# sandyresearch/chipmunk

Hardware: AMD Instinct MI355X
Metric: DiT denoise steps/sec at fixed sparsity (higher is better)
Workload: dtype bf16

## Files before the change

### chipmunk_amd/_native.py

```python
from __future__ import annotations

import ctypes
import os

_HERE = os.path.dirname(os.path.abspath(__file__))
LIB_PATH = os.environ.get("CHIPMUNK_HIP_LIB") or os.path.join(_HERE, "lib", "libchipmunk_hip.so")

SYMBOLS = [
    "chipmunk_last_error", "chipmunk_abi_version", "chipmunk_set_option", "chipmunk_set_random_seed",
    "chipmunk_csp_attn", "chipmunk_csp_attn_out", "chipmunk_csp_128_attn", "chipmunk_dense_attn", "chipmunk_dense_colsum_attn",
    "chipmunk_csp_mlp_mm1", "chipmunk_csp_mlp_mm1_scatter", "chipmunk_csp_mlp_mm1_fp8", "chipmunk_csp_mlp_mm2_and_scatter_add", "chipmunk_csp_scatter_add", "chipmunk_csp_mlp_mm2",
    "chipmunk_csp_mlp_mm1_ragged", "chipmunk_csp_mlp_mm1_scatter_ragged", "chipmunk_csp_mlp_mm1_fp8_ragged", "chipmunk_csp_mlp_mm2_ragged",
    "chipmunk_csp_mlp_mm2_and_scatter_add_ragged", "chipmunk_csp_scatter_add_ragged", "chipmunk_block_mean_ragged", "chipmunk_transpose16_pitched",
    "chipmunk_csp_mlp_mm1_batched", "chipmunk_csp_mlp_mm1_scatter_batched", "chipmunk_csp_mlp_mm1_fp8_batched", "chipmunk_csp_mlp_mm2_batched",
    "chipmunk_csp_mlp_mm2_and_scatter_add_batched", "chipmunk_csp_scatter_add_batched",
    "chipmunk_csp_mlp_mm1_glu", "chipmunk_csp_mlp_mm1_glu_batched", "chipmunk_csp_mlp_mm1_glu_fp8", "chipmunk_csp_mlp_mm1_glu_fp8_batched",
    "chipmunk_topk_indices", "chipmunk_topk_delta_indices", "chipmunk_topk_mask", "chipmunk_mask_to_indices", "chipmunk_mask_to_sorted_indices", "chipmunk_packed_mask_to_indices", "chipmunk_mask_row_counts", "chipmunk_mask_to_ragged_indices", "chipmunk_copy_indices",
    "chipmunk_bitpack", "chipmunk_bitunpack", "chipmunk_transpose16", "chipmunk_block_mean", "chipmunk_quantize_fp8", "chipmunk_gather_rows", "chipmunk_qkv_split_norm", "chipmunk_split_heads_rownorm", "chipmunk_dense_colsum_topk_mask", "chipmunk_dense_attn_strided", "chipmunk_csp_attn_out_ragged", "chipmunk_compact_indices", "chipmunk_residual_ln_modulate", "chipmunk_dense_colsum_attn_strided", "chipmunk_dense_colsum_topk_mask_strided", "chipmunk_release_scratch", "chipmunk_big_scratch_fallbacks",
    "chipmunk_host_alloc", "chipmunk_host_free", "chipmunk_copy_d2h_async", "chipmunk_copy_h2d_async", "chipmunk_host_bytes",
]

_lib = None


def lib() -> ctypes.CDLL:
    global _lib
    if _lib is None:
        if not os.path.exists(LIB_PATH):
            raise ImportError(
                f"{LIB_PATH} is missing: build it with `python -m chipmunk_amd.build` (hipcc --offload-arch=gfx950). "
                "chipmunk_amd has no CPU fallback.")
        _lib = ctypes.CDLL(LIB_PATH)
        _lib.chipmunk_last_error.restype = ctypes.c_char_p
        _lib.chipmunk_abi_version.restype = ctypes.c_int
        for item in filter(None, os.environ.get("CHIPMUNK_AMD_OPTIONS", "").split(",")):
            name, _, val = item.partition("=")
            if _lib.chipmunk_set_option(name.strip().encode(), int(val)) != 0:
                raise ValueError(f"CHIPMUNK_AMD_OPTIONS: {_lib.chipmunk_last_error().decode()}")
    return _lib


def last_error() -> str:
    return lib().chipmunk_last_error().decode()


def check(rc: int, what: str) -> None:
    if rc != 0:
        raise RuntimeError(f"{what}: {last_error()}")


def set_option(name: str, value: int) -> None:
    check(lib().chipmunk_set_option(name.encode(), int(value)), "chipmunk_set_option")


def manual_seed(seed: int) -> None:
    check(lib().chipmunk_set_random_seed(ctypes.c_uint64(int(seed) & 0xFFFFFFFFFFFFFFFF)), "chipmunk_set_random_seed")


class HostBuffer:

    def __init__(self, numel: int, dtype) -> None:
        import torch
        self.dtype = dtype
        self._numel = int(numel)
        self._itemsize = torch.empty(0, dtype=dtype).element_size()
        self.nbytes = self._numel * self._itemsize
        p = ctypes.c_void_p()
        check(lib().chipmunk_host_alloc(ctypes.c_size_t(max(self.nbytes, 1)), ctypes.byref(p)), "chipmunk_host_alloc")
        self.ptr = p.value

    def numel(self) -> int:
        return self._numel

    def element_size(self) -> int:
        return self._itemsize

    def is_pinned(self) -> bool:
        return True

    def free(self) -> None:
        if getattr(self, "ptr", None):
            lib().chipmunk_host_free(ctypes.c_void_p(self.ptr))
            self.ptr = None

    def __del__(self):
        try:
            self.free()
        except Exception:
            pass


def copy_d2h_async(host_ptr: int, dev_ptr: int, nbytes: int, stream: int) -> None:
    check(lib().chipmunk_copy_d2h_async(ctypes.c_void_p(host_ptr), ctypes.c_void_p(dev_ptr), ctypes.c_size_t(nbytes), ctypes.c_void_p(stream)),
          "chipmunk_copy_d2h_async")


def copy_h2d_async(dev_ptr: int, host_ptr: int, nbytes: int, stream: int) -> None:
    check(lib().chipmunk_copy_h2d_async(ctypes.c_void_p(dev_ptr), ctypes.c_void_p(host_ptr), ctypes.c_size_t(nbytes), ctypes.c_void_p(stream)),
          "chipmunk_copy_h2d_async")


# ... 5 lines not shown
```

### chipmunk_amd/csrc/attn.hip

```cpp
#include "common.h"
#include "attn_params.h"
#include <type_traits>

namespace {

constexpr int QG = 192;
constexpr int QW = 48;
constexpr int KVT = 32;
constexpr int NST = 4;
constexpr int KRING = 8;
constexpr int HD = 128;
constexpr int TILE_BYTES = KVT * HD * 2;
constexpr float SCALE_LOG2E = 0.08838834764f * 1.44269504089f;
constexpr int NSTV = NST + 1;
constexpr int KEY_RING_OFF = (NST + NSTV) * TILE_BYTES;
constexpr int CS_OFF = KEY_RING_OFF + KRING * 256;
constexpr int ATTN_LDS_BYTES = CS_OFF + 2 * 2 * 4 * KVT * 4;

__device__ __forceinline__ f32x4 mfma16(bf16x8 a, bf16x8 b, f32x4 c) {
    return __builtin_amdgcn_mfma_f32_16x16x32_bf16(a, b, c, 0, 0, 0);
}

#ifdef ATTN_PROF
__device__ unsigned long long g_attn_prof[8 * 8];
// ... 1132 lines not shown
    p.o_scale = 1.f;
    if (use_dense64(B, H, Nq, Nk)) {
        CM_CHECK((int64_t)Nk * p.ks[2] * 2 < (1ll << 32) && (int64_t)Nk * p.vs[2] * 2 < (1ll << 32),
                 "attention: one head's K or V spans more than 4 GiB (32-bit DMA offsets)");
        return chipmunk_dense64_launch(q, k, v, o, l, p.qs, p.ks, p.vs, p.os, B, H, Nq, Nk, (hipStream_t)stream);
    }
    return launch_attn<false, false, true>(p, (hipStream_t)stream);
}

extern "C" int chipmunk_dense_attn(const void *q, const void *k, const void *v, const int64_t q_strides[3],
                                   const int64_t k_strides[3], const int64_t v_strides[3], void *o, float *l, int B,
                                   int H, int Nq, int Nk, void *stream) {
    return chipmunk_dense_attn_strided(q, k, v, q_strides, k_strides, v_strides, o, nullptr, l, B, H, Nq, Nk, stream);
}

extern "C" int chipmunk_dense_colsum_attn_strided(const void *q, const void *k, const void *v, const int64_t q_strides[3],
                                                  const int64_t k_strides[3], const int64_t v_strides[3], const float *pin,
                                                  void *o, const int64_t *o_strides, void *cs, float *l, int B, int H, int Nq,
                                                  int Nk, int cs_stride, void *stream) {
    if (int e = check_common(q, k, v, o, B, H, Nq, Nk)) return e;
    CM_CHECK(l && cs && pin, "dense_colsum_attn: p / cs / l missing");
    CM_CHECK(cs_stride >= Nk, "dense_colsum_attn: cs row stride %d < Nk %d", cs_stride, Nk);
    if (int e = check_strides(q_strides, "q")) return e;
    if (int e = check_strides(k_strides, "k")) return e;
    if (int e = check_strides(v_strides, "v")) return e;
    AttnParams p = {};
    p.q = (const uint16_t *)q, p.k = (const uint16_t *)k, p.v = (const uint16_t *)v, p.o = (uint16_t *)o;
    for (int i = 0; i < 3; ++i) p.qs[i] = q_strides[i], p.ks[i] = k_strides[i], p.vs[i] = v_strides[i];
    if (int e = output_strides(p.os, o_strides, H, Nq)) return e;
    p.l_out = l, p.p_in = pin, p.cs = (uint16_t *)cs, p.cs_stride = cs_stride;
    p.B = B, p.H = H, p.Nq = Nq, p.Nk = Nk, p.G = (Nq + QG - 1) / QG;
    p.o_scale = 1.f;
    hipStream_t st = (hipStream_t)stream;
    int rc;
    if (chipmunk_get_option("attn_fused_colsum") == 5) {
        if (use_colsum64(B, H, Nq, Nk)) return chipmunk_colsum64_launch(p, st);
        return launch_attn<false, false, false, true>(p, st);
    }
    if (use_dense64(B, H, Nq, Nk)) {
        CM_CHECK((int64_t)Nk * p.ks[2] * 2 < (1ll << 32) && (int64_t)Nk * p.vs[2] * 2 < (1ll << 32),
                 "attention: one head's K or V spans more than 4 GiB (32-bit DMA offsets)");
        if (chipmunk_get_option("attn_fused_colsum") != 2) {
            int hc = H;
            uint16_t *part = nullptr;
            const int hc_min = chipmunk_get_option("attn_fused_colsum") == 4 ? 1 : 0;
            if (hc_min) hc = 1;
            for (; hc >= 1; hc /= 2) {
                part = (uint16_t *)chipmunk_big_scratch(st, chipmunk_colsum_part_bytes(hc == H ? B : 1, hc, Nq, Nk));
                if (part) break;
            }
            if (part && hc == H) return chipmunk_dense64_colsum_launch(p, part, st);
            if (part) {
                for (int b = 0; b < B; ++b)
                    for (int h0 = 0; h0 < H; h0 += hc) {
                        AttnParams c = p;
                        const int hn = H - h0 < hc ? H - h0 : hc;
                        const int64_t bh0 = (int64_t)b * H + h0;
                        c.q += b * p.qs[0] + h0 * p.qs[1], c.k += b * p.ks[0] + h0 * p.ks[1], c.v += b * p.vs[0] + h0 * p.vs[1];
                        c.o += b * p.os[0] + h0 * p.os[1];
                        c.l_out += bh0 * Nq, c.p_in += bh0 * Nq, c.cs += bh0 * p.G * (int64_t)cs_stride;
                        c.B = 1, c.H = hn;
                        if (int e = chipmunk_dense64_colsum_launch(c, part, st)) return e;
                    }
                return CHIPMUNK_OK;
            }
        }
        rc = chipmunk_dense64_launch(q, k, v, o, l, p.qs, p.ks, p.vs, p.os, B, H, Nq, Nk, st);
    } else {
        rc = launch_attn<false, false, true>(p, st);
    }
    if (rc != CHIPMUNK_OK) return rc;
    if (use_colsum64(B, H, Nq, Nk)) return chipmunk_colsum64_launch(p, st);
    return launch_attn<false, false, false, true>(p, st);
}

extern "C" int chipmunk_dense_colsum_attn(const void *q, const void *k, const void *v, const int64_t q_strides[3],
                                          const int64_t k_strides[3], const int64_t v_strides[3], const float *pin,
                                          void *o, void *cs, float *l, int B, int H, int Nq, int Nk, int cs_stride,
                                          void *stream) {
    return chipmunk_dense_colsum_attn_strided(q, k, v, q_strides, k_strides, v_strides, pin, o, nullptr, cs, l, B, H, Nq, Nk,
                                              cs_stride, stream);
}

extern "C" int chipmunk_dense_colsum_topk_mask_strided(const void *q, const void *k, const void *v, const int64_t q_strides[3],
                                               const int64_t k_strides[3], const int64_t v_strides[3], const float *pin, void *o,
                                               const int64_t *o_strides, float *l, int B, int H, int Nq, int Nk, const void *static_mask,
                                               int64_t static_stride, int static_rows, const void *group_flags, void *mask,
                                               int topk, double random_amount, void *stream) {
    if (int e = check_common(q, k, v, o, B, H, Nq, Nk)) return e;
    CM_CHECK(l && pin && mask, "dense_colsum_topk_mask: p / l / mask missing");
    if (int e = check_strides(q_strides, "q")) return e;
    if (int e = check_strides(k_strides, "k")) return e;
    if (int e = check_strides(v_strides, "v")) return e;
    hipStream_t st = (hipStream_t)stream;
    if (!use_dense64(B, H, Nq, Nk) || chipmunk_get_option("attn_fused_colsum") == 2 || (Nk & 3) || Nk > CHIPMUNK_TOPK_MASK_MAX_N)
        return CHIPMUNK_ERR_UNSUPPORTED;
    AttnParams p = {};
    p.q = (const uint16_t *)q, p.k = (const uint16_t *)k, p.v = (const uint16_t *)v, p.o = (uint16_t *)o;
    for (int i = 0; i < 3; ++i) p.qs[i] = q_strides[i], p.ks[i] = k_strides[i], p.vs[i] = v_strides[i];
    CM_CHECK((int64_t)Nk * p.ks[2] * 2 < (1ll << 32) && (int64_t)Nk * p.vs[2] * 2 < (1ll << 32),
             "attention: one head's K or V spans more than 4 GiB (32-bit DMA offsets)");
    if (int e = output_strides(p.os, o_strides, H, Nq)) return e;
    p.l_out = l, p.p_in = pin, p.cs = nullptr, p.cs_stride = 0;
    p.B = B, p.H = H, p.Nq = Nq, p.Nk = Nk, p.G = (Nq + QG - 1) / QG;
    p.o_scale = 1.f;
    uint16_t *part = (uint16_t *)chipmunk_big_scratch(st, chipmunk_colsum_part_bytes(B, H, Nq, Nk));
    if (!part) return CHIPMUNK_ERR_UNSUPPORTED;
    if (int e = chipmunk_dense64_colsum_launch(p, part, st)) return e;
    const int nrb = ((Nq + 255) / 256) * 2;
    return chipmunk_topk_mask_parts(part, chipmunk_colsum_part_stride(Nk), nrb, p.G, Nq, static_mask, static_stride, static_rows, group_flags, mask, B * H * p.G, Nk,
                                    topk, random_amount, st);
}

extern "C" int chipmunk_dense_colsum_topk_mask(const void *q, const void *k, const void *v, const int64_t q_strides[3],
                                               const int64_t k_strides[3], const int64_t v_strides[3], const float *pin, void *o,
                                               float *l, int B, int H, int Nq, int Nk, const void *static_mask,
                                               int64_t static_stride, int static_rows, const void *group_flags, void *mask,
                                               int topk, double random_amount, void *stream) {
    return chipmunk_dense_colsum_topk_mask_strided(q, k, v, q_strides, k_strides, v_strides, pin, o, nullptr, l, B, H, Nq, Nk,
                                                   static_mask, static_stride, static_rows, group_flags, mask, topk, random_amount,
                                                   stream);
}
```

### chipmunk_amd/csrc/attn_params.h

```cpp
#pragma once
#include <stdint.h>
#include <hip/hip_runtime.h>

struct AttnParams {
    const uint16_t *q, *k, *v;
    uint16_t *o;
    const uint16_t *o_in;
    int64_t qs[3], ks[3], vs[3], os[3];
    const int32_t *indices, *counts;
    const int64_t *idx_off;
    float *l_out;
    const float *p_in;
    uint16_t *cs;
    int cs_stride;
    int B, H, Nq, Nk, G, idx_stride;
    float o_scale;
    int split_full, nsplit;
    float *ws;
    int32_t *tickets;
    const int32_t *plan;
    int xcd_chunks;
    const float *kmax;
    uint16_t *cs_part;
    int cs_pstride;
    int probe;
};


int chipmunk_csp64_launch(const AttnParams &p, int inplace, int grid, hipStream_t stream);
int chipmunk_dense64_colsum_launch(const AttnParams &p, uint16_t *part, hipStream_t stream);
int chipmunk_topk_mask_parts(const uint16_t *part, int part_stride, int nrb, int groups_per_bh, int Nq, const void *static_mask, int64_t static_stride,
                             int static_rows, const void *group_flags, void *mask, int rows, int n, int k, double random_amount,
                             hipStream_t stream);
size_t chipmunk_colsum_part_bytes(int B, int H, int Nq, int Nk);
int chipmunk_colsum_part_stride(int Nk);
int chipmunk_colsum64_launch(const AttnParams &p, hipStream_t stream);
int chipmunk_csp96_launch(const AttnParams &p, int inplace, int grid, hipStream_t stream);
const float *chipmunk_knorm_max(const uint16_t *k, const int64_t ks[3], int B, int H, int Nk, hipStream_t stream);

__host__ __device__ inline int colsum_part_rows(int j, int nwg, int &r0, int &r1) {
    const int a = (3 * j) >> 2, w0 = 3 * j - 4 * a;
    r0 = 2 * a + (w0 ? 1 : 0);
    r1 = 2 * (a + 1);
    return (w0 >= 2 && a + 1 < nwg) ? 2 : 1;
}

struct IndexRow {
    const int32_t *ptr;
    int width;
};
__device__ __forceinline__ IndexRow index_row(const AttnParams &p, int64_t item) {
    if (p.idx_off) {
        const int64_t o = p.idx_off[item];
        return {p.indices + o, (int)(p.idx_off[item + 1] - o)};
    }
    return {p.indices + item * p.idx_stride, p.idx_stride};
}
```

### chipmunk_amd/csrc/capi.hip

```cpp
#include "common.h"

static thread_local char g_last_error[512] = "";

void chipmunk_set_error(const char *fmt, ...) {
    va_list ap;
    va_start(ap, fmt);
    vsnprintf(g_last_error, sizeof(g_last_error), fmt, ap);
    va_end(ap);
}

extern "C" const char *chipmunk_last_error(void) { return g_last_error; }
extern "C" int chipmunk_abi_version(void) { return 1; }

#include <string.h>
namespace {
struct Option { const char *name; int value; };
Option g_options[] = {{"mm1_variant", 0}, {"mm2_variant", 0}, {"attn_variant", 0}, {"m2i_variant", 0}, {"topk_variant", 0}, {"mm1_nr", 0}, {"mm2_nr", 0}, {"mm1_probe", 0}, {"attn_xcd_chunks", 0}, {"attn_no_order", 0}, {"attn_no_tail", 0}, {"mm1_no_split", 0}, {"mm2_no_split", 0}, {"attn_no_split", 0}, {"attn_split_gather", 0}, {"attn_pp", 0}, {"attn_dense64", 0}, {"attn_csp64", 0}, {"attn_colsum64", 0}, {"attn_csp96", 0}, {"attn_nomax", 0}, {"attn_fused_colsum", 0}, {"attn_cs_probe", 0}, {"big_scratch_gb", 0}, {"attn_balanced", 0}, {"attn_row_split", 0}, {"mm2_order", 0}, {"topk_mask_stream", 0}};
}
int chipmunk_get_option(const char *name) {
    for (auto &o : g_options) if (strcmp(o.name, name) == 0) return o.value;
    return 0;
}
extern "C" int chipmunk_set_option(const char *name, int value) {
    for (auto &o : g_options) if (strcmp(o.name, name) == 0) { o.value = value; return CHIPMUNK_OK; }
    chipmunk_set_error("unknown option '%s'", name);
    return CHIPMUNK_ERR_INVALID;
}

#include <atomic>
namespace {
std::atomic<uint64_t> g_rng_seed{0x243F6A8885A308D3ull};
std::atomic<uint64_t> g_rng_counter{0};
}
uint32_t chipmunk_next_random_salt() {
    uint64_t z = g_rng_seed.load(std::memory_order_relaxed) + 0x9E3779B97F4A7C15ull * (g_rng_counter.fetch_add(1) + 1);
    z = (z ^ (z >> 30)) * 0xBF58476D1CE4E5B9ull;
    z = (z ^ (z >> 27)) * 0x94D049BB133111EBull;
    z ^= z >> 31;
    return (uint32_t)(z >> 16);
}
extern "C" int chipmunk_set_random_seed(uint64_t seed) {
    g_rng_seed.store(seed * 0xD6E8FEB86659FD93ull + 0x243F6A8885A308D3ull);
    g_rng_counter.store(0);
    return CHIPMUNK_OK;
}

#include <algorithm>
#include <map>
#include <mutex>
#include <utility>
namespace {
struct Scratch { void *ptr; size_t bytes; };
std::mutex g_scratch_mu;
std::map<std::pair<int, hipStream_t>, Scratch> g_scratch;
}
void *chipmunk_scratch(hipStream_t stream, size_t bytes) {
    int dev = 0;
    if (hipGetDevice(&dev) != hipSuccess) return nullptr;
    std::lock_guard<std::mutex> lock(g_scratch_mu);
    Scratch &s = g_scratch[{dev, stream}];
    if (s.bytes >= bytes) return s.ptr;
    if (s.ptr) {
        (void)hipStreamSynchronize(stream);
        (void)hipFree(s.ptr);
        s.ptr = nullptr, s.bytes = 0;
    }
    const size_t want = (bytes + (size_t(1) << 20) - 1) & ~((size_t(1) << 20) - 1);
    void *ptr = nullptr;
    if (hipMalloc(&ptr, want) != hipSuccess) return nullptr;
    if (hipMemsetAsync(ptr, 0, want, stream) != hipSuccess) {
        (void)hipFree(ptr);
        return nullptr;
    }
    s.ptr = ptr, s.bytes = want;
    return ptr;
}
namespace {
std::map<std::pair<int, hipStream_t>, Scratch> g_big;
struct BigFail { size_t want, free_then; int calls_left; };
std::map<int, BigFail> g_big_failed;
int g_big_fallbacks = 0;
}
void *chipmunk_big_scratch(hipStream_t stream, size_t bytes) {
    int dev = 0;
    if (hipGetDevice(&dev) != hipSuccess) return nullptr;
    std::lock_guard<std::mutex> lock(g_scratch_mu);
    Scratch &s = g_big[{dev, stream}];
    if (s.bytes >= bytes) return s.ptr;
    const int cap_gb = chipmunk_get_option("big_scratch_gb");
    const size_t cap = (size_t)(cap_gb > 0 ? cap_gb : 24) << 30;
    const size_t want = (bytes + (size_t(1) << 20) - 1) & ~((size_t(1) << 20) - 1);
    if (want > cap) return ++g_big_fallbacks, nullptr;
    size_t free_b = 0, total_b = 0;
    const bool have_info = hipMemGetInfo(&free_b, &total_b) == hipSuccess;
    auto f = g_big_failed.find(dev);
    if (f != g_big_failed.end() && want >= f->second.want) {
        const bool more_free = have_info && free_b > f->second.free_then + ((size_t)1 << 30);
        if (!more_free && --f->second.calls_left > 0) return ++g_big_fallbacks, nullptr;
        g_big_failed.erase(f);
        f = g_big_failed.end();
// ... 90 lines not shown
```

### chipmunk_amd/csrc/indexed_io.hip

```cpp
#include "common.h"
#include "attn_params.h"

namespace {

__device__ __forceinline__ uint32_t wave_incl_scan(uint32_t x) {
    x += (uint32_t)__builtin_amdgcn_update_dpp(0, (int)x, 0x111, 0xf, 0xf, true);
    x += (uint32_t)__builtin_amdgcn_update_dpp(0, (int)x, 0x112, 0xf, 0xf, true);
    x += (uint32_t)__builtin_amdgcn_update_dpp(0, (int)x, 0x114, 0xf, 0xf, true);
    x += (uint32_t)__builtin_amdgcn_update_dpp(0, (int)x, 0x118, 0xf, 0xf, true);
    x += (uint32_t)__builtin_amdgcn_update_dpp(0, (int)x, 0x142, 0xa, 0xf, false);
    x += (uint32_t)__builtin_amdgcn_update_dpp(0, (int)x, 0x143, 0xc, 0xf, false);
    return x;
}
struct M2IParams {
    const uint8_t *mask;
    int32_t *indices;
    int32_t *counts;
    int n, pad_n, multiple_of;
    const int64_t *offsets;
};

template <bool PACKED, bool SORTED = false, bool RAGGED = false>
__global__ __launch_bounds__(256) void mask_to_indices_kernel(const M2IParams p) {
    extern __shared__ __attribute__((aligned(16))) unsigned char smem[];
// ... 136 lines not shown
        for (int blk = 0; blk < NB; ++blk) {
            pre[tid * NB + blk] = run;
            run += __popcll(T[tid * NB + blk]);
        }
        cls[tid + 1] = run;
    }
    __syncthreads();
    if (tid == 0) {
        uint32_t run = 0;
        for (int t = 0; t < 32; ++t) {
            const uint32_t c = cls[t + 1];
            cls[t] = run;
            run += c;
            if (t == 31) cls[32] = run;
        }
    }
    __syncthreads();
    const int total = (int)cls[32];

    for (int cell = tid; cell < 32 * NB; cell += 256) {
        const int t = cell / NB, blk = cell - t * NB;
        unsigned long long v = T[cell];
        int pos = (int)(cls[t] + pre[cell]);
        while (v) {
            const int bit = __builtin_ctzll(v);
            v &= v - 1;
            put(pos++, ((blk * 64 + bit) << 5) + t);
        }
    }
    if constexpr (RAGGED) zero_rest(total);

    if (tid == 0) {
        const int padded = ((total + p.multiple_of - 1) / p.multiple_of) * p.multiple_of;
        int pos = total;
        for (int i = 0; i < NI && pos < padded; ++i) {
            uint32_t z = ~bits[i];
            const int rem = n - i * 32;
            if (rem < 32) z &= (1u << rem) - 1u;
            while (z && pos < padded) {
                const int bit = __builtin_ctz(z);
                z &= z - 1;
                put(pos++, i * 32 + bit);
            }
        }
        if constexpr (!RAGGED) p.counts[row] = padded;
    }
}

struct RowCountParams {
    const uint8_t *mask;
    int32_t *counts;
    int64_t *lengths;
    int64_t rows;
    int n, pad_n, multiple_of;
};

template <bool PACKED>
__global__ __launch_bounds__(256) void mask_row_counts_kernel(const RowCountParams p) {
    const int lane = threadIdx.x & 63;
    const int64_t row = (int64_t)blockIdx.x * 4 + (threadIdx.x >> 6);
    if (row >= p.rows) return;
    const int nbytes = PACKED ? p.n >> 3 : p.n;
    const uint8_t *src = p.mask + (PACKED ? (row * p.n) >> 3 : row * p.n);
    auto set_in_byte = [](uint32_t b) { return PACKED ? (uint32_t)__popc(b) : (uint32_t)(b != 0); };
    auto set_in_word = [](uint32_t x) {
        if constexpr (!PACKED) x = (x | (x >> 1) | (x >> 2) | (x >> 3) | (x >> 4) | (x >> 5) | (x >> 6) | (x >> 7)) & 0x01010101u;
        return (uint32_t)__popc(x);
    };
    const int head = min(nbytes, (int)((16 - ((uintptr_t)src & 15)) & 15));
    uint32_t cnt = lane < head ? set_in_byte(src[lane]) : 0u;
    const int nvec = (nbytes - head) >> 4;
    const u32x4 *vec = (const u32x4 *)(src + head);
#pragma unroll 4
    for (int i = lane; i < nvec; i += 64) {
        const u32x4 x = vec[i];
        cnt += set_in_word(x[0]) + set_in_word(x[1]) + set_in_word(x[2]) + set_in_word(x[3]);
    }
    const int tail = head + (nvec << 4) + lane;
    if (tail < nbytes) cnt += set_in_byte(src[tail]);
    const int64_t kept = (uint32_t)__builtin_amdgcn_readlane((int)wave_incl_scan(cnt), 63);
    if (lane == 0) {
        const int64_t padded = ((kept + p.multiple_of - 1) / p.multiple_of) * p.multiple_of;
        p.counts[row] = (int32_t)padded;
        p.lengths[row] = (min(padded, (int64_t)p.pad_n) + 31) / 32 * 32;
    }
}

struct TopkParams {
    const void *act;
    void *cache;
    int32_t *indices;
    int32_t *counts;
    int rows, cols, multiple_of;
    float quantile, random_amount;
    uint32_t salt;
};

template <typename T>
__device__ __forceinline__ float load_as_float(const T *p, int i);
template <>
__device__ __forceinline__ float load_as_float<uint16_t>(const uint16_t *p, int i) { return bf16_bits_to_f32(p[i]); }
template <>
__device__ __forceinline__ float load_as_float<_Float16>(const _Float16 *p, int i) { return (float)p[i]; }
template <>
__device__ __forceinline__ float load_as_float<float>(const float *p, int i) { return p[i]; }

template <typename T>
__device__ __forceinline__ float round_to(float x);
template <>
__device__ __forceinline__ float round_to<uint16_t>(float x) { return round_bf16(x); }
template <>
__device__ __forceinline__ float round_to<_Float16>(float x) { return (float)(_Float16)x; }
template <>
__device__ __forceinline__ float round_to<float>(float x) { return x; }

__device__ __forceinline__ float hash_uniform(uint32_t row, uint32_t col, uint32_t salt) {
    uint32_t x = (row * 0x9E3779B9u ^ (col + 0x7F4A7C15u) * 0x85EBCA6Bu) + salt * 0xC2B2AE35u;
    x ^= x >> 16, x *= 0x7feb352du, x ^= x >> 15, x *= 0x846ca68bu, x ^= x >> 16;
    return (float)(x >> 8) * (1.0f / 16777216.0f);
}

__device__ __forceinline__ int compact_slot(bool keep, int lane, int w, uint32_t *wave_tot, int &base) {
    const unsigned long long bal = __ballot(keep);
    const int before = __popcll(bal & ((1ull << lane) - 1ull));
    if (lane == 0) wave_tot[w] = __popcll(bal);
    __syncthreads();
    int off = base, tot = 0;
#pragma unroll
    for (int i = 0; i < 16; ++i) {
        const int c = wave_tot[i];
        off += i < w ? c : 0;
        tot += c;
    }
    __syncthreads();
    base += tot;
    return keep ? off + before : -1;
}

template <typename T, bool DELTA>
__global__ __launch_bounds__(1024) void topk_indices_kernel(const TopkParams p) {
    __shared__ uint32_t wave_tot[16];
    __shared__ float thr_s;
    const int tid = threadIdx.x, lane = tid & 63, w = tid >> 6;
    const int row = blockIdx.x;
    const T *x = (const T *)p.act + (int64_t)row * p.cols;
    T *xc = DELTA ? (T *)p.cache + (int64_t)row * p.cols : nullptr;
    int32_t *out = p.indices + (int64_t)row * p.cols;
    const int cols = p.cols;
    auto value = [&](int c) {
        const float b = load_as_float<T>(x, c);
        if constexpr (DELTA) return fabsf(round_to<T>(b - load_as_float<T>(xc, c)));
        else return b;
    };

    const uint32_t salt = p.salt ^ (__float_as_uint(value(0)) * 0x27D4EB2Fu);
    if (p.quantile == 0.f) {
        if constexpr (DELTA)
            for (int c = tid; c < cols; c += 1024) xc[c] = x[c];
        for (int c = tid; c < cols; c += 1024) out[c] = c;
        if (tid == 0) p.counts[row] = cols;
        return;
    }
    if (p.quantile == 1.f) {
        for (int c = tid; c < cols; c += 1024) out[c] = -1;
        if (tid == 0) p.counts[row] = 0;
        return;
    }
// ... 152 lines not shown
        else if (r0 + r < R)
            for (int e = 0; e < 8; ++e)
                if (c0 + ch * 8 + e < C) {
                    const uint32_t x = src[boff + (int64_t)(r0 + r) * C + c0 + ch * 8 + e];
                    v[e >> 1] |= x << (16 * (e & 1));
                }
#pragma unroll
        for (int e = 0; e < 4; ++e) {
            tile[ch * 8 + 2 * e][r] = (uint16_t)(v[e] & 0xffffu);
            tile[ch * 8 + 2 * e + 1][r] = (uint16_t)(v[e] >> 16);
        }
    }
    __syncthreads();
#pragma unroll
    for (int i = 0; i < 2; ++i) {
        const int item = i * 256 + tid, c = item >> 3, ch = item & 7;
        if (c0 + c >= C) continue;
        uint16_t *d = dst + (int64_t)blockIdx.z * C * ld + (int64_t)(c0 + c) * ld + r0 + ch * 8;
        if (r0 + ch * 8 + 8 <= ld && ((ld & 7) == 0)) *(u32x4 *)d = *(const u32x4 *)&tile[c][ch * 8];
        else
            for (int e = 0; e < 8; ++e)
                if (r0 + ch * 8 + e < ld) d[e] = tile[c][ch * 8 + e];
    }
}

__global__ __launch_bounds__(256) void compact_indices_kernel(const int32_t *indices, int64_t idx_stride, const int32_t *counts,
                                                             const int64_t *offsets, int32_t *flat) {
    const int64_t r = blockIdx.x;
    const int32_t *src = indices + r * idx_stride;
    const int64_t o = offsets[r];
    int32_t *dst = flat + o;
    const int width = (int)(offsets[r + 1] - o);
    int c = counts[r];
    c = c < 0 ? 0 : (c < width ? c : width);
    c = c < idx_stride ? c : (int)idx_stride;
    if ((((uintptr_t)src | (uintptr_t)dst) & 15) == 0) {
        const int c4 = c >> 2;
        for (int i = threadIdx.x; i < c4; i += 256) ((u32x4 *)dst)[i] = ((const u32x4 *)src)[i];
        for (int i = (c4 << 2) + threadIdx.x; i < c; i += 256) dst[i] = src[i];
    } else {
        for (int i = threadIdx.x; i < c; i += 256) dst[i] = src[i];
    }
    for (int i = c + threadIdx.x; i < width; i += 256) dst[i] = 0;
}

size_t m2i_lds_bytes(int n, bool sorted) {
    const int NI = (n + 31) >> 5, NB = (NI + 63) >> 6;
    if (sorted) return (size_t)NB * 64 * 4 + (size_t)(NB + 1) * 4 + 16;
    return (size_t)NB * 64 * 4 + (size_t)32 * NB * 8 + (size_t)32 * NB * 4 + 33 * 4 + 16;
}

template <bool PACKED, bool SORTED = false, bool RAGGED = false>
int launch_m2i(const void *mask, int32_t *indices, int32_t *counts, int64_t rows, int n, int pad_n, int multiple_of,
               void *stream, const int64_t *offsets = nullptr) {
    CM_CHECK(mask && indices && (RAGGED ? (const void *)offsets : (const void *)counts), "mask_to_indices: null pointer");
    CM_CHECK(rows >= 0 && n > 0 && pad_n >= n && multiple_of > 0, "mask_to_indices: bad sizes rows=%lld n=%d pad_n=%d multiple_of=%d",
             (long long)rows, n, pad_n, multiple_of);
    CM_CHECK(rows < (1ll << 31), "mask_to_indices: too many rows");
    if (PACKED) CM_CHECK(n % 8 == 0, "packed_mask_to_indices: n must be a multiple of 8 (got %d)", n);
    const size_t lds = m2i_lds_bytes(n, SORTED);
    CM_CHECK(lds <= 160 * 1024, "mask_to_indices: row length %d needs %zu B of LDS (> 160 KiB)", n, lds);
    if (rows == 0) return CHIPMUNK_OK;
    auto kern = mask_to_indices_kernel<PACKED, SORTED, RAGGED>;
    if (lds > 64 * 1024) (void)hipFuncSetAttribute((const void *)kern, hipFuncAttributeMaxDynamicSharedMemorySize, (int)lds);
    M2IParams p = {(const uint8_t *)mask, indices, counts, n, pad_n, multiple_of, offsets};
    hipLaunchKernelGGL(kern, dim3((unsigned)rows), dim3(256), lds, (hipStream_t)stream, p);
    CM_LAUNCH_CHECK();
    return CHIPMUNK_OK;
}


struct TopkMaskParams {
    const uint16_t *cs;
    const uint8_t *stat;
    const uint8_t *groups;
    uint8_t *mask;
    int64_t cs_stride, stat_stride;
    int rows, n, k, stat_rows;
    float random_amount;
    uint32_t salt;
    const uint16_t *parts;
    int64_t pstride;
    int nrb, ngroups, nq;
};

__device__ __forceinline__ uint32_t bf16_key(uint32_t u) {
    return (u & 0x8000u) ? (~u & 0xffffu) : (u | 0x8000u);
}

template <int KPT, bool ALIGNED, bool PARTS = false>
__global__ __launch_bounds__(1024) void topk_mask_kernel(const TopkMaskParams p) {
    constexpr int NV = KPT / 4;
    __shared__ int wave_cnt[16];
    const int tid = threadIdx.x, lane = tid & 63, w = tid >> 6;
    const int row = blockIdx.x;
    const int n = p.n;
    const uint16_t *x = nullptr;
    int prow = 1;
    int64_t row1 = 0;
    if constexpr (PARTS) {
        const int bh = row / p.ngroups, g = row - bh * p.ngroups;
        int r0, r1;
        prow = colsum_part_rows(g, p.nrb / 2, r0, r1);
        x = p.parts + ((int64_t)bh * p.nrb + r0) * p.pstride;
        row1 = (int64_t)(r1 - r0) * p.pstride;
    } else {
        x = p.cs + (int64_t)row * p.cs_stride;
    }
    const uint32_t lane_off8 = 8u * (uint32_t)tid;
    const uint32_t lane_off4 = 4u * (uint32_t)tid;
    uint32_t key[NV][2];
    constexpr int LB = NV % 10 == 0 ? 10 : (NV % 8 == 0 ? 8 : (NV % 6 == 0 ? 6 : 4));
    static_assert(NV % LB == 0, "NV must split into whole load batches");
#pragma unroll
    for (int j0 = 0; j0 < NV; j0 += LB) {
        uint32_t raw[LB][2];
#pragma unroll
        for (int jj = 0; jj < LB; ++jj) {
            const int c = 4 * tid + 4096 * (j0 + jj);
            uint32_t v0 = 0xffffffffu, v1 = 0xffffffffu;
            if constexpr (ALIGNED) {
                if (c < n) {
                    const u32x2 v = *(const u32x2 *)((const unsigned char *)(x + 4096 * (j0 + jj)) + lane_off8);
                    v0 = v[0], v1 = v[1];
                    if constexpr (PARTS) {
                        if (prow == 2) {
                            float a0 = __uint_as_float(v0 << 16), a1 = __uint_as_float(v0 & 0xffff0000u);
                            float a2 = __uint_as_float(v1 << 16), a3 = __uint_as_float(v1 & 0xffff0000u);
                            const u32x2 y = *(const u32x2 *)((const unsigned char *)(x + row1 + 4096 * (j0 + jj)) + lane_off8);
                            a0 += __uint_as_float(y[0] << 16), a1 += __uint_as_float(y[0] & 0xffff0000u);
                            a2 += __uint_as_float(y[1] << 16), a3 += __uint_as_float(y[1] & 0xffff0000u);
                            v0 = pack_bf16x2(a0, a1), v1 = pack_bf16x2(a2, a3);
                        }
                    }
                }
            } else if (c < n) {
                v0 = v1 = 0;
#pragma unroll
                for (int e = 0; e < 4; ++e) {
                    const uint32_t u = c + e < n ? x[c + e] : 0xffffu;
                    if (e < 2) v0 |= u << (16 * e);
                    else v1 |= u << (16 * (e - 2));
                }
            }
            raw[jj][0] = v0, raw[jj][1] = v1;
        }
#pragma unroll
        for (int jj = 0; jj < LB; ++jj) {
            key[j0 + jj][0] = bf16_key(raw[jj][0] & 0xffffu) | (bf16_key(raw[jj][0] >> 16) << 16);
            key[j0 + jj][1] = bf16_key(raw[jj][1] & 0xffffu) | (bf16_key(raw[jj][1] >> 16) << 16);
        }
        __builtin_amdgcn_sched_barrier(0);
    }
    auto block_count = [&](int mine) {
#pragma unroll
        for (int d = 32; d > 0; d >>= 1) mine += __shfl_xor(mine, d);
        if (lane == 0) wave_cnt[w] = mine;
        __syncthreads();
        int t = 0;
#pragma unroll
        for (int i = 0; i < 16; ++i) t += wave_cnt[i];
        __syncthreads();
        return t;
    };
    const bool active = p.groups == nullptr || p.groups[row] != 0;
    const int k = p.k < n ? p.k : n;
// ... 274 lines not shown
                    }
                }
            }
            const int mine = (int)(cnt2 & 0xffffu) + (int)(cnt2 >> 16);
            if (block_count(mine) >= k) res = cand;
        }
        thr = res;
        int gt = 0;
        for (int j0 = 0; j0 < nsteps; j0 += U) {
            uint32_t kw[U][2];
#pragma unroll
            for (int jj = 0; jj < U; ++jj) load_raw(j0 + jj, kw[jj][0], kw[jj][1]);
#pragma unroll
            for (int jj = 0; jj < U; ++jj) {
                to_keys(kw[jj][0], kw[jj][1]);
#pragma unroll
                for (int h = 0; h < 2; ++h) {
                    const uint32_t lo = kw[jj][h] & 0xffffu, hi = kw[jj][h] >> 16;
                    gt += (lo > thr ? 1 : 0) + (hi > thr ? 1 : 0);
                    my_ties += (lo == thr ? 1 : 0) + (hi == thr ? 1 : 0);
                }
            }
        }
        ties_to_take = k - block_count(gt);
    }
    int tie_budget = 0;
    {
        int incl = my_ties;
#pragma unroll
        for (int d = 1; d < 64; d <<= 1) {
            const int o = __shfl_up(incl, d);
            if (lane >= d) incl += o;
        }
        if (lane == 63) wave_cnt[w] = incl;
        __syncthreads();
        int before = incl - my_ties;
#pragma unroll
        for (int i = 0; i < 16; ++i) before += i < w ? wave_cnt[i] : 0;
        __syncthreads();
        tie_budget = ties_to_take - before;
    }
    uint8_t *out = p.mask + (int64_t)row * n;
    const uint8_t *st = p.stat ? p.stat + (int64_t)(row % p.stat_rows) * p.stat_stride : nullptr;
    for (int j0 = 0; j0 < nsteps; j0 += U) {
        uint32_t kw[U][2], sbv[U];
#pragma unroll
        for (int jj = 0; jj < U; ++jj) {
            const int c = 4 * tid + 4096 * (j0 + jj);
            kw[jj][0] = kw[jj][1] = 0;
            if (select) load_raw(j0 + jj, kw[jj][0], kw[jj][1]);
            sbv[jj] = 0;
            if constexpr (ALIGNED) {
                if (st && c < n) sbv[jj] = *(const uint32_t *)(st + c);
            } else if (st) {
#pragma unroll
                for (int e = 0; e < 4; ++e)
                    if (c + e < n) sbv[jj] |= (uint32_t)st[c + e] << (8 * e);
            }
        }
#pragma unroll
        for (int jj = 0; jj < U; ++jj) {
            const int c = 4 * tid + 4096 * (j0 + jj);
            if (c >= n) continue;
            if (select) to_keys(kw[jj][0], kw[jj][1]);
            uint32_t bytes = 0;
#pragma unroll
            for (int e = 0; e < 4; ++e) {
                const uint32_t kv = (kw[jj][e >> 1] >> (16 * (e & 1))) & 0xffffu;
                bool keep = kv > thr;
                const bool tie = kv == thr && tie_budget > 0 && c + e < n;
                tie_budget -= tie ? 1 : 0;
                keep = keep || tie;
                if (rnd && !keep) keep = hash_uniform(row, c + e, salt) < p.random_amount;
                keep = keep || ((sbv[jj] >> (8 * e)) & 0xffu) != 0;
                bytes |= (keep ? 1u : 0u) << (8 * e);
            }
            if constexpr (ALIGNED) {
                *(uint32_t *)(out + c) = bytes;
            } else {
#pragma unroll
                for (int e = 0; e < 4; ++e)
                    if (c + e < n) out[c + e] = (uint8_t)(bytes >> (8 * e));
            }
        }
    }
}

}

extern "C" int chipmunk_mask_to_indices(const void *mask, int32_t *indices, int32_t *counts, int64_t rows, int n,
                                        int pad_n, int multiple_of, void *stream) {
    return launch_m2i<false>(mask, indices, counts, rows, n, pad_n, multiple_of, stream);
}

extern "C" int chipmunk_packed_mask_to_indices(const void *packed, int32_t *indices, int32_t *counts, int64_t rows,
                                               int n, int pad_n, int multiple_of, void *stream) {
    return launch_m2i<true>(packed, indices, counts, rows, n, pad_n, multiple_of, stream);
}

static int launch_topk(const void *activation, void *cache, int dtype, int32_t *indices, int32_t *counts, int rows,
                       int cols, double sparsity_amount, int multiple_of, double random_amount, void *stream) {
    CM_CHECK(activation && indices && counts, "topk_indices: null pointer");
    CM_CHECK(rows >= 0 && cols >= 1024, "topk_indices: rows >= 0 and cols >= 1024 required (the quantile is taken over the first 1024 columns); got rows=%d cols=%d", rows, cols);
    CM_CHECK(multiple_of > 0, "topk_indices: multiple_of must be positive");
    CM_CHECK(sparsity_amount >= 0.0 && sparsity_amount <= 1.0, "topk_indices: sparsity_amount must be in [0,1]");
    if (rows == 0) return CHIPMUNK_OK;
    TopkParams p = {activation, cache, indices, counts, rows, cols, multiple_of, (float)sparsity_amount, (float)random_amount,
                    random_amount > 0.0 ? chipmunk_next_random_salt() : 0u};
    hipStream_t s = (hipStream_t)stream;
#define LAUNCH_TOPK(T)                                                                                           \
    do {                                                                                                         \
        if (cache) hipLaunchKernelGGL((topk_indices_kernel<T, true>), dim3(rows), dim3(1024), 0, s, p);          \
        else hipLaunchKernelGGL((topk_indices_kernel<T, false>), dim3(rows), dim3(1024), 0, s, p);               \
    } while (0)
    switch (dtype) {
        case CHIPMUNK_DTYPE_BF16: LAUNCH_TOPK(uint16_t); break;
        case CHIPMUNK_DTYPE_FP16: LAUNCH_TOPK(_Float16); break;
        case CHIPMUNK_DTYPE_FP32: LAUNCH_TOPK(float); break;
        default: CM_CHECK(false, "topk_indices: unsupported dtype code %d", dtype);
    }
#undef LAUNCH_TOPK
    CM_LAUNCH_CHECK();
    return CHIPMUNK_OK;
}

extern "C" int chipmunk_mask_to_sorted_indices(const void *mask, int packed, int32_t *indices, int32_t *counts,
                                               int64_t rows, int n, int pad_n, int multiple_of, void *stream) {
    return packed ? launch_m2i<true, true>(mask, indices, counts, rows, n, pad_n, multiple_of, stream)
                  : launch_m2i<false, true>(mask, indices, counts, rows, n, pad_n, multiple_of, stream);
}

extern "C" int chipmunk_mask_row_counts(const void *mask, int packed, int32_t *counts, int64_t *lengths, int64_t rows, int n,
                                        int pad_n, int multiple_of, void *stream) {
    CM_CHECK(mask && counts && lengths, "mask_row_counts: null pointer");
    CM_CHECK(rows >= 0 && n > 0 && pad_n >= n && multiple_of > 0, "mask_row_counts: bad sizes rows=%lld n=%d pad_n=%d multiple_of=%d",
             (long long)rows, n, pad_n, multiple_of);
    CM_CHECK(rows < (1ll << 31), "mask_row_counts: too many rows");
    CM_CHECK(!packed || n % 8 == 0, "mask_row_counts: n must be a multiple of 8 for a packed mask (got %d)", n);
    const size_t lds = m2i_lds_bytes(n, true);
    CM_CHECK(lds <= 160 * 1024, "mask_to_indices: row length %d needs %zu B of LDS (> 160 KiB)", n, lds);
    if (rows == 0) return CHIPMUNK_OK;
    RowCountParams p = {(const uint8_t *)mask, counts, lengths, rows, n, pad_n, multiple_of};
    const dim3 grid((unsigned)((rows + 3) / 4));
    if (packed) hipLaunchKernelGGL(mask_row_counts_kernel<true>, grid, dim3(256), 0, (hipStream_t)stream, p);
    else hipLaunchKernelGGL(mask_row_counts_kernel<false>, grid, dim3(256), 0, (hipStream_t)stream, p);
    CM_LAUNCH_CHECK();
    return CHIPMUNK_OK;
}

extern "C" int chipmunk_mask_to_ragged_indices(const void *mask, int packed, int sorted, const int64_t *offsets, int32_t *flat,
                                               int64_t rows, int n, int multiple_of, void *stream) {
    if (packed) return sorted ? launch_m2i<true, true, true>(mask, flat, nullptr, rows, n, n, multiple_of, stream, offsets)
                              : launch_m2i<true, false, true>(mask, flat, nullptr, rows, n, n, multiple_of, stream, offsets);
    return sorted ? launch_m2i<false, true, true>(mask, flat, nullptr, rows, n, n, multiple_of, stream, offsets)
                  : launch_m2i<false, false, true>(mask, flat, nullptr, rows, n, n, multiple_of, stream, offsets);
}

extern "C" int chipmunk_topk_indices(const void *activation, int dtype, int32_t *indices, int32_t *counts, int rows,
                                     int cols, double sparsity_amount, int multiple_of, double random_amount,
                                     void *stream) {
    return launch_topk(activation, nullptr, dtype, indices, counts, rows, cols, sparsity_amount, multiple_of,
                       random_amount, stream);
}

extern "C" int chipmunk_topk_delta_indices(const void *activation, void *cache, int dtype, int32_t *indices,
                                           int32_t *counts, int rows, int cols, double sparsity_amount,
// ... 15 lines not shown
    if (elem_size == 2)
        hipLaunchKernelGGL(copy_indices_kernel<uint16_t>, dim3((unsigned)rows), dim3(256), 0, s, (const uint16_t *)src,
                           (uint16_t *)dst, inds, counts, M, R, F);
    else
        hipLaunchKernelGGL(copy_indices_kernel<uint32_t>, dim3((unsigned)rows), dim3(256), 0, s, (const uint32_t *)src,
                           (uint32_t *)dst, inds, counts, M, R, F);
    CM_LAUNCH_CHECK();
    return CHIPMUNK_OK;
}

extern "C" int chipmunk_bitpack(const void *mask, void *packed, int64_t n, void *stream) {
    CM_CHECK(mask && packed && n >= 0, "bitpack: bad arguments");
    if (n == 0) return CHIPMUNK_OK;
    const int64_t nb = (n + 7) >> 3;
    const unsigned grid = (unsigned)((nb + 255) / 256 < 8192 ? (nb + 255) / 256 : 8192);
    hipLaunchKernelGGL(bitpack_kernel, dim3(grid), dim3(256), 0, (hipStream_t)stream, (const uint8_t *)mask,
                       (uint8_t *)packed, n);
    CM_LAUNCH_CHECK();
    return CHIPMUNK_OK;
}

extern "C" int chipmunk_bitunpack(const void *packed, void *mask, int64_t n, void *stream) {
    CM_CHECK(mask && packed && n >= 0, "bitunpack: bad arguments");
    if (n == 0) return CHIPMUNK_OK;
    const int64_t nb = (n + 7) >> 3;
    const unsigned grid = (unsigned)((nb + 255) / 256 < 8192 ? (nb + 255) / 256 : 8192);
    hipLaunchKernelGGL(bitunpack_kernel, dim3(grid), dim3(256), 0, (hipStream_t)stream, (const uint8_t *)packed,
                       (uint8_t *)mask, n);
    CM_LAUNCH_CHECK();
    return CHIPMUNK_OK;
}

extern "C" int chipmunk_transpose16(const void *src, void *dst, int B, int R, int C, void *stream) {
    CM_CHECK(src && dst && B > 0 && R > 0 && C > 0, "transpose16: bad arguments");
    CM_CHECK((C & 7) == 0 || true, "unreachable");
    hipLaunchKernelGGL(transpose16_kernel, dim3((C + 63) / 64, (R + 63) / 64, B), dim3(256), 0, (hipStream_t)stream,
                       (const uint16_t *)src, (uint16_t *)dst, R, C, R);
    CM_LAUNCH_CHECK();
    return CHIPMUNK_OK;
}

extern "C" int chipmunk_transpose16_pitched(const void *src, void *dst, int B, int R, int C, int ld, void *stream) {
    CM_CHECK(src && dst && B > 0 && R > 0 && C > 0, "transpose16: bad arguments");
    CM_CHECK(ld >= R, "transpose16: the output pitch ld (%d) must be at least R (%d)", ld, R);
    hipLaunchKernelGGL(transpose16_kernel, dim3((C + 63) / 64, (ld + 63) / 64, B), dim3(256), 0, (hipStream_t)stream,
                       (const uint16_t *)src, (uint16_t *)dst, R, C, ld);
    CM_LAUNCH_CHECK();
    return CHIPMUNK_OK;
}

template <typename V>
__global__ __launch_bounds__(256) void gather_rows_kernel(const V *src, V *dst, const int32_t *map, int64_t n_out,
                                                          int64_t n_src, int64_t cpr, int64_t total) {
    for (int64_t idx = (int64_t)blockIdx.x * 256 + threadIdx.x; idx < total; idx += (int64_t)gridDim.x * 256) {
        const int64_t row = idx / cpr, c = idx - row * cpr;
        const int64_t o = row / n_out, r = row - o * n_out;
        dst[idx] = src[(o * n_src + map[r]) * cpr + c];
    }
}

extern "C" int chipmunk_gather_rows(const void *src, void *dst, const int32_t *map, int64_t outer, int64_t n_src,
                                    int64_t n_out, int64_t row_bytes, void *stream) {
    CM_CHECK(src && dst && map, "gather_rows: null pointer");
    CM_CHECK(outer >= 0 && n_src > 0 && n_out >= 0 && row_bytes > 0, "gather_rows: bad sizes");
    if (outer == 0 || n_out == 0) return CHIPMUNK_OK;
    hipStream_t s = (hipStream_t)stream;
    const uintptr_t align = (uintptr_t)src | (uintptr_t)dst | (uintptr_t)row_bytes;
#define LAUNCH_GATHER(V)                                                                                              \
    do {                                                                                                              \
        const int64_t cpr = row_bytes / (int64_t)sizeof(V), total = outer * n_out * cpr;                               \
        const int64_t blocks = (total + 255) / 256;                                                                    \
        hipLaunchKernelGGL((gather_rows_kernel<V>), dim3((unsigned)(blocks > 65536 * 16 ? 65536 * 16 : blocks)),       \
                           dim3(256), 0, s, (const V *)src, (V *)dst, map, n_out, n_src, cpr, total);                  \
    } while (0)
    if ((align & 15) == 0) LAUNCH_GATHER(u32x4);
    else if ((align & 3) == 0) LAUNCH_GATHER(uint32_t);
    else if ((align & 1) == 0) LAUNCH_GATHER(uint16_t);
    else LAUNCH_GATHER(uint8_t);
#undef LAUNCH_GATHER
    CM_LAUNCH_CHECK();
    return CHIPMUNK_OK;
}

int chipmunk_topk_mask_parts(const uint16_t *part, int part_stride, int nrb, int groups_per_bh, int Nq, const void *static_mask, int64_t static_stride,
                             int static_rows, const void *group_flags, void *mask, int rows, int n, int k, double random_amount,
                             hipStream_t s) {
    CM_CHECK(part && mask && rows >= 0 && n > 0 && (n & 3) == 0 && n <= CHIPMUNK_TOPK_MASK_MAX_N && k >= 0 && part_stride >= n && (part_stride & 3) == 0, "topk_mask_parts: bad arguments");
    CM_CHECK(!static_mask || (static_rows > 0 && static_stride >= n && (static_stride & 3) == 0 && ((uintptr_t)static_mask & 3) == 0),
             "topk_mask_parts: bad static mask geometry");
    CM_CHECK(((uintptr_t)mask & 3) == 0 && ((uintptr_t)part & 7) == 0, "topk_mask_parts: unaligned buffers");
    if (rows == 0) return CHIPMUNK_OK;
    TopkMaskParams p = {nullptr, (const uint8_t *)static_mask, (const uint8_t *)group_flags, (uint8_t *)mask, 0, static_stride,
                        rows, n, k, static_mask ? static_rows : 1, (float)random_amount,
                        random_amount > 0.0 ? chipmunk_next_random_salt() : 0u};
    p.parts = part, p.pstride = part_stride, p.nrb = nrb, p.ngroups = groups_per_bh, p.nq = Nq;
    if (n > 1024 * 120 || chipmunk_get_option("topk_mask_stream") == 1) hipLaunchKernelGGL((topk_mask_stream_kernel<true, true>), dim3(rows), dim3(1024), 0, s, p);
    else if (n <= 1024 * 16) hipLaunchKernelGGL((topk_mask_kernel<16, true, true>), dim3(rows), dim3(1024), 0, s, p);
    else if (n <= 1024 * 48) hipLaunchKernelGGL((topk_mask_kernel<48, true, true>), dim3(rows), dim3(1024), 0, s, p);
    else hipLaunchKernelGGL((topk_mask_kernel<120, true, true>), dim3(rows), dim3(1024), 0, s, p);
    CM_LAUNCH_CHECK();
    return CHIPMUNK_OK;
}

__global__ __launch_bounds__(256) void qkv_split_norm_kernel(const uint16_t *qkv, int64_t row_stride, const uint16_t *qw,
                                                             const uint16_t *kw, uint16_t *q, uint16_t *k, uint16_t *v, int64_t n,
                                                             int H, float eps, int64_t segments, const float *fcos, const float *fsin,
                                                             int64_t rope_rows) {
    const int l15 = threadIdx.x & 15;
    u32x4 wq = {0x3f803f80u, 0x3f803f80u, 0x3f803f80u, 0x3f803f80u}, wk = wq;
    if (qw) wq = *(const u32x4 *)(qw + l15 * 8);
    if (kw) wk = *(const u32x4 *)(kw + l15 * 8);
    for (int64_t seg = ((int64_t)blockIdx.x * 256 + threadIdx.x) >> 4; seg < segments; seg += ((int64_t)gridDim.x * 256) >> 4) {
        const int64_t tok = seg / (3 * H);
        const int rem = (int)(seg - tok * 3 * H), which = rem / H, h = rem - which * H;
        u32x4 x = *(const u32x4 *)(qkv + tok * row_stride + (int64_t)rem * 128 + l15 * 8);
        uint16_t *dst = (which == 0 ? q : which == 1 ? k : v) + ((int64_t)h * n + tok) * 128 + l15 * 8;
        if (which < 2) {
            float f[8], ss = 0.f;
#pragma unroll
            for (int e = 0; e < 4; ++e) {
                f[2 * e] = __uint_as_float(x[e] << 16), f[2 * e + 1] = __uint_as_float(x[e] & 0xffff0000u);
                ss = __builtin_fmaf(f[2 * e], f[2 * e], ss);
                ss = __builtin_fmaf(f[2 * e + 1], f[2 * e + 1], ss);
            }
            ss = row16_sum(ss);
            const float r = 1.0f / __builtin_sqrtf(ss * (1.0f / 128.0f) + eps);
            const u32x4 w = which == 0 ? wq : wk;
#pragma unroll
            for (int e = 0; e < 4; ++e) {
                float a = f[2 * e] * r, b = f[2 * e + 1] * r;
                round_bf16_pair(a, b);
                x[e] = pack_bf16x2(a * __uint_as_float(w[e] << 16), b * __uint_as_float(w[e] & 0xffff0000u));
            }
            if (fcos && tok < rope_rows) {
                const f32x4 c0 = *(const f32x4 *)(fcos + tok * 128 + l15 * 8), c1 = *(const f32x4 *)(fcos + tok * 128 + l15 * 8 + 4);
                const f32x4 s0 = *(const f32x4 *)(fsin + tok * 128 + l15 * 8), s1 = *(const f32x4 *)(fsin + tok * 128 + l15 * 8 + 4);
#pragma unroll
                for (int e = 0; e < 4; ++e) {
                    const float re = __uint_as_float(x[e] << 16), im = __uint_as_float(x[e] & 0xffff0000u);
                    const float cr = e < 2 ? c0[2 * e] : c1[2 * e - 4], ci = e < 2 ? c0[2 * e + 1] : c1[2 * e - 3];
                    const float sr = e < 2 ? s0[2 * e] : s1[2 * e - 4], si = e < 2 ? s0[2 * e + 1] : s1[2 * e - 3];
                    x[e] = pack_bf16x2(re * cr + (-im) * sr, im * ci + re * si);
                }
            }
        }
        *(u32x4 *)dst = x;
    }
}

extern "C" int chipmunk_qkv_split_norm(const void *qkv, int64_t row_stride, const void *q_weight, const void *k_weight, void *q,
                                       void *k, void *v, int64_t n, int heads, float eps, const float *freqs_cos,
                                       const float *freqs_sin, int64_t rope_rows, void *stream) {
    CM_CHECK(qkv && q && k && v, "qkv_split_norm: null pointer");
    CM_CHECK(n >= 0 && heads > 0 && row_stride >= (int64_t)3 * heads * 128, "qkv_split_norm: bad sizes");
    CM_CHECK((((uintptr_t)qkv | (uintptr_t)q | (uintptr_t)k | (uintptr_t)v | (uintptr_t)q_weight | (uintptr_t)k_weight) & 15) == 0 &&
                 (row_stride & 7) == 0 && (((uintptr_t)freqs_cos | (uintptr_t)freqs_sin) & 15) == 0,
             "qkv_split_norm: pointers and the row stride must be 16-byte aligned");
    CM_CHECK((freqs_cos == nullptr) == (freqs_sin == nullptr) && rope_rows >= 0 && rope_rows <= n, "qkv_split_norm: bad rotary arguments");
    if (n == 0) return CHIPMUNK_OK;
    const int64_t segments = n * 3 * heads, blocks = (segments + 15) / 16;
    hipLaunchKernelGGL(qkv_split_norm_kernel, dim3((unsigned)(blocks > 256 * 64 ? 256 * 64 : blocks)), dim3(256), 0, (hipStream_t)stream,
                       (const uint16_t *)qkv, row_stride, (const uint16_t *)q_weight, (const uint16_t *)k_weight, (uint16_t *)q,
                       (uint16_t *)k, (uint16_t *)v, n, heads, eps, segments, freqs_cos, freqs_sin, freqs_cos ? rope_rows : 0);
    CM_LAUNCH_CHECK();
    return CHIPMUNK_OK;
}

extern "C" int chipmunk_topk_mask(const void *cs, int64_t cs_stride, const void *static_mask, int64_t static_stride,
                                  int static_rows, const void *group_flags, void *mask, int rows, int n, int k,
                                  double random_amount, void *stream) {
    CM_CHECK(cs && mask, "topk_mask: null pointer");
    CM_CHECK(rows >= 0 && n > 0 && k >= 0, "topk_mask: bad sizes (rows=%d n=%d k=%d)", rows, n, k);
    CM_CHECK(cs_stride >= n, "topk_mask: cs row stride %lld < n %d", (long long)cs_stride, n);
    CM_CHECK(n <= CHIPMUNK_TOPK_MASK_MAX_N, "topk_mask: rows of more than %d columns are not supported (got %d)", CHIPMUNK_TOPK_MASK_MAX_N, n);
    CM_CHECK(!static_mask || (static_rows > 0 && static_stride >= n), "topk_mask: bad static mask geometry");
    CM_CHECK(random_amount >= 0.0 && random_amount <= 1.0, "topk_mask: random_amount must be in [0,1]");
    if (rows == 0) return CHIPMUNK_OK;
    TopkMaskParams p = {(const uint16_t *)cs, (const uint8_t *)static_mask, (const uint8_t *)group_flags, (uint8_t *)mask,
                        cs_stride, static_stride, rows, n, k, static_mask ? static_rows : 1, (float)random_amount,
                        random_amount > 0.0 ? chipmunk_next_random_salt() : 0u};
    hipStream_t s = (hipStream_t)stream;
    const bool aligned = n % 4 == 0 && (((uintptr_t)cs) & 7) == 0 && (cs_stride * 2) % 8 == 0 && (((uintptr_t)mask) & 3) == 0 &&
                         (!static_mask || ((((uintptr_t)static_mask) & 3) == 0 && static_stride % 4 == 0));
#define LAUNCH_TM(KPT)                                                                                       \
    do {                                                                                                     \
        if (aligned) hipLaunchKernelGGL((topk_mask_kernel<KPT, true>), dim3(rows), dim3(1024), 0, s, p);     \
        else hipLaunchKernelGGL((topk_mask_kernel<KPT, false>), dim3(rows), dim3(1024), 0, s, p);            \
    } while (0)
    if (n > 1024 * 120 || chipmunk_get_option("topk_mask_stream") == 1) {
        if (aligned) hipLaunchKernelGGL((topk_mask_stream_kernel<true, false>), dim3(rows), dim3(1024), 0, s, p);
        else hipLaunchKernelGGL((topk_mask_stream_kernel<false, false>), dim3(rows), dim3(1024), 0, s, p);
    } else if (n <= 1024 * 16) LAUNCH_TM(16);
    else if (n <= 1024 * 48) LAUNCH_TM(48);
    else LAUNCH_TM(120);
#undef LAUNCH_TM
    CM_LAUNCH_CHECK();
    return CHIPMUNK_OK;
}

extern "C" int chipmunk_compact_indices(const int32_t *indices, int64_t idx_stride, const int32_t *counts, const int64_t *offsets,
                                        int32_t *flat, int64_t rows, void *stream) {
    CM_CHECK(indices && counts && offsets && flat, "compact_indices: null pointer");
    CM_CHECK(rows >= 0 && rows < (1ll << 31) && idx_stride > 0, "compact_indices: bad sizes rows=%lld idx_stride=%lld", (long long)rows,
             (long long)idx_stride);
    if (rows == 0) return CHIPMUNK_OK;
    hipLaunchKernelGGL(compact_indices_kernel, dim3((unsigned)rows), dim3(256), 0, (hipStream_t)stream, indices, idx_stride, counts,
                       offsets, flat);
    CM_LAUNCH_CHECK();
    return CHIPMUNK_OK;
}
```

### chipmunk_amd/csrc/torch_registry.cpp

```cpp
#include <ATen/ATen.h>
#include <ATen/hip/impl/HIPStreamMasqueradingAsCUDA.h>
#include <Python.h>
#include <c10/core/DeviceGuard.h>
#include <torch/library.h>

#include <vector>

#include "../../include/chipmunk_hip.h"

extern "C" {
PyObject *PyInit_cuda(void) {
    static struct PyModuleDef module_def = {PyModuleDef_HEAD_INIT, "cuda", NULL, -1, NULL};
    return PyModule_Create(&module_def);
}
}

namespace chipmunk {
namespace {

void *cur_stream(const at::Tensor &t) {
    return (void *)c10::hip::getCurrentHIPStreamMasqueradingAsCUDA(t.device().index()).stream();
}
void check(int rc, const char *op) { TORCH_CHECK(rc == 0, "chipmunk::", op, ": ", chipmunk_last_error()); }

// ... 659 lines not shown
          "packed_mask_to_indices");
    return {indices, counts};
}

at::Tensor transpose_last2(at::Tensor x) {
    CHECK_DEV(x);
    TORCH_CHECK(x.dim() >= 2 && x.element_size() == 2, "transpose_last2: need a >=2-D tensor of a 16-bit dtype");
    x = x.contiguous();
    const int64_t R = x.size(-2), C = x.size(-1), B = x.numel() / (R * C);
    auto sizes = x.sizes().vec();
    std::swap(sizes[sizes.size() - 1], sizes[sizes.size() - 2]);
    c10::DeviceGuard guard(x.device());
    at::Tensor out = at::empty(sizes, x.options());
    check(chipmunk_transpose16(x.data_ptr(), out.data_ptr(), (int)B, (int)R, (int)C, cur_stream(x)), "transpose_last2");
    return out;
}

at::Tensor transpose_last2_pitched(at::Tensor x, int64_t ld) {
    CHECK_DEV(x);
    TORCH_CHECK(x.dim() >= 2 && x.element_size() == 2, "transpose_last2_pitched: need a >=2-D tensor of a 16-bit dtype");
    x = x.contiguous();
    const int64_t R = x.size(-2), C = x.size(-1), B = x.numel() / (R * C);
    TORCH_CHECK(ld >= R, "transpose_last2_pitched: ld must be at least the row count");
    auto sizes = x.sizes().vec();
    sizes[sizes.size() - 2] = C;
    sizes[sizes.size() - 1] = ld;
    c10::DeviceGuard guard(x.device());
    at::Tensor out = at::empty(sizes, x.options());
    check(chipmunk_transpose16_pitched(x.data_ptr(), out.data_ptr(), (int)B, (int)R, (int)C, (int)ld, cur_stream(x)), "transpose_last2_pitched");
    return out;
}

at::Tensor block_mean(at::Tensor x, int64_t mbm) {
    CHECK_DEV(x);
    TORCH_CHECK(x.dim() == 3 && x.scalar_type() == at::kBFloat16, "block_mean: need a [b, n, c] bfloat16 tensor");
    TORCH_CHECK(mbm > 0 && x.size(1) > 0, "block_mean: mbm and n must be positive");
    x = x.contiguous();
    c10::DeviceGuard guard(x.device());
    const int64_t n = x.size(1), blocks = (n + mbm - 1) / mbm;
    at::Tensor out = at::empty({x.size(0), blocks, x.size(2)}, x.options());
    if (n % mbm == 0) {
        check(chipmunk_block_mean(x.data_ptr(), out.data_ptr(), x.size(0) * n, (int)x.size(2), (int)mbm, cur_stream(x)), "block_mean");
    } else {
        for (int64_t b = 0; b < x.size(0); ++b)
            check(chipmunk_block_mean_ragged(x[b].data_ptr(), out[b].data_ptr(), n, (int)x.size(2), (int)mbm, cur_stream(x)), "block_mean");
    }
    return out;
}

at::Tensor quantize_fp8(at::Tensor x, at::Tensor scale, double max_value) {
    CHECK_DEV(x); CHECK_DEV(scale);
    TORCH_CHECK(x.scalar_type() == at::kBFloat16, "quantize_fp8: x must be bfloat16");
    TORCH_CHECK(scale.scalar_type() == at::kFloat && scale.numel() == 1, "quantize_fp8: scale must be a one-element float32 tensor");
    TORCH_CHECK(x.numel() % 8 == 0, "quantize_fp8: the element count must be a multiple of 8");
    x = x.contiguous();
    c10::DeviceGuard guard(x.device());
    at::Tensor out = at::empty(x.sizes(), x.options().dtype(at::kFloat8_e4m3fn));
    check(chipmunk_quantize_fp8(x.data_ptr(), scale.data_ptr<float>(), out.data_ptr(), x.numel(), (float)max_value, cur_stream(x)), "quantize_fp8");
    return out;
}

std::vector<at::Tensor> mask_to_sorted_indices(at::Tensor mask, at::IntArrayRef shape, int64_t multiple_of,
                                               int64_t pad_to_multiple_of) {
    CHECK_DEV(mask);
    const bool packed = mask.scalar_type() == at::kByte;
    TORCH_CHECK(packed || mask.scalar_type() == at::kBool, "mask must be bool, or uint8 bit-packed with a shape");
    mask = mask.contiguous();
    std::vector<int64_t> shp = packed ? shape.vec() : mask.sizes().vec();
    TORCH_CHECK(shp.size() == 4, "shape must be [b, h, m, n]");
    const int64_t b = shp[0], h = shp[1], m = shp[2], n = shp[3];
    if (packed) TORCH_CHECK(n % 8 == 0 && mask.numel() * 8 >= b * h * m * n, "bad packed mask");
    const int64_t pad_n = ((n + pad_to_multiple_of - 1) / pad_to_multiple_of) * pad_to_multiple_of;
    c10::DeviceGuard guard(mask.device());
    at::Tensor indices = at::empty({b, h, m, pad_n}, mask.options().dtype(at::kInt));
    at::Tensor counts = at::empty({b, h, m}, mask.options().dtype(at::kInt));
    check(chipmunk_mask_to_sorted_indices(mask.data_ptr(), packed ? 1 : 0, indices.data_ptr<int>(),
                                          counts.data_ptr<int>(), b * h * m, (int)n, (int)pad_n, (int)multiple_of,
                                          cur_stream(mask)),
          "mask_to_sorted_indices");
    return {indices, counts};
}

std::vector<at::Tensor> mask_to_ragged_indices(at::Tensor mask, at::IntArrayRef shape, int64_t multiple_of, int64_t pad_to_multiple_of,
                                               bool sorted) {
    CHECK_DEV(mask);
    const bool packed = mask.scalar_type() == at::kByte;
    TORCH_CHECK(packed || mask.scalar_type() == at::kBool, "mask must be bool, or uint8 bit-packed with a shape");
    TORCH_CHECK(multiple_of > 0 && pad_to_multiple_of > 0, "multiple_of and pad_to_multiple_of must be positive");
    mask = mask.contiguous();
    std::vector<int64_t> shp = packed ? shape.vec() : mask.sizes().vec();
    TORCH_CHECK(shp.size() == 4, "shape must be [b, h, m, n]");
    const int64_t b = shp[0], h = shp[1], m = shp[2], n = shp[3], rows = b * h * m;
    if (packed) TORCH_CHECK(n % 8 == 0 && mask.numel() * 8 >= rows * n, "bad packed mask");
    const int64_t pad_n = ((n + pad_to_multiple_of - 1) / pad_to_multiple_of) * pad_to_multiple_of;
    TORCH_CHECK(n > 0 && pad_n <= INT_MAX, "rows must have between 1 and 2^31 - 1 columns");
    c10::DeviceGuard guard(mask.device());
    at::Tensor counts = at::empty({b, h, m}, mask.options().dtype(at::kInt));
    at::Tensor len = at::empty({rows}, mask.options().dtype(at::kLong));
    check(chipmunk_mask_row_counts(mask.data_ptr(), packed ? 1 : 0, counts.data_ptr<int>(), len.data_ptr<int64_t>(), rows, (int)n,
                                   (int)pad_n, (int)multiple_of, cur_stream(mask)),
          "mask_to_ragged_indices");
    at::Tensor offsets = at::zeros({rows + 1}, len.options());
    if (rows) offsets.narrow(0, 1, rows).copy_(len.cumsum(0));
    const int64_t total = rows ? offsets[rows].item<int64_t>() : 0;
    at::Tensor flat = at::empty({total + 64}, counts.options());
    flat.narrow(0, total, 64).zero_();
    check(chipmunk_mask_to_ragged_indices(mask.data_ptr(), packed ? 1 : 0, sorted ? 1 : 0, offsets.data_ptr<int64_t>(), flat.data_ptr<int>(),
                                          rows, (int)n, (int)multiple_of, cur_stream(mask)),
          "mask_to_ragged_indices");
    return {flat, offsets, counts};
}

std::vector<at::Tensor> dense_colsum_attn_layout(at::Tensor q, at::Tensor k, at::Tensor v, at::Tensor p, bool token_major_o);
at::Tensor topk_mask(at::Tensor cs, int64_t k, double random_amount, const c10::optional<at::Tensor> &groups,
                     const c10::optional<at::Tensor> &static_mask);
std::vector<at::Tensor> dense_colsum_topk_mask(at::Tensor q, at::Tensor k, at::Tensor v, at::Tensor p, int64_t k_top, double random_amount,
                                               const c10::optional<at::Tensor> &groups, const c10::optional<at::Tensor> &static_mask,
                                               bool token_major_o) {
    CHECK_DEV(q); CHECK_DEV(k); CHECK_DEV(v); CHECK_DEV(p);
    CHECK_BF16(q); CHECK_BF16(k); CHECK_BF16(v);
    const bool shapes_ok = q.dim() == 4 && k.dim() == 4 && v.dim() == 4 && q.size(3) == 128 && q.stride(3) == 1 && k.stride(3) == 1 &&
                           v.stride(3) == 1 && p.scalar_type() == at::kFloat && p.is_contiguous();
    if (shapes_ok) {
        const int64_t B = q.size(0), H = q.size(1), Nq = q.size(2), Nk = k.size(2), G = (Nq + 191) / 192;
        const void *st = nullptr, *gf = nullptr;
        int64_t st_stride = 0, st_rows = 1;
        at::Tensor stc, gfc;
        bool ok = p.numel() == B * H * Nq;
        if (ok && static_mask.has_value() && static_mask->defined()) {
            stc = *static_mask;
            ok = stc.is_cuda() && stc.scalar_type() == at::kBool && stc.dim() == 4 && stc.size(3) == Nk && stc.size(2) == G && stc.size(1) == H &&
                 (stc.size(0) == 1 || stc.size(0) == B) && stc.stride(3) == 1 && stc.stride(1) == G * stc.stride(2) &&
                 (stc.size(0) == 1 || stc.stride(0) == H * stc.stride(1));
            if (ok) st = stc.data_ptr(), st_stride = stc.stride(2), st_rows = stc.size(0) * H * G;
        }
        if (ok && groups.has_value() && groups->defined()) {
            gfc = *groups;
            ok = gfc.is_cuda() && gfc.scalar_type() == at::kBool && gfc.dim() == 4 && gfc.size(3) == 1 && gfc.size(2) == G && gfc.size(1) == H &&
                 (gfc.size(0) == 1 || gfc.size(0) == B);
            if (ok) {
                gfc = gfc.expand({B, H, G, 1}).contiguous();
                gf = gfc.data_ptr();
            }
        }
        if (ok) {
            c10::DeviceGuard guard(q.device());
            at::Tensor o = alloc_o(q, q, token_major_o);
            const int64_t os[3] = {o.stride(0), o.stride(1), o.stride(2)};
            at::Tensor l = at::empty({B, H, Nq, 1}, q.options().dtype(at::kFloat));
            at::Tensor mask = at::empty({B, H, G, Nk}, q.options().dtype(at::kBool));
            const int64_t qs[3] = {q.stride(0), q.stride(1), q.stride(2)}, ks[3] = {k.stride(0), k.stride(1), k.stride(2)},
                          vs[3] = {v.stride(0), v.stride(1), v.stride(2)};
            const int rc = chipmunk_dense_colsum_topk_mask_strided(q.data_ptr(), k.data_ptr(), v.data_ptr(), qs, ks, vs, p.data_ptr<float>(), o.data_ptr(),
                                                           os, l.data_ptr<float>(), (int)B, (int)H, (int)Nq, (int)Nk, st, st_stride, (int)st_rows, gf,
                                                           mask.data_ptr(), (int)k_top, random_amount, cur_stream(q));
            if (rc == CHIPMUNK_OK) return {o, mask, l};
            if (rc != CHIPMUNK_ERR_UNSUPPORTED) check(rc, "dense_colsum_topk_mask");
        }
    }
    auto ocl = dense_colsum_attn_layout(q, k, v, p, token_major_o);
    at::Tensor cs = ocl[1];
    const int64_t Nk = k.size(2), G = (q.size(2) + 191) / 192;
    if (cs.size(-1) != Nk || cs.size(-2) != G) cs = cs.slice(-2, 0, G).slice(-1, 0, Nk);
    return {ocl[0], topk_mask(cs, k_top, random_amount, groups, static_mask), ocl[2]};
}

at::Tensor topk_mask(at::Tensor cs, int64_t k, double random_amount, const c10::optional<at::Tensor> &groups,
                     const c10::optional<at::Tensor> &static_mask) {
    CHECK_DEV(cs); CHECK_BF16(cs);
    TORCH_CHECK(cs.dim() == 4 && cs.stride(3) == 1, "cs must be [B, H, G, N] with a contiguous last dim");
    const int64_t B = cs.size(0), H = cs.size(1), G = cs.size(2), N = cs.size(3);
    if (!(cs.stride(1) == G * cs.stride(2) && (B == 1 || cs.stride(0) == H * cs.stride(1)))) cs = cs.contiguous();
    const int64_t rows = B * H * G;
    c10::DeviceGuard guard(cs.device());
    at::Tensor mask = at::empty({B, H, G, N}, cs.options().dtype(at::kBool));
    const void *st = nullptr, *gf = nullptr;
    int64_t st_stride = 0, st_rows = 1;
    at::Tensor stc, gfc;
    if (static_mask.has_value() && static_mask->defined()) {
        stc = *static_mask;
        CHECK_DEV(stc);
        TORCH_CHECK(stc.scalar_type() == at::kBool && stc.dim() == 4 && stc.size(3) == N && stc.size(2) == G &&
                    stc.size(1) == H && (stc.size(0) == 1 || stc.size(0) == B), "static_mask must be bool [1|B, H, G, N]");
        if (!(stc.stride(3) == 1 && stc.stride(1) == G * stc.stride(2) && (stc.size(0) == 1 || stc.stride(0) == H * stc.stride(1))))
            stc = stc.contiguous();
        st = stc.data_ptr(), st_stride = stc.stride(2), st_rows = stc.size(0) * H * G;
    }
    if (groups.has_value() && groups->defined()) {
        gfc = *groups;
        CHECK_DEV(gfc);
        TORCH_CHECK(gfc.scalar_type() == at::kBool && gfc.dim() == 4 && gfc.size(3) == 1 && gfc.size(2) == G &&
                    gfc.size(1) == H && (gfc.size(0) == 1 || gfc.size(0) == B), "groups must be bool [1|B, H, G, 1]");
        gfc = gfc.expand({B, H, G, 1}).contiguous();
        gf = gfc.data_ptr();
    }
    check(chipmunk_topk_mask(cs.data_ptr(), cs.stride(2), st, st_stride, (int)st_rows, gf, mask.data_ptr(), (int)rows, (int)N,
                             (int)k, random_amount, cur_stream(cs)),
          "topk_mask");
    return mask;
}

at::Tensor bitpack(at::Tensor mask) {
    TORCH_CHECK(mask.scalar_type() == at::kBool, "mask must be bool type");
    CHECK_DEV(mask);
    mask = mask.contiguous();
    c10::DeviceGuard guard(mask.device());
    at::Tensor packed = at::empty({(mask.numel() + 7) / 8}, mask.options().dtype(at::kByte));
    check(chipmunk_bitpack(mask.data_ptr(), packed.data_ptr(), mask.numel(), cur_stream(mask)), "bitpack");
    return packed;
}
at::Tensor bitunpack(at::Tensor packed, at::IntArrayRef shape) {
    TORCH_CHECK(packed.scalar_type() == at::kByte && packed.is_contiguous(), "packed must be a contiguous uint8 tensor");
    CHECK_DEV(packed);
    int64_t n = 1;
    for (auto d : shape) n *= d;
    TORCH_CHECK(packed.numel() * 8 >= n, "packed is too short for the given shape");
    c10::DeviceGuard guard(packed.device());
    at::Tensor mask = at::empty(shape, packed.options().dtype(at::kBool));
    check(chipmunk_bitunpack(packed.data_ptr(), mask.data_ptr(), n, cur_stream(packed)), "bitunpack");
    return mask;
}

std::vector<at::Tensor> qkv_split_norm(at::Tensor qkv, const c10::optional<at::Tensor> &q_weight, const c10::optional<at::Tensor> &k_weight,
                                       int64_t heads, double eps, const c10::optional<at::Tensor> &freqs_cos,
                                       const c10::optional<at::Tensor> &freqs_sin) {
    CHECK_DEV(qkv); CHECK_BF16(qkv);
    TORCH_CHECK(qkv.dim() == 2 && qkv.stride(1) == 1 && qkv.size(1) >= 3 * heads * 128, "qkv_split_norm: qkv must be [n, >= 3*heads*128] with a contiguous last dim");
    const void *qw = nullptr, *kw = nullptr;
    at::Tensor qwc, kwc;
    if (q_weight.has_value() && q_weight->defined()) { qwc = q_weight->contiguous(); CHECK_DEV(qwc); CHECK_BF16(qwc); TORCH_CHECK(qwc.numel() == 128); qw = qwc.data_ptr(); }
    if (k_weight.has_value() && k_weight->defined()) { kwc = k_weight->contiguous(); CHECK_DEV(kwc); CHECK_BF16(kwc); TORCH_CHECK(kwc.numel() == 128); kw = kwc.data_ptr(); }
    const int64_t n = qkv.size(0);
    const float *fc = nullptr, *fs = nullptr;
    int64_t rope_rows = 0;
    at::Tensor fcc, fsc;
    if (freqs_cos.has_value() && freqs_cos->defined()) {
        TORCH_CHECK(freqs_sin.has_value() && freqs_sin->defined(), "qkv_split_norm: freqs_cos without freqs_sin");
        fcc = freqs_cos->contiguous(), fsc = freqs_sin->contiguous();
        CHECK_DEV(fcc); CHECK_DEV(fsc);
        TORCH_CHECK(fcc.scalar_type() == at::kFloat && fsc.scalar_type() == at::kFloat && fcc.dim() == 2 && fcc.size(1) == 128 &&
                    fsc.sizes() == fcc.sizes() && fcc.size(0) <= n, "qkv_split_norm: freqs must be float32 [rows <= n, 128]");
        fc = fcc.data_ptr<float>(), fs = fsc.data_ptr<float>(), rope_rows = fcc.size(0);
    }
    c10::DeviceGuard guard(qkv.device());
    at::Tensor out = at::empty({3, 1, heads, n, 128}, qkv.options());
    check(chipmunk_qkv_split_norm(qkv.data_ptr(), qkv.stride(0), qw, kw, out[0].data_ptr(), out[1].data_ptr(), out[2].data_ptr(), n,
                                  (int)heads, (float)eps, fc, fs, rope_rows, cur_stream(qkv)),
          "qkv_split_norm");
    return {out[0], out[1], out[2]};
}

std::vector<at::Tensor> split_heads_rownorm(at::Tensor x, int64_t heads, int64_t parts, const c10::optional<at::Tensor> &w0,
                                            const c10::optional<at::Tensor> &w1, const c10::optional<at::Tensor> &w2, int64_t norm_mask,
                                            int64_t rope_mask, double eps, const c10::optional<at::Tensor> &freqs_cos,
                                            const c10::optional<at::Tensor> &freqs_sin) {
    CHECK_DEV(x); CHECK_BF16(x);
    TORCH_CHECK(parts >= 1 && parts <= 3 && heads >= 1 && heads <= 64, "split_heads_rownorm: parts must be in 1 .. 3 and heads in 1 .. 64");
    TORCH_CHECK((x.dim() == 2 || x.dim() == 3) && x.stride(-1) == 1 && x.size(-1) >= parts * heads * 128,
                "split_heads_rownorm: x must be [B, n, >= parts*heads*128] or [n, >= parts*heads*128] with a contiguous last dim");
    TORCH_CHECK(norm_mask >= 0 && rope_mask >= 0 && (norm_mask >> parts) == 0 && (rope_mask >> parts) == 0, "split_heads_rownorm: a mask names a part past parts");
    const int64_t B = x.dim() == 3 ? x.size(0) : 1, n = x.size(-2), C = heads * 128;
    TORCH_CHECK(B >= 1, "split_heads_rownorm: empty batch");
    const c10::optional<at::Tensor> *ws[3] = {&w0, &w1, &w2};
    at::Tensor wc[3];
    const void *wp[3] = {nullptr, nullptr, nullptr};
    int wd[3] = {0, 0, 0};
    for (int p = 0; p < 3; ++p) {
        if (!(ws[p]->has_value() && (*ws[p])->defined())) continue;
        TORCH_CHECK(p < parts && (norm_mask >> p & 1), "split_heads_rownorm: weight ", p, " belongs to a part that is not normalised");
        wc[p] = (*ws[p])->contiguous();
        CHECK_DEV(wc[p]);
        TORCH_CHECK((wc[p].scalar_type() == at::kBFloat16 || wc[p].scalar_type() == at::kFloat) && wc[p].numel() == C,
                    "split_heads_rownorm: a weight must be bfloat16 or float32 with heads*128 entries");
        wp[p] = wc[p].data_ptr(), wd[p] = wc[p].scalar_type() == at::kFloat ? 2 : 1;
    }
    const float *fc = nullptr, *fs = nullptr;
    int64_t rope_rows = 0;
    at::Tensor fcc, fsc;
    const bool has_cos = freqs_cos.has_value() && freqs_cos->defined(), has_sin = freqs_sin.has_value() && freqs_sin->defined();
    TORCH_CHECK(has_cos == has_sin, "split_heads_rownorm: freqs_cos and freqs_sin come together");
    TORCH_CHECK(rope_mask == 0 || has_cos, "split_heads_rownorm: a rotated part needs freqs_cos / freqs_sin");
    if (has_cos) {
        fcc = freqs_cos->contiguous(), fsc = freqs_sin->contiguous();
        CHECK_DEV(fcc); CHECK_DEV(fsc);
        TORCH_CHECK(fcc.scalar_type() == at::kFloat && fsc.scalar_type() == at::kFloat && fcc.dim() == 2 && fcc.size(1) == 128 &&
                    fsc.sizes() == fcc.sizes() && fcc.size(0) <= n, "split_heads_rownorm: freqs must be float32 [rows <= n, 128]");
        fc = fcc.data_ptr<float>(), fs = fsc.data_ptr<float>(), rope_rows = fcc.size(0);
    }
    c10::DeviceGuard guard(x.device());
    at::Tensor out = at::empty({parts, B, heads, n, 128}, x.options());
    void *op[3] = {nullptr, nullptr, nullptr};
    std::vector<at::Tensor> res;
    for (int p = 0; p < parts; ++p) res.push_back(out[p]), op[p] = res.back().data_ptr();
    if (n == 0) return res;
    check(chipmunk_split_heads_rownorm(x.data_ptr(), x.dim() == 3 ? x.stride(0) : 0, x.stride(-2), (int)parts, wp[0], wd[0], wp[1], wd[1], wp[2],
                                       wd[2], op[0], op[1], op[2], (unsigned)norm_mask, (unsigned)rope_mask, B, n, (int)heads, (float)eps, fc,
                                       fs, rope_rows, cur_stream(x)),
          "split_heads_rownorm");
    return res;
}

at::Tensor gather_rows(at::Tensor src, at::Tensor map) {
    CHECK_DEV(src);
    CHECK_DEV(map);
    TORCH_CHECK(src.dim() >= 2, "gather_rows: src must be [..., n, d]");
    TORCH_CHECK(map.scalar_type() == at::kInt && map.dim() == 1 && map.is_contiguous(), "gather_rows: map must be a contiguous int32 vector");
    src = src.contiguous();
    const int64_t n_src = src.size(-2), d = src.size(-1), n_out = map.numel();
    const int64_t outer = n_src * d == 0 ? 0 : src.numel() / (n_src * d);
    auto sizes = src.sizes().vec();
    sizes[sizes.size() - 2] = n_out;
    c10::DeviceGuard guard(src.device());
    at::Tensor dst = at::empty(sizes, src.options());
    if (dst.numel() == 0) return dst;
    check(chipmunk_gather_rows(src.data_ptr(), dst.data_ptr(), map.data_ptr<int>(), outer, n_src, n_out,
                               d * (int64_t)src.element_size(), cur_stream(src)),
          "gather_rows");
    return dst;
}

}

TORCH_LIBRARY(chipmunk, m) {
    m.def("csp_mlp_mm1(Tensor a, Tensor b_colmajor, Tensor(c!) c, Tensor bias, Tensor pa_cache_colmajor, Tensor indices, Tensor indices_counts) -> ()");
    m.def("csp_mlp_mm2_and_scatter_add(Tensor packed, Tensor(unpacked_colmajor!) unpacked_colmajor, Tensor sp_inds, Tensor sp_counts, Tensor mma_a, Tensor mma_b, Tensor mma_c, int num_sms_scatter_add, int matmul_kernel) -> ()");

    m.def("csp_attn(Tensor q, Tensor k, Tensor v, Tensor o, Tensor indices, Tensor indices_counts, int o_scale) -> ()");
    m.def("csp_128_attn(Tensor q, Tensor k, Tensor v, Tensor indices, Tensor indices_counts) -> Tensor");
    m.def("dense_attn(Tensor q, Tensor k, Tensor v) -> Tensor[]");
    m.def("dense_colsum_attn(Tensor q, Tensor k, Tensor v, Tensor p) -> Tensor[]");

    m.def("copy_indices(Tensor bmfc1, Tensor(bm_mid_cache!) bm_mid_cache, Tensor sp_inds, Tensor sp_counts) -> ()");
    m.def("topk_indices(Tensor activation, Tensor(indices!) indices, Tensor counts, float sparsity_amount, int multiple_of, float random_amount) -> ()");
    m.def("csp_scatter_add(Tensor packed, Tensor(unpacked_colmajor!) unpacked_colmajor, Tensor sp_inds, Tensor sp_counts, int num_sms) -> ()");
    m.def("mask_to_indices(Tensor mask, int multiple_of, int pad_to_multiple_of) -> Tensor[]");

    m.def("csp_attn_out(Tensor q, Tensor k, Tensor v, Tensor o_in, Tensor indices, Tensor indices_counts, int o_scale) -> Tensor");
    m.def("csp_mlp_mm1_scatter(Tensor a, Tensor b_colmajor, Tensor(c!) c, Tensor bias, Tensor(pa_cache_colmajor!) pa_cache_colmajor, Tensor indices, Tensor indices_counts) -> ()");
    m.def("csp_mlp_mm2(Tensor mma_a, Tensor mma_b, Tensor indices, Tensor counts, Tensor(mma_c!) mma_c) -> ()");
    m.def("csp_mlp_mm1_fp8(Tensor a, Tensor b, Tensor(c!) c, Tensor bias, Tensor(pa_cache_colmajor!) pa_cache_colmajor, Tensor indices, Tensor indices_counts, Tensor scale_a, Tensor scale_b, bool update_cache) -> ()");
    m.def("csp_mlp_mm1_fp8_scatter(Tensor a, Tensor b, Tensor(c!) c, Tensor bias, Tensor(pa_cache_colmajor!) pa_cache_colmajor, Tensor indices, Tensor indices_counts, Tensor scale_a, Tensor scale_b) -> ()");
    m.def("csp_mlp_mm1_glu(Tensor a, Tensor b_gate, Tensor b_up, Tensor(c!) c, Tensor? bias_gate, Tensor? bias_up, Tensor(pa_cache_colmajor!) pa_cache_colmajor, Tensor indices, Tensor indices_counts, str act, bool update_cache) -> ()");
    m.def("csp_mlp_mm1_glu_fp8(Tensor a, Tensor b_gate, Tensor b_up, Tensor(c!) c, Tensor? bias_gate, Tensor? bias_up, Tensor(pa_cache_colmajor!) pa_cache_colmajor, Tensor indices, Tensor indices_counts, Tensor scale_a, Tensor scale_b_gate, Tensor scale_b_up, str act, bool update_cache) -> ()");
    m.def("topk_delta_indices(Tensor activation, Tensor(cache!) cache, Tensor(indices!) indices, Tensor(counts!) counts, float sparsity_amount, int multiple_of, float random_amount) -> ()");
    m.def("packed_mask_to_indices(Tensor packed, int[] shape, int multiple_of, int pad_to_multiple_of) -> Tensor[]");
    m.def("mask_to_sorted_indices(Tensor mask, int[] shape, int multiple_of, int pad_to_multiple_of) -> Tensor[]");
    m.def("topk_mask(Tensor cs, int k, float random_amount, Tensor? groups, Tensor? static_mask) -> Tensor");
    m.def("dense_colsum_topk_mask(Tensor q, Tensor k, Tensor v, Tensor p, int k_top, float random_amount, Tensor? groups, Tensor? static_mask, bool token_major_o=False) -> Tensor[]");
    m.def("dense_attn_layout(Tensor q, Tensor k, Tensor v, bool token_major_o) -> Tensor[]");
    m.def("dense_colsum_attn_layout(Tensor q, Tensor k, Tensor v, Tensor p, bool token_major_o) -> Tensor[]");
    m.def("compact_indices(Tensor indices, Tensor counts) -> Tensor[]");
    m.def("mask_to_ragged_indices(Tensor mask, int[] shape, int multiple_of, int pad_to_multiple_of, bool sorted) -> Tensor[]");
    m.def("csp_attn_out_ragged(Tensor q, Tensor k, Tensor v, Tensor o_in, Tensor indices, Tensor offsets, Tensor indices_counts, int o_scale) -> Tensor");
    m.def("residual_ln_modulate(Tensor x, Tensor? y, Tensor? gate, Tensor shift, Tensor scale, float eps) -> Tensor[]");
    m.def("transpose_last2(Tensor x) -> Tensor");
    m.def("transpose_last2_pitched(Tensor x, int ld) -> Tensor");
    m.def("block_mean(Tensor x, int mbm) -> Tensor");
    m.def("quantize_fp8(Tensor x, Tensor scale, float max_value) -> Tensor");
    m.def("bitpack(Tensor mask) -> Tensor");
    m.def("bitunpack(Tensor packed, int[] shape) -> Tensor");
    m.def("gather_rows(Tensor src, Tensor map) -> Tensor");
    m.def("qkv_split_norm(Tensor qkv, Tensor? q_weight, Tensor? k_weight, int heads, float eps, Tensor? freqs_cos=None, Tensor? freqs_sin=None) -> Tensor[]");
    m.def("split_heads_rownorm(Tensor x, int heads, int parts, Tensor? w0, Tensor? w1, Tensor? w2, int norm_mask, int rope_mask, float eps, Tensor? freqs_cos=None, Tensor? freqs_sin=None) -> Tensor[]");
}

TORCH_LIBRARY_IMPL(chipmunk, CUDA, m) {
    m.impl("qkv_split_norm", &qkv_split_norm);
    m.impl("split_heads_rownorm", &split_heads_rownorm);
    m.impl("csp_mlp_mm1_fp8_scatter", &csp_mlp_mm1_fp8_scatter);
    m.impl("dense_colsum_topk_mask", &dense_colsum_topk_mask);
    m.impl("csp_mlp_mm1", &csp_mlp_mm1);
    m.impl("csp_mlp_mm2_and_scatter_add", &csp_mlp_mm2_and_scatter_add);
    m.impl("copy_indices", &copy_indices);
    m.impl("topk_indices", &topk_indices);
    m.impl("csp_scatter_add", &csp_scatter_add);
    m.impl("mask_to_indices", &mask_to_indices);
    m.impl("csp_attn", &csp_attn);
    m.impl("csp_128_attn", &csp_128_attn);
    m.impl("dense_attn", &dense_attn);
    m.impl("dense_colsum_attn", &dense_colsum_attn);
    m.impl("compact_indices", &compact_indices);
    m.impl("residual_ln_modulate", &residual_ln_modulate);
    m.impl("csp_attn_out_ragged", &csp_attn_out_ragged);
    m.impl("dense_attn_layout", &dense_attn_layout);
    m.impl("dense_colsum_attn_layout", &dense_colsum_attn_layout);
    m.impl("csp_attn_out", &csp_attn_out);
    m.impl("csp_mlp_mm1_scatter", &csp_mlp_mm1_scatter);
    m.impl("csp_mlp_mm2", &csp_mlp_mm2);
    m.impl("csp_mlp_mm1_fp8", &csp_mlp_mm1_fp8);
    m.impl("csp_mlp_mm1_glu", &csp_mlp_mm1_glu);
    m.impl("csp_mlp_mm1_glu_fp8", &csp_mlp_mm1_glu_fp8);
    m.impl("topk_delta_indices", &topk_delta_indices);
    m.impl("packed_mask_to_indices", &packed_mask_to_indices);
    m.impl("mask_to_sorted_indices", &mask_to_sorted_indices);
    m.impl("mask_to_ragged_indices", &mask_to_ragged_indices);
    m.impl("topk_mask", &topk_mask);
    m.impl("transpose_last2", &transpose_last2);
    m.impl("transpose_last2_pitched", &transpose_last2_pitched);
    m.impl("block_mean", &block_mean);
    m.impl("quantize_fp8", &quantize_fp8);
    m.impl("bitpack", &bitpack);
    m.impl("bitunpack", &bitunpack);
    m.impl("gather_rows", &gather_rows);
}

}
```

### chipmunk_amd/modules/attn.py

```python
from __future__ import annotations

from typing import Optional, Tuple

import torch
import torch.nn.functional as F
from torch import Tensor, nn

from .. import ops
from ..ops.voxel import get_local_indices_with_text
from ..util.config import GLOBAL_CONFIG, amd_key
from ..util.layer_counter import LayerCounter
from ..util.storage import AttnStorage
from ..util.storage.offloaded_tensor import release_kept_offloaded, release_resident, reserve_kept_offloaded, reserve_resident

singleton_static_mask: Optional[Tensor] = None
singleton_video_query_groups: Optional[Tensor] = None


def _cdiv(a: int, b: int) -> int:
    return (a + b - 1) // b


def _dense_attn_raw(q: Tensor, k: Tensor, v: Tensor, token_major_o: bool):
    return torch.ops.chipmunk.dense_attn_layout(q, k, v, True) if token_major_o else torch.ops.chipmunk.dense_attn(q, k, v)
# ... 32 lines not shown

    def _static(self, heads: int, qg: int, n: int):
        g0 = self.query_group_offset
        assert heads <= singleton_static_mask.shape[1] or singleton_static_mask.shape[1] == 1, (
            f"this module serves {heads} heads but initialize_static_mask() built {singleton_static_mask.shape[1]} head planes "
            "(local_heads_num): build the static mask for the largest head chunk")
        h = min(heads, singleton_static_mask.shape[1])
        return (singleton_static_mask[:, :h, g0:g0 + qg, :n], singleton_video_query_groups[:, :h, g0:g0 + qg, :])

    def random_and_topk(self, cs: Tensor, topk: int) -> Tensor:
        cfg = GLOBAL_CONFIG["attn"]
        qg, n = cs.shape[-2], cs.shape[-1]
        static, groups = self._static(cs.shape[1], qg, n)
        if cs.is_cuda and amd_key("attn", "fused_topk_mask") and cs.dtype == torch.bfloat16 and n <= ops.TOPK_MASK_MAX_N:
            return ops.topk_mask(cs, topk, 0.01, groups, static)
        mask = torch.randint(0, 100, cs.shape, device=cs.device, dtype=torch.uint8) == 0
        mask.scatter_(-1, cs.topk(k=topk, dim=-1).indices, True)
        mask.logical_and_(groups)
        mask.logical_or_(static)
        return mask

    def release_kept_indices(self) -> None:
        for inv, old in enumerate(self._unpacked):
            if old is not None:
                self._release_kept(old)
                self._unpacked[inv] = None

    @staticmethod
    def _release_kept(kept) -> None:
        release_resident(kept[3])
        if kept[4]:
            release_kept_offloaded(kept[3])

    def __del__(self):
        try:
            self.release_kept_indices()
        except Exception:
            pass

    @torch.compiler.disable
    def _remember_indices(self, inds: Optional[Tensor], counts: Tensor, ragged=None) -> None:
        inv = self.layer_counter.cur_model_invocation_per_step
        old, self._unpacked[inv] = self._unpacked[inv], None
        if old is not None:
            self._release_kept(old)
        self.storage.indices.suppress_current(False)
        if not (counts.is_cuda and amd_key("attn", "keep_unpacked_indices") and amd_key("attn", "fused_residual")
                and (self.storage.indices.is_resident() or amd_key("attn", "keep_unpacked_indices_offloaded"))):
            return
        if not reserve_resident(0):
            return
        flat, offsets = ragged if ragged is not None else ops.compact_indices(inds, counts)
        nbytes = 4 * flat.numel() + 8 * offsets.numel() + 4 * counts.numel()
        off_mode = not self.storage.indices.is_resident()
        if off_mode and not reserve_kept_offloaded(nbytes):
            return
        if not reserve_resident(nbytes):
            if off_mode:
                release_kept_offloaded(nbytes)
            return
        self._unpacked[inv] = (flat, offsets, counts, nbytes, off_mode)
        self.storage.indices.suppress_current(off_mode and bool(GLOBAL_CONFIG["attn"]["recompute_mask"]))

    def _kept_indices(self):
        kept = self._unpacked[self.layer_counter.cur_model_invocation_per_step]
        if kept is not None and GLOBAL_CONFIG["attn"]["should_compress_indices"] and (
                self.storage.indices.is_resident() or amd_key("attn", "keep_unpacked_indices_offloaded")):
            return kept[:3]
        return None

    def _stored_mask(self):
        if self.storage.indices.is_suppressed():
            self.storage.indices.suppress_current(False)
            self.storage.indices.load_async()
            self.storage.indices.load_async_wait()
        return self.storage.get_indices(), self.mask_shape[self.layer_counter.cur_model_invocation_per_step]

    @staticmethod
    def _ragged_enabled(x: Tensor) -> bool:
        return bool(x.is_cuda and GLOBAL_CONFIG["attn"]["should_compress_indices"] and amd_key("attn", "fused_residual")
                    and amd_key("attn", "fused_packed_mask_to_indices") and amd_key("attn", "ragged_mask_to_indices"))

    @torch.compiler.disable
    def _ragged_indices(self, packed: Tensor, shape, multiple_of: int, bm: int, mask: Optional[Tensor] = None):
        if shape[-1] % 8 != 0:
            packed = mask if mask is not None else ops.bitunpack(packed, shape)
        return ops.mask_to_ragged_indices(packed, shape, multiple_of, bm, bool(amd_key("attn", "sorted_indices")))

    def _stored_indices(self, multiple_of: int, bm: int):
        cfg = GLOBAL_CONFIG["attn"]
        if cfg["should_compress_indices"]:
            packed, shape = self._stored_mask()
            if amd_key("attn", "fused_packed_mask_to_indices") and packed.is_cuda and shape[-1] % 8 == 0:
                if amd_key("attn", "sorted_indices"):
                    return ops.mask_to_sorted_indices(packed, shape, multiple_of, bm)
                return ops.packed_mask_to_indices(packed, shape, multiple_of, bm)
            return ops.mask_to_indices(ops.bitunpack(packed, shape), multiple_of, bm)
        return self.storage.get_indices(), self.storage.get_counts()

    def _fast_attention(self, q: Tensor, k: Tensor, v: Tensor, inference_step: int, do_full_step: bool) -> Tensor:
        cfg = GLOBAL_CONFIG["attn"]
        bm = cfg["mbm"]
        assert bm == 192, "The kernel was written for BM=192. You may need to change the kernel."
        do_padding = cfg["pad_qkv_before_kernel"]
        multiple_of = 128 if do_padding else cfg["counts_multiple_of"]

        tm = bool(q.is_cuda and amd_key("attn", "token_major_output"))
        use_ragged = self._ragged_enabled(q)
        if self.layer_num < cfg["first_n_dense_layers"]:
            o, _ = ops.dense_attn(q, k, v, tm)
            return o

        if do_full_step:
            if inference_step == 0:
                o, lse = ops.dense_attn(q, k, v, tm) if do_padding else _dense_attn_raw(q, k, v, tm)
                lse[..., k.shape[-2]:, :] = 0
                self.storage.set_lse_constants(lse)
                return o

            ragged = None
            if inference_step == 1 or cfg["recompute_mask"]:
                prev_lse = self.storage.get_lse_constants()
                tk = int(multiple_of * round((cfg["top_keys"] * k.shape[-2]) / multiple_of))
                mask = bs = None
                if (q.is_cuda and cfg["should_compress_indices"] and tk > 0 and amd_key("attn", "fused_colsum_topk")
                        and amd_key("attn", "fused_topk_mask") and k.shape[-2] <= ops.TOPK_MASK_MAX_N):
                    static, groups = self._static(q.shape[1], _cdiv(q.shape[-2], bm), k.shape[-2])
                    o, mask, lse = ops.dense_colsum_topk_mask(q, k, v, prev_lse, tk, 0.01, groups, static, tm)
                elif do_padding:
                    o, bs, lse = ops.dense_colsum_attn(q, k, v, prev_lse, tm)
                else:
                    o, bs, lse = (torch.ops.chipmunk.dense_colsum_attn_layout(q, k, v, prev_lse, True) if tm else
                                  torch.ops.chipmunk.dense_colsum_attn(q, k, v, prev_lse))
                lse[..., k.shape[-2]:, :] = 0
                self.storage.set_lse_constants(lse)
                if cfg["should_compress_indices"]:
                    if mask is not None:
                        pass
                    elif tk > 0:
                        mask = self.random_and_topk(bs, tk)
                    else:
                        mask = self._static(bs.shape[1], bs.shape[-2], bs.shape[-1])[0]
                    packed, mask_shape = ops.bitpack(mask)
                    self.mask_shape[self.layer_counter.cur_model_invocation_per_step] = mask_shape
                    self.storage.set_indices(packed)
                    if use_ragged:
                        ragged = self._ragged_indices(packed, mask_shape, multiple_of, bm, mask)
                        self._remember_indices(None, ragged[2], ragged[:2])
                    else:
                        if mask.is_cuda and amd_key("attn", "fused_packed_mask_to_indices") and amd_key("attn", "sorted_indices"):
                            inds, counts = ops.mask_to_sorted_indices(mask, mask.shape, multiple_of, bm)
                        else:
                            inds, counts = ops.mask_to_indices(mask, multiple_of, bm)
                        self._remember_indices(inds, counts)
                else:
                    kseq = k.shape[-2]
                    bs = bs[..., :_cdiv(kseq, bm), :kseq]
                    inds = torch.topk(bs, k=tk, dim=-1).indices
                    counts = torch.full((q.shape[0], q.shape[1], _cdiv(q.shape[-2], bm)), tk, device=q.device,
                                        dtype=torch.int32)
                    pad = torch.empty((*counts.shape, q.shape[-2] - tk), device=q.device, dtype=torch.int32)
                    inds = torch.cat([inds, pad], dim=-1).to(torch.int32)
                    self.storage.set_indices(inds)
                    self.storage.set_counts(counts)
            else:
                o, _ = ops.dense_attn(q, k, v, tm)

            if use_ragged:
                if ragged is None:
                    ragged = self._ragged_indices(*self._stored_mask(), multiple_of, bm)
            elif not (inference_step == 1 or cfg["recompute_mask"]):
                inds, counts = self._stored_indices(multiple_of, bm)

            if ragged is not None:
                o_cache = ops.csp_attn_out_ragged(q, k, v, o, ragged[0], ragged[1], ragged[2], -1)
            elif o.is_cuda and amd_key("attn", "fused_residual"):
                o_cache = ops.csp_attn_out(q, k, v, o, inds, counts, -1)
            elif do_padding:
                o_cache = o - ops.csp_attn(q, k, v, inds, counts)
            else:
                o_cache = o.clone()
                ops.csp_attn_inplace(q, k, v, o_cache, inds, counts, -1)
            self.storage.set_out_cache(o_cache)
            return o

        o = self.storage.get_out_cache()
        kept = self._kept_indices() if (o.is_cuda and amd_key("attn", "fused_residual")) else None
        if kept is not None:
            return ops.csp_attn_out_ragged(q, k, v, o, kept[0], kept[1], kept[2], 1)
        if use_ragged:
            flat, offsets, counts = self._ragged_indices(*self._stored_mask(), multiple_of, bm)
            return ops.csp_attn_out_ragged(q, k, v, o, flat, offsets, counts, 1)
        inds, counts = self._stored_indices(multiple_of, bm)
        if do_padding:
            if o.is_cuda and amd_key("attn", "fused_residual"):
                return ops.csp_attn_out(q, k, v, o, inds, counts, 1)
            return o + ops.csp_attn(q, k, v, inds, counts)
        persistent = self.storage.out_cache.is_resident()
        if o.is_cuda and amd_key("attn", "fused_residual") and persistent:
            return ops.csp_attn_out(q, k, v, o, inds, counts, 1)
        if persistent:
            o = o.clone()
        ops.csp_attn_inplace(q, k, v, o, inds, counts, 1)
        return o

    def forward(self, q: Tensor, k: Tensor, v: Tensor) -> Tensor:
        if not GLOBAL_CONFIG["attn"]["is_enabled"]:
            return F.scaled_dot_product_attention(q, k, v)
        do_full_step = self.layer_counter.should_do_full_attn_step()
        out = self._fast_attention(q, k, v, self.layer_counter.cur_inference_step, do_full_step)
        self.layer_counter.increment()
        return out

    def __call__(self, *args, **kwargs):
        return self.forward(*args, **kwargs)
```

### chipmunk_amd/ops/__init__.py

```python
from .mlp import run_e2e as mlp
from .mlp import run_e2e_glu as mlp_glu, run_e2e_glu, mm1_glu
from .mlp import run_e2e_glu_fp8 as mlp_glu_fp8, run_e2e_glu_fp8, mm1_glu_fp8
from .indexed_io import (copy_indices, topk_indices, mask_to_indices, scatter_add, packed_mask_to_indices,
                         mask_to_sorted_indices, mask_to_ragged_indices, topk_mask, manual_seed, TOPK_MASK_MAX_N)
from .attn import compact_indices, csp_attn, csp_attn_inplace, csp_attn_out, csp_attn_out_ragged, dense_attn, dense_colsum_attn, dense_colsum_topk_mask
from .patch import patchify, unpatchify, patchify_rope
from .bitpack import bitpack, bitunpack
from . import voxel
from .qkv import qkv_split_norm, residual_ln_modulate, split_heads_rownorm, wan_rope_table

__all__ = ["mlp", "copy_indices", "topk_indices", "mask_to_indices", "scatter_add", "csp_attn", "dense_attn",
           "dense_colsum_attn", "patchify", "unpatchify", "patchify_rope", "bitpack", "bitunpack",
           "packed_mask_to_indices", "mask_to_sorted_indices", "csp_attn_inplace", "csp_attn_out", "topk_mask", "TOPK_MASK_MAX_N", "voxel", "manual_seed", "qkv_split_norm", "dense_colsum_topk_mask", "compact_indices", "csp_attn_out_ragged", "residual_ln_modulate",
           "split_heads_rownorm", "wan_rope_table", "mask_to_ragged_indices", "mlp_glu", "run_e2e_glu", "mm1_glu",
           "mlp_glu_fp8", "run_e2e_glu_fp8", "mm1_glu_fp8"]

from . import _fake
```

### chipmunk_amd/ops/_fake.py

```python
import torch


def _o_like(q, token_major):
    B, H, N, D = q.shape
    return q.new_empty((B, N, H, D)).permute(0, 2, 1, 3) if token_major else q.new_empty((B, H, N, D))


def _register():
    lib = torch.library

    @lib.register_fake("chipmunk::csp_128_attn")
    def _(q, k, v, indices, indices_counts):
        return torch.empty_like(q)

    @lib.register_fake("chipmunk::csp_attn_out")
    def _(q, k, v, o_in, indices, indices_counts, o_scale):
        return torch.empty_like(o_in)

    @lib.register_fake("chipmunk::residual_ln_modulate")
    def _(x, y, gate, shift, scale, eps):
        return [torch.empty_like(x), torch.empty_like(x)] if y is not None else [torch.empty_like(x)]

    @lib.register_fake("chipmunk::csp_attn_out_ragged")
    def _(q, k, v, o_in, indices, offsets, indices_counts, o_scale):
        return torch.empty_like(o_in)

    @lib.register_fake("chipmunk::dense_attn")
    def _(q, k, v):
        return [_o_like(q, False), q.new_empty((q.shape[0], q.shape[1], q.shape[2], 1), dtype=torch.float32)]

    @lib.register_fake("chipmunk::dense_attn_layout")
    def _(q, k, v, token_major_o):
        return [_o_like(q, token_major_o), q.new_empty((q.shape[0], q.shape[1], q.shape[2], 1), dtype=torch.float32)]

    @lib.register_fake("chipmunk::dense_colsum_attn_layout")
    def _(q, k, v, p, token_major_o):
        groups = (q.shape[2] + 191) // 192
        return [_o_like(q, token_major_o),
                q.new_empty((q.shape[0], q.shape[1], groups, max(q.shape[2], k.shape[2]))),
                q.new_empty((q.shape[0], q.shape[1], q.shape[2], 1), dtype=torch.float32)]

    @lib.register_fake("chipmunk::dense_colsum_attn")
    def _(q, k, v, p):
        groups = (q.shape[2] + 191) // 192
        return [_o_like(q, False),
                q.new_empty((q.shape[0], q.shape[1], groups, max(q.shape[2], k.shape[2]))),
                q.new_empty((q.shape[0], q.shape[1], q.shape[2], 1), dtype=torch.float32)]

    @lib.register_fake("chipmunk::mask_to_indices")
    def _(mask, multiple_of, pad_to_multiple_of):
        b, h, m, n = mask.shape
        pad_n = (n + pad_to_multiple_of - 1) // pad_to_multiple_of * pad_to_multiple_of
        return [mask.new_empty((b, h, m, pad_n), dtype=torch.int32), mask.new_empty((b, h, m), dtype=torch.int32)]

    @lib.register_fake("chipmunk::packed_mask_to_indices")
    def _(packed, shape, multiple_of, pad_to_multiple_of):
        b, h, m, n = shape
        pad_n = (n + pad_to_multiple_of - 1) // pad_to_multiple_of * pad_to_multiple_of
        return [packed.new_empty((b, h, m, pad_n), dtype=torch.int32), packed.new_empty((b, h, m), dtype=torch.int32)]

    @lib.register_fake("chipmunk::topk_mask")
    def _(cs, k, random_amount, groups, static_mask):
        return cs.new_empty(cs.shape, dtype=torch.bool)

    @lib.register_fake("chipmunk::block_mean")
    def _(x, mbm):
        return x.new_empty((x.shape[0], (x.shape[1] + mbm - 1) // mbm, x.shape[2]))

    @lib.register_fake("chipmunk::transpose_last2")
    def _(x):
        return x.new_empty(x.shape[:-2] + (x.shape[-1], x.shape[-2]))

    @lib.register_fake("chipmunk::transpose_last2_pitched")
    def _(x, ld):
        return x.new_empty(x.shape[:-2] + (x.shape[-1], ld))

    @lib.register_fake("chipmunk::quantize_fp8")
    def _(x, scale, max_value):
        return x.new_empty(x.shape, dtype=torch.float8_e4m3fn)

    @lib.register_fake("chipmunk::bitpack")
    def _(mask):
        return mask.new_empty(((mask.numel() + 7) // 8,), dtype=torch.uint8)

    @lib.register_fake("chipmunk::bitunpack")
    def _(packed, shape):
        return packed.new_empty(tuple(shape), dtype=torch.bool)

    @lib.register_fake("chipmunk::gather_rows")
    def _(src, map):
        shape = list(src.shape)
        shape[-2] = map.shape[0]
        return src.new_empty(shape)

    @lib.register_fake("chipmunk::dense_colsum_topk_mask")
    def _(q, k, v, p, k_top, random_amount, groups, static_mask, token_major_o=False):
        B, H, Nq, D = q.shape
        G = (Nq + 191) // 192
        return [_o_like(q, token_major_o), q.new_empty((B, H, G, k.shape[2]), dtype=torch.bool),
                q.new_empty((B, H, Nq, 1), dtype=torch.float32)]

    @lib.register_fake("chipmunk::qkv_split_norm")
    def _(qkv, q_weight, k_weight, heads, eps, freqs_cos=None, freqs_sin=None):
        out = qkv.new_empty((3, 1, heads, qkv.shape[0], 128))
        return [out[0], out[1], out[2]]

    @lib.register_fake("chipmunk::split_heads_rownorm")
    def _(x, heads, parts, w0, w1, w2, norm_mask, rope_mask, eps, freqs_cos=None, freqs_sin=None):
        out = x.new_empty((parts, x.shape[0] if x.dim() == 3 else 1, heads, x.shape[-2], 128))
        return [out[p] for p in range(parts)]

    @lib.register_fake("chipmunk::csp_mlp_mm1_glu")
    def _(a, b_gate, b_up, c, bias_gate, bias_up, pa_cache_colmajor, indices, indices_counts, act, update_cache):
        torch._check(a.shape[-1] == b_gate.shape[1] and b_gate.shape == b_up.shape, lambda: "a, b_gate and b_up must share K; b_up the shape of b_gate")
        torch._check(c.shape == a.shape[:-1] + (b_gate.shape[0],), lambda: "c must be [M, F] ([B, M, F] with the batch size of a)")
        torch._check(act in ("gelu_tanh", "silu", "gelu"), lambda: f"csp_mlp_mm1_glu: unknown activation '{act}'")
        return None

    @lib.register_fake("chipmunk::csp_mlp_mm1_glu_fp8")
    def _(a, b_gate, b_up, c, bias_gate, bias_up, pa_cache_colmajor, indices, indices_counts, scale_a, scale_b_gate, scale_b_up, act,
          update_cache):
        f8 = torch.float8_e4m3fn
        torch._check(a.dtype == f8 and b_gate.dtype == f8 and b_up.dtype == f8, lambda: "a, b_gate and b_up must be float8_e4m3fn")
        torch._check(c.dtype == torch.bfloat16 and pa_cache_colmajor.dtype == torch.bfloat16, lambda: "c and pa_cache_colmajor must be bfloat16")
        torch._check(a.shape[-1] == b_gate.shape[1] and b_gate.shape == b_up.shape, lambda: "a, b_gate and b_up must share K; b_up the shape of b_gate")
        torch._check(c.shape == a.shape[:-1] + (b_gate.shape[0],), lambda: "c must be [M, F] ([B, M, F] with the batch size of a)")
        for s in (scale_a, scale_b_gate, scale_b_up):
            torch._check(s.dtype == torch.float32 and s.numel() == 1, lambda: "scale_a, scale_b_gate and scale_b_up must be one-element float32 tensors")
        torch._check(act in ("gelu_tanh", "silu", "gelu"), lambda: f"csp_mlp_mm1_glu_fp8: unknown activation '{act}'")
        return None


_register()
```

### chipmunk_amd/ops/attn.py

```python
from __future__ import annotations

from typing import Tuple

import torch
import torch.nn.functional as F

PM = 192


def _pad_len(n: int) -> int:
    return ((n + PM - 1) // PM) * PM


def _last_dim_contiguous(t: torch.Tensor) -> torch.Tensor:
    return t if t.stride(-1) == 1 else t.contiguous()


def dense_attn(q: torch.Tensor, k: torch.Tensor, v: torch.Tensor, token_major_o: bool = False) -> Tuple[torch.Tensor, torch.Tensor]:
    n = q.shape[-2]
    q, k, v = _last_dim_contiguous(q), _last_dim_contiguous(k), _last_dim_contiguous(v)
    o, l = torch.ops.chipmunk.dense_attn_layout(q, k, v, True) if token_major_o else torch.ops.chipmunk.dense_attn(q, k, v)
    padded = _pad_len(n)
    if padded != n:
        l = F.pad(l, (0, 0, 0, padded - n))
    return o, l


def dense_colsum_attn(q: torch.Tensor, k: torch.Tensor, v: torch.Tensor, p: torch.Tensor, token_major_o: bool = False
                      ) -> Tuple[torch.Tensor, torch.Tensor, torch.Tensor]:
    n = q.shape[-2]
    padded = _pad_len(n)
    assert p.shape[-2] in (n, padded), "p must be the l vector of the previous full step"
    p_rows = p[..., :n, :].contiguous()
    q, k, v = _last_dim_contiguous(q), _last_dim_contiguous(k), _last_dim_contiguous(v)
    if token_major_o:
        o, cs, l = torch.ops.chipmunk.dense_colsum_attn_layout(q, k, v, p_rows, True)
    else:
        o, cs, l = torch.ops.chipmunk.dense_colsum_attn(q, k, v, p_rows)
    if padded != n:
        l = F.pad(l, (0, 0, 0, padded - n))
    kseq = k.shape[-2]
    kgroups = (kseq + PM - 1) // PM
    if cs.shape[-2] != kgroups or cs.shape[-1] != kseq:
        cs = cs[..., :kgroups, :kseq]
    return o, cs, l


def dense_colsum_topk_mask(q: torch.Tensor, k: torch.Tensor, v: torch.Tensor, p: torch.Tensor, k_top: int, random_amount: float,
                           groups, static_mask, token_major_o: bool = False) -> Tuple[torch.Tensor, torch.Tensor, torch.Tensor]:
    n = q.shape[-2]
    padded = _pad_len(n)
    assert p.shape[-2] in (n, padded), "p must be the l vector of the previous full step"
    o, mask, l = torch.ops.chipmunk.dense_colsum_topk_mask(_last_dim_contiguous(q), _last_dim_contiguous(k), _last_dim_contiguous(v),
                                                           p[..., :n, :].contiguous(), k_top, random_amount, groups, static_mask,
                                                           token_major_o)
    if padded != n:
        l = F.pad(l, (0, 0, 0, padded - n))
    return o, mask, l


def csp_attn(q: torch.Tensor, k: torch.Tensor, v: torch.Tensor, indices: torch.Tensor,
             indices_counts: torch.Tensor) -> torch.Tensor:
    return torch.ops.chipmunk.csp_128_attn(q.contiguous(), k.contiguous(), v.contiguous(), indices.contiguous(),
                                           indices_counts.contiguous())


def csp_attn_inplace(q: torch.Tensor, k: torch.Tensor, v: torch.Tensor, o: torch.Tensor, indices: torch.Tensor,
                     indices_counts: torch.Tensor, o_scale: int) -> None:
    torch.ops.chipmunk.csp_attn(q, k, v, o, indices, indices_counts, o_scale)


def csp_attn_out(q: torch.Tensor, k: torch.Tensor, v: torch.Tensor, o_in: torch.Tensor, indices: torch.Tensor,
                 indices_counts: torch.Tensor, o_scale: int) -> torch.Tensor:
    return torch.ops.chipmunk.csp_attn_out(q, k, v, o_in, indices, indices_counts, o_scale)


def compact_indices(indices: torch.Tensor, indices_counts: torch.Tensor) -> Tuple[torch.Tensor, torch.Tensor]:
    return tuple(torch.ops.chipmunk.compact_indices(indices.contiguous(), indices_counts.contiguous()))


def csp_attn_out_ragged(q: torch.Tensor, k: torch.Tensor, v: torch.Tensor, o_in: torch.Tensor, indices: torch.Tensor,
                        offsets: torch.Tensor, indices_counts: torch.Tensor, o_scale: int) -> torch.Tensor:
    return torch.ops.chipmunk.csp_attn_out_ragged(q, k, v, o_in, indices, offsets, indices_counts, o_scale)


__all__ = ["csp_attn", "csp_attn_inplace", "csp_attn_out", "csp_attn_out_ragged", "compact_indices", "dense_attn", "dense_colsum_attn",
           "dense_colsum_topk_mask"]
```

### chipmunk_amd/ops/indexed_io.py

```python
from __future__ import annotations

from typing import List, Optional, Sequence

import torch

TOPK_MASK_MAX_N = 1024 * 512


def copy_indices(bm_fc1: torch.Tensor, bm_mid_cache: torch.Tensor, indices: torch.Tensor, counts: torch.Tensor) -> None:
    torch.ops.chipmunk.copy_indices(bm_fc1, bm_mid_cache, indices, counts)


def topk_indices(activations: torch.Tensor, indices_out: torch.Tensor, counts_out: torch.Tensor,
                 sparsity_amount: float, multiple_of: int, rk: float) -> None:
    torch.ops.chipmunk.topk_indices(activations, indices_out, counts_out, sparsity_amount, multiple_of, rk)


def scatter_add(packed: torch.Tensor, unpacked: torch.Tensor, indices: torch.Tensor, counts: torch.Tensor,
                num_sms: int) -> None:
    if packed.ndim == 3:
        torch.ops.chipmunk.csp_scatter_add(packed, unpacked, indices, counts, num_sms)
        return
    torch.ops.chipmunk.csp_scatter_add(packed.unsqueeze(0), unpacked.unsqueeze(0), indices.unsqueeze(0),
                                       counts.unsqueeze(0), num_sms)


def mask_to_indices(mask: torch.Tensor, multiple_of: int, pad_to_multiple_of: int) -> List[torch.Tensor]:
    return torch.ops.chipmunk.mask_to_indices(mask, multiple_of, pad_to_multiple_of)


def packed_mask_to_indices(packed: torch.Tensor, shape: Sequence[int], multiple_of: int,
                           pad_to_multiple_of: int) -> List[torch.Tensor]:
    return torch.ops.chipmunk.packed_mask_to_indices(packed, list(shape), multiple_of, pad_to_multiple_of)


def mask_to_sorted_indices(mask: torch.Tensor, shape: Sequence[int], multiple_of: int,
                           pad_to_multiple_of: int) -> List[torch.Tensor]:
    return torch.ops.chipmunk.mask_to_sorted_indices(mask, list(shape), multiple_of, pad_to_multiple_of)


def mask_to_ragged_indices(mask: torch.Tensor, shape: Sequence[int], multiple_of: int, pad_to_multiple_of: int,
                           sorted: bool = True) -> List[torch.Tensor]:
    if mask.is_cuda:
        return torch.ops.chipmunk.mask_to_ragged_indices(mask, list(shape), multiple_of, pad_to_multiple_of, sorted)
    if mask.dtype == torch.uint8:
        from .bitpack import bitunpack
        mask = bitunpack(mask, shape)
    b, h, m, n = mask.shape
    pad_n = (n + pad_to_multiple_of - 1) // pad_to_multiple_of * pad_to_multiple_of
    rows = mask.reshape(-1, n) != 0
    kept = rows.sum(dim=1)
    counts = (kept + multiple_of - 1) // multiple_of * multiple_of
    lengths = (counts.clamp(max=pad_n) + 31) // 32 * 32
    offsets = torch.zeros(rows.shape[0] + 1, dtype=torch.int64)
    offsets[1:] = lengths.cumsum(0)
    flat = torch.zeros(int(offsets[-1]) + 64, dtype=torch.int32)
    cols = torch.arange(n, dtype=torch.int32)
    for r in range(rows.shape[0]):
        true = cols[rows[r]]
        if not sorted:
            true = true[torch.argsort(true % 32, stable=True)]
        row = torch.cat([true, cols[~rows[r]][:int(counts[r] - kept[r])]])
        flat[int(offsets[r]):int(offsets[r]) + row.numel()] = row
    return [flat, offsets, counts.to(torch.int32).view(b, h, m)]


def topk_mask(cs: torch.Tensor, k: int, random_amount: float = 0.0, groups: Optional[torch.Tensor] = None,
              static_mask: Optional[torch.Tensor] = None) -> torch.Tensor:
    return torch.ops.chipmunk.topk_mask(cs, k, random_amount, groups, static_mask)


def manual_seed(seed: int) -> None:
    from .._native import manual_seed as _seed
    _seed(seed)
```

### chipmunk_amd/util/config.py

```python
from __future__ import annotations

import copy
from typing import Any, Dict

import yaml

BASE_CONFIG: Dict[str, Any] = {
    "num_model_invocations_per_inference_step": 1,
    "should_profile": False,
    "generation_index": 0,
    "steps": 50,
    "world_size": 1,
    "mlp": {
        "is_enabled": True,
        "is_fp8": False,
        "top_keys": "dd",
        "random_keys": 0.05,
        "full_step_every": 10,
        "block_mask_cache": 2,
        "first_n_dense_layers": 2,
        "counts_multiple_of": 256,
        "bm": 128,
        "mbm": 128,
    },
    "patchify": {
        "is_enabled": True,
        "chunk_size_1": 8,
        "chunk_size_2": 4,
    },
    "attn": {
        "is_enabled": True,
        "top_keys": 0.05,
        "random_keys": 0.01,
        "local_voxels": 0,
        "local_1d_window": 0,
        "first_n_dense_layers": 2,
        "full_step_every": 10,
        "full_step_schedule": None,
        "recompute_mask": True,
        "should_compress_indices": True,
        "counts_multiple_of": 128,
        "pad_qkv_before_kernel": True,
        "mbm": 192,
    },
    "offloading": {
        "global_disable_offloading": False,
        "mlp.out_cache": False,
        "mlp.indices": False,
        "mlp.counts": False,
        "mlp.sparse_act_T": False,
        "mlp.blockmean_mid_cache": False,
        "attn.out_cache": True,
        "attn.indices": True,
        "attn.counts": False,
        "attn.lse_constants": False,
        "text_encoders": True,
    },
    "step_caching": {
        "is_enabled": True,
        "skip_step_schedule": {7, 11, 13, 14, 15, 17, 18, 19, 21, 22, 23, 25, 26, 27, 29, 31, 33, 34, 35, 37, 38, 39,
                               41, 42, 43},
    },
}

AMD_EXTRA_KEYS: Dict[str, Any] = {
    "offloading.keep_resident_if_fits": False,
    "offloading.hbm_budget_gb": 200.0,
    "offloading.native_host_pool": True,
    "attn.fused_packed_mask_to_indices": True,
    "attn.sorted_indices": True,
    "mlp.fused_topk_delta": True,
    "mlp.fused_block_mean": True,
    "mlp.fused_fp8_quantize": True,
    "attn.fused_residual": True,
    "attn.fused_topk_mask": True,
    "attn.fused_colsum_topk": True,
    "mlp.fused_scatter": True,
    "attn.token_major_output": False,
    "attn.keep_unpacked_indices": True,
    "attn.keep_unpacked_indices_offloaded": True,
    "attn.kept_indices_offloaded_budget_gb": 8.0,
    "attn.ragged_mask_to_indices": True,
}
BASE_CONFIG["offloading"]["keep_resident_if_fits"] = AMD_EXTRA_KEYS["offloading.keep_resident_if_fits"]
BASE_CONFIG["offloading"]["hbm_budget_gb"] = AMD_EXTRA_KEYS["offloading.hbm_budget_gb"]
BASE_CONFIG["offloading"]["native_host_pool"] = AMD_EXTRA_KEYS["offloading.native_host_pool"]
BASE_CONFIG["attn"]["fused_packed_mask_to_indices"] = AMD_EXTRA_KEYS["attn.fused_packed_mask_to_indices"]
BASE_CONFIG["attn"]["sorted_indices"] = AMD_EXTRA_KEYS["attn.sorted_indices"]
BASE_CONFIG["mlp"]["fused_topk_delta"] = AMD_EXTRA_KEYS["mlp.fused_topk_delta"]
BASE_CONFIG["attn"]["fused_residual"] = AMD_EXTRA_KEYS["attn.fused_residual"]
BASE_CONFIG["attn"]["fused_topk_mask"] = AMD_EXTRA_KEYS["attn.fused_topk_mask"]
BASE_CONFIG["attn"]["fused_colsum_topk"] = AMD_EXTRA_KEYS["attn.fused_colsum_topk"]
BASE_CONFIG["mlp"]["fused_scatter"] = AMD_EXTRA_KEYS["mlp.fused_scatter"]
BASE_CONFIG["attn"]["token_major_output"] = AMD_EXTRA_KEYS["attn.token_major_output"]
BASE_CONFIG["attn"]["keep_unpacked_indices"] = AMD_EXTRA_KEYS["attn.keep_unpacked_indices"]
BASE_CONFIG["attn"]["keep_unpacked_indices_offloaded"] = AMD_EXTRA_KEYS["attn.keep_unpacked_indices_offloaded"]
BASE_CONFIG["attn"]["kept_indices_offloaded_budget_gb"] = AMD_EXTRA_KEYS["attn.kept_indices_offloaded_budget_gb"]
BASE_CONFIG["attn"]["ragged_mask_to_indices"] = AMD_EXTRA_KEYS["attn.ragged_mask_to_indices"]

GLOBAL_CONFIG: Dict[str, Any] = copy.deepcopy(BASE_CONFIG)


def amd_key(section: str, key: str) -> Any:
    return GLOBAL_CONFIG.get(section, {}).get(key, AMD_EXTRA_KEYS[f"{section}.{key}"])


def update_global_config(config: Dict[str, Any]) -> None:
    GLOBAL_CONFIG.update(config)


def _deep_update(dst: Dict[str, Any], src: Dict[str, Any]) -> None:
    for key, value in src.items():
        if isinstance(value, dict) and isinstance(dst.get(key), dict):
            _deep_update(dst[key], value)
        else:
            dst[key] = value


def load_from_file(config_file: str) -> None:
    with open(config_file, "r") as f:
        loaded = yaml.safe_load(f)
    if loaded:
        _deep_update(GLOBAL_CONFIG, loaded)
        print(f"CHIPMUNK: using config file {config_file}")


def reset_to_base() -> None:
    fresh = copy.deepcopy(BASE_CONFIG)
    GLOBAL_CONFIG.clear()
    GLOBAL_CONFIG.update(fresh)
```

### include/chipmunk_hip.h

```cpp
#ifndef CHIPMUNK_HIP_H
#define CHIPMUNK_HIP_H

#include <stdint.h>

#ifdef __cplusplus
extern "C" {
#endif

#define CHIPMUNK_OK 0
#define CHIPMUNK_ERR_INVALID 1
#define CHIPMUNK_ERR_LAUNCH 2
#define CHIPMUNK_ERR_UNSUPPORTED 3

#define CHIPMUNK_DTYPE_BF16 0
#define CHIPMUNK_DTYPE_FP16 1
#define CHIPMUNK_DTYPE_FP32 2

const char *chipmunk_last_error(void);
int chipmunk_abi_version(void);
int chipmunk_set_option(const char *name, int value);
int chipmunk_set_random_seed(uint64_t seed);

int chipmunk_csp_attn(const void *q, const void *k, const void *v, void *o, const int64_t q_strides[3],
                      const int64_t k_strides[3], const int64_t v_strides[3], const int64_t o_strides[3],
// ... 51 lines not shown

int chipmunk_csp_mlp_mm2_and_scatter_add(const void *packed, void *unpacked_colmajor, const int32_t *indices,
                                         const int32_t *counts, const void *mma_a, const void *mma_b, void *mma_c,
                                         int M, int F, int N2, int num_sms_scatter_add, void *stream);

int chipmunk_csp_scatter_add(const void *packed, void *unpacked_colmajor, const int32_t *indices,
                             const int32_t *counts, int M, int F, int num_sms, void *stream);

int chipmunk_csp_mlp_mm2(const void *mma_a, const void *mma_b, void *mma_c, const int32_t *indices,
                         const int32_t *counts, int M, int F, int N2, void *stream);

int chipmunk_csp_mlp_mm1_ragged(const void *a, const void *b, void *c, const void *bias, const void *pa_cache,
                                const int32_t *indices, const int32_t *counts, int M, int K, int F, int ldc, void *stream);
int chipmunk_csp_mlp_mm1_scatter_ragged(const void *a, const void *b, void *c, const void *bias, void *pa_cache,
                                        const int32_t *indices, const int32_t *counts, int M, int K, int F, int ldc,
                                        void *stream);
int chipmunk_csp_mlp_mm1_fp8_ragged(const void *a, const void *b, void *c, const void *bias, void *pa_cache,
                                    const int32_t *indices, const int32_t *counts, const float *scale_a,
                                    const float *scale_b, int M, int K, int F, int ldc, int update_cache, void *stream);
int chipmunk_csp_mlp_mm2_ragged(const void *mma_a, const void *mma_b, void *mma_c, const int32_t *indices,
                                const int32_t *counts, int M, int F, int N2, void *stream);
int chipmunk_csp_mlp_mm2_and_scatter_add_ragged(const void *packed, void *unpacked_colmajor, const int32_t *indices,
                                                const int32_t *counts, const void *mma_a, const void *mma_b, void *mma_c,
                                                int M, int F, int N2, int ldc, void *stream);
int chipmunk_csp_scatter_add_ragged(const void *packed, void *unpacked_colmajor, const int32_t *indices,
                                    const int32_t *counts, int M, int F, int ldc, void *stream);

int chipmunk_csp_mlp_mm1_batched(const void *a, const void *b, void *c, const void *bias, const void *pa_cache,
                                 const int32_t *indices, const int32_t *counts, int M, int K, int F, int ldc, int B,
                                 int64_t cache_batch_stride, void *stream);
int chipmunk_csp_mlp_mm1_scatter_batched(const void *a, const void *b, void *c, const void *bias, void *pa_cache,
                                         const int32_t *indices, const int32_t *counts, int M, int K, int F, int ldc, int B,
                                         int64_t cache_batch_stride, void *stream);
int chipmunk_csp_mlp_mm1_fp8_batched(const void *a, const void *b, void *c, const void *bias, void *pa_cache,
                                     const int32_t *indices, const int32_t *counts, const float *scale_a, const float *scale_b,
                                     int M, int K, int F, int ldc, int update_cache, int B, int64_t cache_batch_stride,
                                     void *stream);
int chipmunk_csp_mlp_mm2_batched(const void *mma_a, const void *mma_b, void *mma_c, const int32_t *indices,
                                 const int32_t *counts, int M, int F, int N2, int B, void *stream);
int chipmunk_csp_mlp_mm2_and_scatter_add_batched(const void *packed, void *unpacked_colmajor, const int32_t *indices,
                                                 const int32_t *counts, const void *mma_a, const void *mma_b, void *mma_c,
                                                 int M, int F, int N2, int ldc, int B, int64_t cache_batch_stride,
                                                 void *stream);
int chipmunk_csp_scatter_add_batched(const void *packed, void *unpacked_colmajor, const int32_t *indices,
                                     const int32_t *counts, int M, int F, int ldc, int B, int64_t cache_batch_stride,
                                     void *stream);

#define CHIPMUNK_ACT_GELU_TANH 0
#define CHIPMUNK_ACT_SILU 1
#define CHIPMUNK_ACT_GELU_ERF 2
int chipmunk_csp_mlp_mm1_glu(const void *a, const void *b_gate, const void *b_up, void *c, const void *bias_gate,
                             const void *bias_up, void *pa_cache, const int32_t *indices, const int32_t *counts, int M, int K,
                             int F, int ldc, int act, int update_cache, void *stream);
int chipmunk_csp_mlp_mm1_glu_batched(const void *a, const void *b_gate, const void *b_up, void *c, const void *bias_gate,
                                     const void *bias_up, void *pa_cache, const int32_t *indices, const int32_t *counts, int M,
                                     int K, int F, int ldc, int act, int update_cache, int B, int64_t cache_batch_stride,
                                     void *stream);
int chipmunk_csp_mlp_mm1_glu_fp8(const void *a, const void *b_gate, const void *b_up, void *c, const void *bias_gate,
                                 const void *bias_up, void *pa_cache, const int32_t *indices, const int32_t *counts,
                                 const float *scale_a, const float *scale_b_gate, const float *scale_b_up, int M, int K, int F,
                                 int ldc, int act, int update_cache, void *stream);
int chipmunk_csp_mlp_mm1_glu_fp8_batched(const void *a, const void *b_gate, const void *b_up, void *c, const void *bias_gate,
                                         const void *bias_up, void *pa_cache, const int32_t *indices, const int32_t *counts,
                                         const float *scale_a, const float *scale_b_gate, const float *scale_b_up, int M, int K,
                                         int F, int ldc, int act, int update_cache, int B, int64_t cache_batch_stride,
                                         void *stream);

int chipmunk_topk_indices(const void *activation, int dtype, int32_t *indices, int32_t *counts, int rows, int cols,
                          double sparsity_amount, int multiple_of, double random_amount, void *stream);

int chipmunk_topk_delta_indices(const void *activation, void *cache, int dtype, int32_t *indices, int32_t *counts,
                                int rows, int cols, double sparsity_amount, int multiple_of, double random_amount,
                                void *stream);

int chipmunk_dense_colsum_topk_mask(const void *q, const void *k, const void *v, const int64_t q_strides[3],
                                    const int64_t k_strides[3], const int64_t v_strides[3], const float *p, void *o, float *l,
                                    int B, int H, int Nq, int Nk, const void *static_mask, int64_t static_stride, int static_rows,
                                    const void *group_flags, void *mask, int k_top, double random_amount, void *stream);

int chipmunk_topk_mask(const void *cs, int64_t cs_stride, const void *static_mask, int64_t static_stride,
                       int static_rows, const void *group_flags, void *mask, int rows, int n, int k,
                       double random_amount, void *stream);

int chipmunk_mask_to_indices(const void *mask, int32_t *indices, int32_t *counts, int64_t rows, int n, int pad_n,
                             int multiple_of, void *stream);

int chipmunk_packed_mask_to_indices(const void *packed, int32_t *indices, int32_t *counts, int64_t rows, int n,
                                    int pad_n, int multiple_of, void *stream);

int chipmunk_mask_to_sorted_indices(const void *mask, int packed, int32_t *indices, int32_t *counts, int64_t rows,
                                    int n, int pad_n, int multiple_of, void *stream);

int chipmunk_mask_row_counts(const void *mask, int packed, int32_t *counts, int64_t *lengths, int64_t rows, int n, int pad_n,
                             int multiple_of, void *stream);
int chipmunk_mask_to_ragged_indices(const void *mask, int packed, int sorted, const int64_t *offsets, int32_t *flat, int64_t rows,
                                    int n, int multiple_of, void *stream);

int chipmunk_copy_indices(const void *src, void *dst, const int32_t *inds, const int32_t *counts, int B, int M, int R,
                          int F, int elem_size, void *stream);

int chipmunk_transpose16(const void *src, void *dst, int B, int R, int C, void *stream);
int chipmunk_transpose16_pitched(const void *src, void *dst, int B, int R, int C, int ld, void *stream);

int chipmunk_block_mean(const void *x, void *out, int64_t rows, int C, int mbm, void *stream);
int chipmunk_block_mean_ragged(const void *x, void *out, int64_t rows, int C, int mbm, void *stream);

int chipmunk_quantize_fp8(const void *x, const float *scale, void *out, int64_t n, float max_value, void *stream);

int chipmunk_bitpack(const void *mask, void *packed, int64_t n, void *stream);
int chipmunk_bitunpack(const void *packed, void *mask, int64_t n, void *stream);

int chipmunk_gather_rows(const void *src, void *dst, const int32_t *map, int64_t outer, int64_t n_src, int64_t n_out,
                         int64_t row_bytes, void *stream);

int chipmunk_host_alloc(size_t bytes, void **host_ptr);
int chipmunk_host_free(void *host_ptr);
int chipmunk_copy_d2h_async(void *host_dst, const void *dev_src, size_t bytes, void *stream);
int chipmunk_copy_h2d_async(void *dev_dst, const void *host_src, size_t bytes, void *stream);
size_t chipmunk_host_bytes(void);

int chipmunk_release_scratch(void);
int chipmunk_big_scratch_fallbacks(void);

int chipmunk_qkv_split_norm(const void *qkv, int64_t row_stride, const void *q_weight, const void *k_weight, void *q, void *k,
                            void *v, int64_t n, int heads, float eps, const float *freqs_cos, const float *freqs_sin,
                            int64_t rope_rows, void *stream);

int chipmunk_split_heads_rownorm(const void *x, int64_t batch_stride, int64_t row_stride, int parts, const void *w0, int w0_dtype,
                                 const void *w1, int w1_dtype, const void *w2, int w2_dtype, void *out0, void *out1, void *out2,
                                 unsigned norm_mask, unsigned rope_mask, int64_t B, int64_t n, int heads, float eps,
                                 const float *freqs_cos, const float *freqs_sin, int64_t rope_rows, void *stream);

#ifdef __cplusplus
}
#endif
#endif
```

Before: 0.5810.

## Fuse packed mask and padded counts into topk selection kernel

Adds a topk select kernel that, while thresholding column sums, directly emits the bit-packed mask and per-row padded counts, plus an _ex variant of the fused dense colsum+topk path that can skip the byte mask. This removes the separate bitpack and mask row-count passes, and the unpacked byte mask write, in the attention sparsity update step. It adds new output plumbing through the C API, torch ops and config, and the tie-breaking logic has to match the previous kernel.

```diff
diff --git a/chipmunk_amd/_native.py b/chipmunk_amd/_native.py
--- a/chipmunk_amd/_native.py
+++ b/chipmunk_amd/_native.py
@@ -17,6 +17,7 @@
     "chipmunk_csp_mlp_mm1_glu", "chipmunk_csp_mlp_mm1_glu_batched", "chipmunk_csp_mlp_mm1_glu_fp8", "chipmunk_csp_mlp_mm1_glu_fp8_batched",
     "chipmunk_topk_indices", "chipmunk_topk_delta_indices", "chipmunk_topk_mask", "chipmunk_mask_to_indices", "chipmunk_mask_to_sorted_indices", "chipmunk_packed_mask_to_indices", "chipmunk_mask_row_counts", "chipmunk_mask_to_ragged_indices", "chipmunk_copy_indices",
     "chipmunk_bitpack", "chipmunk_bitunpack", "chipmunk_transpose16", "chipmunk_block_mean", "chipmunk_quantize_fp8", "chipmunk_gather_rows", "chipmunk_qkv_split_norm", "chipmunk_split_heads_rownorm", "chipmunk_dense_colsum_topk_mask", "chipmunk_dense_attn_strided", "chipmunk_csp_attn_out_ragged", "chipmunk_compact_indices", "chipmunk_residual_ln_modulate", "chipmunk_dense_colsum_attn_strided", "chipmunk_dense_colsum_topk_mask_strided", "chipmunk_release_scratch", "chipmunk_big_scratch_fallbacks",
+    "chipmunk_topk_mask_ex", "chipmunk_topk_select_fused", "chipmunk_dense_colsum_topk_mask_ex",
     "chipmunk_host_alloc", "chipmunk_host_free", "chipmunk_copy_d2h_async", "chipmunk_copy_h2d_async", "chipmunk_host_bytes",
 ]
 
diff --git a/chipmunk_amd/csrc/attn.hip b/chipmunk_amd/csrc/attn.hip
--- a/chipmunk_amd/csrc/attn.hip
+++ b/chipmunk_amd/csrc/attn.hip
@@ -1238,19 +1238,22 @@
                                               cs_stride, stream);
 }
 
-extern "C" int chipmunk_dense_colsum_topk_mask_strided(const void *q, const void *k, const void *v, const int64_t q_strides[3],
+extern "C" int chipmunk_dense_colsum_topk_mask_ex(const void *q, const void *k, const void *v, const int64_t q_strides[3],
                                                const int64_t k_strides[3], const int64_t v_strides[3], const float *pin, void *o,
                                                const int64_t *o_strides, float *l, int B, int H, int Nq, int Nk, const void *static_mask,
-                                               int64_t static_stride, int static_rows, const void *group_flags, void *mask,
-                                               int topk, double random_amount, void *stream) {
+                                               int64_t static_stride, int static_rows, const void *group_flags, void *mask, void *packed,
+                                               int32_t *counts, int multiple_of, int topk, double random_amount, void *stream) {
     if (int e = check_common(q, k, v, o, B, H, Nq, Nk)) return e;
-    CM_CHECK(l && pin && mask, "dense_colsum_topk_mask: p / l / mask missing");
+    CM_CHECK(l && pin && (mask || packed), "dense_colsum_topk_mask: p / l / mask missing");
+    CM_CHECK(!packed || Nk % 8 == 0, "dense_colsum_topk_mask: the packed output needs Nk %% 8 == 0 (got %d)", Nk);
+    CM_CHECK(!counts || multiple_of > 0, "dense_colsum_topk_mask: counts need a positive multiple_of (got %d)", multiple_of);
     if (int e = check_strides(q_strides, "q")) return e;
     if (int e = check_strides(k_strides, "k")) return e;
     if (int e = check_strides(v_strides, "v")) return e;
     hipStream_t st = (hipStream_t)stream;
     if (!use_dense64(B, H, Nq, Nk) || chipmunk_get_option("attn_fused_colsum") == 2 || (Nk & 3) || Nk > CHIPMUNK_TOPK_MASK_MAX_N)
         return CHIPMUNK_ERR_UNSUPPORTED;
+    if (!mask && !chipmunk_topk_select_fused(Nk)) return CHIPMUNK_ERR_UNSUPPORTED;
     AttnParams p = {};
     p.q = (const uint16_t *)q, p.k = (const uint16_t *)k, p.v = (const uint16_t *)v, p.o = (uint16_t *)o;
     for (int i = 0; i < 3; ++i) p.qs[i] = q_strides[i], p.ks[i] = k_strides[i], p.vs[i] = v_strides[i];
@@ -1264,8 +1267,18 @@
     if (!part) return CHIPMUNK_ERR_UNSUPPORTED;
     if (int e = chipmunk_dense64_colsum_launch(p, part, st)) return e;
     const int nrb = ((Nq + 255) / 256) * 2;
-    return chipmunk_topk_mask_parts(part, chipmunk_colsum_part_stride(Nk), nrb, p.G, Nq, static_mask, static_stride, static_rows, group_flags, mask, B * H * p.G, Nk,
-                                    topk, random_amount, st);
+    return chipmunk_topk_mask_parts_ex(part, chipmunk_colsum_part_stride(Nk), nrb, p.G, Nq, static_mask, static_stride, static_rows, group_flags, mask,
+                                       packed, counts, multiple_of, B * H * p.G, Nk, topk, random_amount, st);
+}
+
+extern "C" int chipmunk_dense_colsum_topk_mask_strided(const void *q, const void *k, const void *v, const int64_t q_strides[3],
+                                               const int64_t k_strides[3], const int64_t v_strides[3], const float *pin, void *o,
+                                               const int64_t *o_strides, float *l, int B, int H, int Nq, int Nk, const void *static_mask,
+                                               int64_t static_stride, int static_rows, const void *group_flags, void *mask,
+                                               int topk, double random_amount, void *stream) {
+    CM_CHECK(mask, "dense_colsum_topk_mask: p / l / mask missing");
+    return chipmunk_dense_colsum_topk_mask_ex(q, k, v, q_strides, k_strides, v_strides, pin, o, o_strides, l, B, H, Nq, Nk, static_mask,
+                                              static_stride, static_rows, group_flags, mask, nullptr, nullptr, 0, topk, random_amount, stream);
 }
 
 extern "C" int chipmunk_dense_colsum_topk_mask(const void *q, const void *k, const void *v, const int64_t q_strides[3],
diff --git a/chipmunk_amd/csrc/attn_params.h b/chipmunk_amd/csrc/attn_params.h
--- a/chipmunk_amd/csrc/attn_params.h
+++ b/chipmunk_amd/csrc/attn_params.h
@@ -32,6 +32,9 @@
 int chipmunk_topk_mask_parts(const uint16_t *part, int part_stride, int nrb, int groups_per_bh, int Nq, const void *static_mask, int64_t static_stride,
                              int static_rows, const void *group_flags, void *mask, int rows, int n, int k, double random_amount,
                              hipStream_t stream);
+int chipmunk_topk_mask_parts_ex(const uint16_t *part, int part_stride, int nrb, int groups_per_bh, int Nq, const void *static_mask,
+                                int64_t static_stride, int static_rows, const void *group_flags, void *mask, void *packed, int32_t *counts,
+                                int multiple_of, int rows, int n, int k, double random_amount, hipStream_t stream);
 size_t chipmunk_colsum_part_bytes(int B, int H, int Nq, int Nk);
 int chipmunk_colsum_part_stride(int Nk);
 int chipmunk_colsum64_launch(const AttnParams &p, hipStream_t stream);
diff --git a/chipmunk_amd/csrc/capi.hip b/chipmunk_amd/csrc/capi.hip
--- a/chipmunk_amd/csrc/capi.hip
+++ b/chipmunk_amd/csrc/capi.hip
@@ -15,7 +15,8 @@
 #include <string.h>
 namespace {
 struct Option { const char *name; int value; };
-Option g_options[] = {{"mm1_variant", 0}, {"mm2_variant", 0}, {"attn_variant", 0}, {"m2i_variant", 0}, {"topk_variant", 0}, {"mm1_nr", 0}, {"mm2_nr", 0}, {"mm1_probe", 0}, {"attn_xcd_chunks", 0}, {"attn_no_order", 0}, {"attn_no_tail", 0}, {"mm1_no_split", 0}, {"mm2_no_split", 0}, {"attn_no_split", 0}, {"attn_split_gather", 0}, {"attn_pp", 0}, {"attn_dense64", 0}, {"attn_csp64", 0}, {"attn_colsum64", 0}, {"attn_csp96", 0}, {"attn_nomax", 0}, {"attn_fused_colsum", 0}, {"attn_cs_probe", 0}, {"big_scratch_gb", 0}, {"attn_balanced", 0}, {"attn_row_split", 0}, {"mm2_order", 0}, {"topk_mask_stream", 0}};
+Option g_options[] = {{"mm1_variant", 0}, {"mm2_variant", 0}, {"attn_variant", 0}, {"m2i_variant", 0}, {"topk_variant", 0}, {"mm1_nr", 0}, {"mm2_nr", 0}, {"mm1_probe", 0}, {"attn_xcd_chunks", 0}, {"attn_no_order", 0}, {"attn_no_tail", 0}, {"mm1_no_split", 0}, {"mm2_no_split", 0}, {"attn_no_split", 0}, {"attn_split_gather", 0}, {"attn_pp", 0}, {"attn_dense64", 0}, {"attn_csp64", 0}, {"attn_colsum64", 0}, {"attn_csp96", 0}, {"attn_nomax", 0}, {"attn_fused_colsum", 0}, {"attn_cs_probe", 0}, {"big_scratch_gb", 0}, {"attn_balanced", 0}, {"attn_row_split", 0}, {"mm2_order", 0}, {"topk_mask_stream", 0},
+                      {"topk_mask_select", 1}};
 }
 int chipmunk_get_option(const char *name) {
     for (auto &o : g_options) if (strcmp(o.name, name) == 0) return o.value;
diff --git a/chipmunk_amd/csrc/indexed_io.hip b/chipmunk_amd/csrc/indexed_io.hip
--- a/chipmunk_amd/csrc/indexed_io.hip
+++ b/chipmunk_amd/csrc/indexed_io.hip
@@ -242,7 +242,7 @@
     if (lane == 0) {
         const int64_t padded = ((kept + p.multiple_of - 1) / p.multiple_of) * p.multiple_of;
         p.counts[row] = (int32_t)padded;
-        p.lengths[row] = (min(padded, (int64_t)p.pad_n) + 31) / 32 * 32;
+        if (p.lengths) p.lengths[row] = (min(padded, (int64_t)p.pad_n) + 31) / 32 * 32;
     }
 }
 
@@ -561,6 +561,9 @@
     const uint16_t *parts;
     int64_t pstride;
     int nrb, ngroups, nq;
+    uint8_t *packed;
+    int32_t *counts;
+    int multiple_of;
 };
 
 __device__ __forceinline__ uint32_t bf16_key(uint32_t u) {
@@ -1001,6 +1004,222 @@
                 for (int e = 0; e < 4; ++e)
                     if (c + e < n) out[c + e] = (uint8_t)(bytes >> (8 * e));
             }
+        }
+    }
+}
+
+template <int KPT, bool PARTS>
+__global__ __launch_bounds__(1024) void topk_select_kernel(const TopkMaskParams p) {
+    constexpr int NV = KPT / 4;
+    __shared__ int wave_cnt[2][16];
+    __shared__ int wave_tie[16];
+    __shared__ uint32_t wave_lo[16], wave_hi[16];
+    const int tid = threadIdx.x, lane = tid & 63, w = tid >> 6;
+    const int row = blockIdx.x;
+    const int n = p.n;
+    const uint16_t *x = nullptr;
+    int prow = 1;
+    int64_t row1 = 0;
+    if constexpr (PARTS) {
+        const int bh = row / p.ngroups, g = row - bh * p.ngroups;
+        int r0, r1;
+        prow = colsum_part_rows(g, p.nrb / 2, r0, r1);
+        x = p.parts + ((int64_t)bh * p.nrb + r0) * p.pstride;
+        row1 = (int64_t)(r1 - r0) * p.pstride;
+    } else {
+        x = p.cs + (int64_t)row * p.cs_stride;
+    }
+    const uint32_t lane_off8 = 8u * (uint32_t)tid;
+    uint32_t key[NV][2];
+    constexpr int LB = NV % 10 == 0 ? 10 : (NV % 8 == 0 ? 8 : (NV % 6 == 0 ? 6 : 4));
+    static_assert(NV % LB == 0, "NV must split into whole load batches");
+#pragma unroll
+    for (int j0 = 0; j0 < NV; j0 += LB) {
+        uint32_t raw[LB][2];
+#pragma unroll
+        for (int jj = 0; jj < LB; ++jj) {
+            const int c = 4 * tid + 4096 * (j0 + jj);
+            uint32_t v0 = 0xffffffffu, v1 = 0xffffffffu;
+            if (c < n) {
+                const u32x2 v = *(const u32x2 *)((const unsigned char *)(x + 4096 * (j0 + jj)) + lane_off8);
+                v0 = v[0], v1 = v[1];
+                if constexpr (PARTS) {
+                    if (prow == 2) {
+                        float a0 = __uint_as_float(v0 << 16), a1 = __uint_as_float(v0 & 0xffff0000u);
+                        float a2 = __uint_as_float(v1 << 16), a3 = __uint_as_float(v1 & 0xffff0000u);
+                        const u32x2 y = *(const u32x2 *)((const unsigned char *)(x + row1 + 4096 * (j0 + jj)) + lane_off8);
+                        a0 += __uint_as_float(y[0] << 16), a1 += __uint_as_float(y[0] & 0xffff0000u);
+                        a2 += __uint_as_float(y[1] << 16), a3 += __uint_as_float(y[1] & 0xffff0000u);
+                        v0 = pack_bf16x2(a0, a1), v1 = pack_bf16x2(a2, a3);
+                    }
+                }
+            }
+            raw[jj][0] = v0, raw[jj][1] = v1;
+        }
+#pragma unroll
+        for (int jj = 0; jj < LB; ++jj) {
+            const uint32_t k0 = bf16_key2(raw[jj][0]), k1 = bf16_key2(raw[jj][1]);
+            key[j0 + jj][0] = k0, key[j0 + jj][1] = k1;
+        }
+        __builtin_amdgcn_sched_barrier(0);
+    }
+    const bool active = p.groups == nullptr || p.groups[row] != 0;
+    const int k = p.k < n ? p.k : n;
+    uint32_t thr = 0x10000u;
+    int ties_to_take = 0;
+    if (active && k > 0) {
+        uint32_t lo2 = 0xffffffffu, hi2 = 0u;
+        int tid_b = tid;
+        asm volatile("" : "+v"(tid_b));
+#pragma unroll
+        for (int j = 0; j < NV; ++j) {
+            uint32_t pm;
+            asm volatile("v_pk_max_u16 %0, %1, %2" : "=v"(pm) : "v"(key[j][0]), "v"(key[j][1]));
+            asm volatile("v_pk_max_u16 %0, %1, %2" : "=v"(hi2) : "v"(hi2), "v"(pm));
+            const uint32_t pmr = 4 * tid_b + 4096 * j < n ? pm : 0xffffffffu;
+            asm volatile("v_pk_min_u16 %0, %1, %2" : "=v"(lo2) : "v"(lo2), "v"(pmr));
+        }
+        uint32_t lo = min(lo2 & 0xffffu, lo2 >> 16), hi = max(hi2 & 0xffffu, hi2 >> 16);
+#pragma unroll
+        for (int d = 32; d > 0; d >>= 1) {
+            lo = min(lo, (uint32_t)__shfl_xor((int)lo, d));
+            hi = max(hi, (uint32_t)__shfl_xor((int)hi, d));
+        }
+        if (lane == 0) wave_lo[w] = lo, wave_hi[w] = hi;
+        __syncthreads();
+#pragma unroll
+        for (int i = 0; i < 16; ++i) lo = min(lo, wave_lo[i]), hi = max(hi, wave_hi[i]);
+        if (2 * k > n) lo = 0;
+        int above = 0, buf = 0;
+        while (lo < hi) {
+            const uint32_t cand = (lo + hi + 1u) >> 1;
+            const uint32_t cm1 = (cand - 1u) | ((cand - 1u) << 16);
+            const uint32_t one2 = 0x00010001u;
+            uint32_t cnt2 = 0;
+#pragma unroll
+            for (int j = 0; j < NV; ++j)
+#pragma unroll
+                for (int h = 0; h < 2; ++h) {
+                    uint32_t d;
+                    asm volatile("v_pk_sub_u16 %0, %1, %2 clamp\n\tv_pk_min_u16 %0, %0, %3" : "=&v"(d) : "v"(key[j][h]), "v"(cm1), "v"(one2));
+                    asm volatile("v_pk_add_u16 %0, %0, %1" : "+v"(cnt2) : "v"(d));
+                }
+            int t = (int)(cnt2 & 0xffffu) + (int)(cnt2 >> 16);
+#pragma unroll
+            for (int d = 32; d > 0; d >>= 1) t += __shfl_xor(t, d);
+            if (lane == 0) wave_cnt[buf][w] = t;
+            __syncthreads();
+            t = 0;
+#pragma unroll
+            for (int i = 0; i < 16; ++i) t += wave_cnt[buf][i];
+            buf ^= 1;
+            if (t >= k) lo = cand;
+            else hi = cand - 1u, above = t;
+        }
+        thr = lo;
+        ties_to_take = k - above;
+    }
+    int my_ties = 0;
+    if (ties_to_take > 0) {
+        const uint32_t t2 = thr | (thr << 16), one2 = 0x00010001u;
+        uint32_t ne2 = 0;
+#pragma unroll
+        for (int j = 0; j < NV; ++j)
+#pragma unroll
+            for (int h = 0; h < 2; ++h) {
+                uint32_t d = key[j][h] ^ t2;
+                asm volatile("v_pk_min_u16 %0, %0, %1" : "+v"(d) : "v"(one2));
+                asm volatile("v_pk_add_u16 %0, %0, %1" : "+v"(ne2) : "v"(d));
+            }
+        my_ties = 4 * NV - (int)(ne2 & 0xffffu) - (int)(ne2 >> 16);
+    }
+    int tie_budget = 0;
+    {
+        int incl = my_ties;
+#pragma unroll
+        for (int d = 1; d < 64; d <<= 1) {
+            const int o = __shfl_up(incl, d);
+            if (lane >= d) incl += o;
+        }
+        if (lane == 63) wave_tie[w] = incl;
+        __syncthreads();
+        int before = incl - my_ties;
+#pragma unroll
+        for (int i = 0; i < 16; ++i) before += i < w ? wave_tie[i] : 0;
+        tie_budget = ties_to_take - before;
+    }
+    uint8_t *out = p.mask ? p.mask + (int64_t)row * n : nullptr;
+    uint8_t *outp = p.packed ? p.packed + (((int64_t)row * n) >> 3) : nullptr;
+    const uint8_t *st = p.stat ? p.stat + (int64_t)(row % p.stat_rows) * p.stat_stride : nullptr;
+    const bool rnd = active && p.random_amount > 0.f;
+    uint32_t first = x[0];
+    if constexpr (PARTS) {
+        float a0 = __uint_as_float(first << 16);
+        if (prow == 2) a0 += __uint_as_float((uint32_t)x[row1] << 16);
+        first = pack_bf16x2(a0, 0.f) & 0xffffu;
+    }
+    const uint32_t salt = p.salt ^ (first * 0x27D4EB2Fu);
+    const uint32_t hrow = (uint32_t)row * 0x9E3779B9u, hsalt = salt * 0xC2B2AE35u;
+    const uint32_t hcol = (4u * (uint32_t)tid + 0x7F4A7C15u) * 0x85EBCA6Bu;
+    const uint32_t hthr = rnd ? (uint32_t)__builtin_ceilf(p.random_amount * 16777216.0f) : 0u;
+    int kept = 0;
+    int tid_o = tid;
+    asm volatile("" : "+v"(tid_o));
+    constexpr int OB = 5;
+#pragma unroll
+    for (int j0 = 0; j0 < NV; j0 += OB) {
+        uint32_t sbv[OB];
+#pragma unroll
+        for (int jj = 0; jj < OB; ++jj) {
+            const int c = 4 * tid_o + 4096 * (j0 + jj);
+            sbv[jj] = (j0 + jj < NV && st && c < n) ? *(const uint32_t *)(st + c) : 0u;
+        }
+        __builtin_amdgcn_sched_barrier(0);
+#pragma unroll
+        for (int jj = 0; jj < OB; ++jj) {
+            if constexpr (true) {
+                if (j0 + jj < NV) {
+                    const int j = j0 + jj < NV ? j0 + jj : 0;
+                    const int c = 4 * tid_o + 4096 * j;
+                    const bool real = c < n;
+                    uint32_t v0 = key[j][0], v1 = key[j][1];
+                    asm volatile("" : "+v"(v0), "+v"(v1));
+                    uint32_t nib = 0;
+#pragma unroll
+                    for (int e = 0; e < 4; ++e) {
+                        const uint32_t kv = ((e < 2 ? v0 : v1) >> (16 * (e & 1))) & 0xffffu;
+                        bool keep = kv > thr;
+                        const bool tie = kv == thr && tie_budget > 0 && real;
+                        tie_budget -= tie ? 1 : 0;
+                        keep = keep || tie;
+                        uint32_t hx = (hrow ^ (hcol + (uint32_t)(4096 * j + e) * 0x85EBCA6Bu)) + hsalt;
+                        hx ^= hx >> 16, hx *= 0x7feb352du, hx ^= hx >> 15, hx *= 0x846ca68bu, hx ^= hx >> 16;
+                        keep = keep || (hx >> 8) < hthr;
+                        keep = keep || ((sbv[jj] >> (8 * e)) & 0xffu) != 0;
+                        nib |= (keep && real ? 1u : 0u) << e;
+                    }
+                    kept += __popc(nib);
+                    if (out && real) *(uint32_t *)(out + c) = (nib | (nib << 7) | (nib << 14) | (nib << 21)) & 0x01010101u;
+                    if (outp) {
+                        const uint32_t other = (uint32_t)__shfl_xor((int)nib, 1);
+                        if (!(tid & 1) && real) outp[c >> 3] = (uint8_t)(nib | (other << 4));
+                    }
+                    asm volatile("" ::: "memory");
+                }
+            }
+        }
+        __builtin_amdgcn_sched_barrier(0);
+    }
+    if (p.counts) {
+#pragma unroll
+        for (int d = 32; d > 0; d >>= 1) kept += __shfl_xor(kept, d);
+        if (lane == 0) wave_cnt[0][w] = kept;
+        __syncthreads();
+        if (tid == 0) {
+            int64_t total = 0;
+#pragma unroll
+            for (int i = 0; i < 16; ++i) total += wave_cnt[0][i];
+            p.counts[row] = (int32_t)((total + p.multiple_of - 1) / p.multiple_of * p.multiple_of);
         }
     }
 }
@@ -1182,24 +1401,70 @@
     return CHIPMUNK_OK;
 }
 
-int chipmunk_topk_mask_parts(const uint16_t *part, int part_stride, int nrb, int groups_per_bh, int Nq, const void *static_mask, int64_t static_stride,
-                             int static_rows, const void *group_flags, void *mask, int rows, int n, int k, double random_amount,
-                             hipStream_t s) {
-    CM_CHECK(part && mask && rows >= 0 && n > 0 && (n & 3) == 0 && n <= CHIPMUNK_TOPK_MASK_MAX_N && k >= 0 && part_stride >= n && (part_stride & 3) == 0, "topk_mask_parts: bad arguments");
+static bool topk_select_takes(int n) {
+    return n <= 1024 * 120 && chipmunk_get_option("topk_mask_select") != 0 && chipmunk_get_option("topk_mask_stream") != 1;
+}
+extern "C" int chipmunk_topk_select_fused(int n) { return n > 0 && n % 4 == 0 && topk_select_takes(n) ? 1 : 0; }
+
+template <bool PARTS>
+static void launch_topk_select(const TopkMaskParams &p, hipStream_t s) {
+    if (p.n <= 1024 * 16) hipLaunchKernelGGL((topk_select_kernel<16, PARTS>), dim3(p.rows), dim3(1024), 0, s, p);
+    else if (p.n <= 1024 * 48) hipLaunchKernelGGL((topk_select_kernel<48, PARTS>), dim3(p.rows), dim3(1024), 0, s, p);
+    else hipLaunchKernelGGL((topk_select_kernel<120, PARTS>), dim3(p.rows), dim3(1024), 0, s, p);
+}
+
+static int check_select_outputs(const char *what, const void *mask, const void *packed, const int32_t *counts, int multiple_of, int n) {
+    CM_CHECK(mask || packed, "%s: null pointer (a mask or a packed mask is needed)", what);
+    CM_CHECK(!packed || n % 8 == 0, "%s: the packed output needs n %% 8 == 0 (got %d)", what, n);
+    CM_CHECK(!counts || multiple_of > 0, "%s: counts need a positive multiple_of (got %d)", what, multiple_of);
+    return CHIPMUNK_OK;
+}
+static int select_outputs_from_mask(const void *mask, void *packed, int32_t *counts, int multiple_of, int rows, int n, hipStream_t s) {
+    if (packed)
+        if (int e = chipmunk_bitpack(mask, packed, (int64_t)rows * n, s)) return e;
+    if (counts) {
+        RowCountParams rp = {(const uint8_t *)mask, counts, nullptr, rows, n, n, multiple_of};
+        hipLaunchKernelGGL(mask_row_counts_kernel<false>, dim3((unsigned)((rows + 3) / 4)), dim3(256), 0, s, rp);
+        CM_LAUNCH_CHECK();
+    }
+    return CHIPMUNK_OK;
+}
+
+int chipmunk_topk_mask_parts_ex(const uint16_t *part, int part_stride, int nrb, int groups_per_bh, int Nq, const void *static_mask,
+                                int64_t static_stride, int static_rows, const void *group_flags, void *mask, void *packed, int32_t *counts,
+                                int multiple_of, int rows, int n, int k, double random_amount, hipStream_t s) {
+    CM_CHECK(part && rows >= 0 && n > 0 && (n & 3) == 0 && n <= CHIPMUNK_TOPK_MASK_MAX_N && k >= 0 && part_stride >= n && (part_stride & 3) == 0, "topk_mask_parts: bad arguments");
+    if (int e = check_select_outputs("topk_mask_parts", mask, packed, counts, multiple_of, n)) return e;
     CM_CHECK(!static_mask || (static_rows > 0 && static_stride >= n && (static_stride & 3) == 0 && ((uintptr_t)static_mask & 3) == 0),
              "topk_mask_parts: bad static mask geometry");
     CM_CHECK(((uintptr_t)mask & 3) == 0 && ((uintptr_t)part & 7) == 0, "topk_mask_parts: unaligned buffers");
+    const bool select = topk_select_takes(n);
+    CM_CHECK(select || mask, "topk_mask_parts: rows of %d columns (or the options set) take a form that needs the bool mask", n);
     if (rows == 0) return CHIPMUNK_OK;
     TopkMaskParams p = {nullptr, (const uint8_t *)static_mask, (const uint8_t *)group_flags, (uint8_t *)mask, 0, static_stride,
                         rows, n, k, static_mask ? static_rows : 1, (float)random_amount,
                         random_amount > 0.0 ? chipmunk_next_random_salt() : 0u};
     p.parts = part, p.pstride = part_stride, p.nrb = nrb, p.ngroups = groups_per_bh, p.nq = Nq;
+    if (select) {
+        p.packed = (uint8_t *)packed, p.counts = counts, p.multiple_of = multiple_of;
+        launch_topk_select<true>(p, s);
+        CM_LAUNCH_CHECK();
+        return CHIPMUNK_OK;
+    }
     if (n > 1024 * 120 || chipmunk_get_option("topk_mask_stream") == 1) hipLaunchKernelGGL((topk_mask_stream_kernel<true, true>), dim3(rows), dim3(1024), 0, s, p);
     else if (n <= 1024 * 16) hipLaunchKernelGGL((topk_mask_kernel<16, true, true>), dim3(rows), dim3(1024), 0, s, p);
     else if (n <= 1024 * 48) hipLaunchKernelGGL((topk_mask_kernel<48, true, true>), dim3(rows), dim3(1024), 0, s, p);
     else hipLaunchKernelGGL((topk_mask_kernel<120, true, true>), dim3(rows), dim3(1024), 0, s, p);
     CM_LAUNCH_CHECK();
-    return CHIPMUNK_OK;
+    return select_outputs_from_mask(mask, packed, counts, multiple_of, rows, n, s);
+}
+
+int chipmunk_topk_mask_parts(const uint16_t *part, int part_stride, int nrb, int groups_per_bh, int Nq, const void *static_mask, int64_t static_stride,
+                             int static_rows, const void *group_flags, void *mask, int rows, int n, int k, double random_amount,
+                             hipStream_t s) {
+    CM_CHECK(mask, "topk_mask_parts: bad arguments");
+    return chipmunk_topk_mask_parts_ex(part, part_stride, nrb, groups_per_bh, Nq, static_mask, static_stride, static_rows, group_flags, mask,
+                                       nullptr, nullptr, 0, rows, n, k, random_amount, s);
 }
 
 __global__ __launch_bounds__(256) void qkv_split_norm_kernel(const uint16_t *qkv, int64_t row_stride, const uint16_t *qw,
@@ -1266,22 +1531,31 @@
     return CHIPMUNK_OK;
 }
 
-extern "C" int chipmunk_topk_mask(const void *cs, int64_t cs_stride, const void *static_mask, int64_t static_stride,
-                                  int static_rows, const void *group_flags, void *mask, int rows, int n, int k,
-                                  double random_amount, void *stream) {
-    CM_CHECK(cs && mask, "topk_mask: null pointer");
+extern "C" int chipmunk_topk_mask_ex(const void *cs, int64_t cs_stride, const void *static_mask, int64_t static_stride,
+                                     int static_rows, const void *group_flags, void *mask, void *packed, int32_t *counts,
+                                     int multiple_of, int rows, int n, int k, double random_amount, void *stream) {
+    CM_CHECK(cs, "topk_mask: null pointer");
     CM_CHECK(rows >= 0 && n > 0 && k >= 0, "topk_mask: bad sizes (rows=%d n=%d k=%d)", rows, n, k);
+    if (int e = check_select_outputs("topk_mask", mask, packed, counts, multiple_of, n)) return e;
     CM_CHECK(cs_stride >= n, "topk_mask: cs row stride %lld < n %d", (long long)cs_stride, n);
     CM_CHECK(n <= CHIPMUNK_TOPK_MASK_MAX_N, "topk_mask: rows of more than %d columns are not supported (got %d)", CHIPMUNK_TOPK_MASK_MAX_N, n);
     CM_CHECK(!static_mask || (static_rows > 0 && static_stride >= n), "topk_mask: bad static mask geometry");
     CM_CHECK(random_amount >= 0.0 && random_amount <= 1.0, "topk_mask: random_amount must be in [0,1]");
+    const bool aligned = n % 4 == 0 && (((uintptr_t)cs) & 7) == 0 && (cs_stride * 2) % 8 == 0 && (((uintptr_t)mask) & 3) == 0 &&
+                         (!static_mask || ((((uintptr_t)static_mask) & 3) == 0 && static_stride % 4 == 0));
+    const bool select = aligned && topk_select_takes(n);
+    CM_CHECK(select || mask, "topk_mask: rows of %d columns (or their alignment, or the options set) take a form that needs the bool mask", n);
     if (rows == 0) return CHIPMUNK_OK;
     TopkMaskParams p = {(const uint16_t *)cs, (const uint8_t *)static_mask, (const uint8_t *)group_flags, (uint8_t *)mask,
                         cs_stride, static_stride, rows, n, k, static_mask ? static_rows : 1, (float)random_amount,
                         random_amount > 0.0 ? chipmunk_next_random_salt() : 0u};
     hipStream_t s = (hipStream_t)stream;
-    const bool aligned = n % 4 == 0 && (((uintptr_t)cs) & 7) == 0 && (cs_stride * 2) % 8 == 0 && (((uintptr_t)mask) & 3) == 0 &&
-                         (!static_mask || ((((uintptr_t)static_mask) & 3) == 0 && static_stride % 4 == 0));
+    if (select) {
+        p.packed = (uint8_t *)packed, p.counts = counts, p.multiple_of = multiple_of;
+        launch_topk_select<false>(p, s);
+        CM_LAUNCH_CHECK();
+        return CHIPMUNK_OK;
+    }
 #define LAUNCH_TM(KPT)                                                                                       \
     do {                                                                                                     \
         if (aligned) hipLaunchKernelGGL((topk_mask_kernel<KPT, true>), dim3(rows), dim3(1024), 0, s, p);     \
@@ -1295,7 +1569,15 @@
     else LAUNCH_TM(120);
 #undef LAUNCH_TM
     CM_LAUNCH_CHECK();
-    return CHIPMUNK_OK;
+    return select_outputs_from_mask(mask, packed, counts, multiple_of, rows, n, s);
+}
+
+extern "C" int chipmunk_topk_mask(const void *cs, int64_t cs_stride, const void *static_mask, int64_t static_stride,
+                                  int static_rows, const void *group_flags, void *mask, int rows, int n, int k,
+                                  double random_amount, void *stream) {
+    CM_CHECK(cs && mask, "topk_mask: null pointer");
+    return chipmunk_topk_mask_ex(cs, cs_stride, static_mask, static_stride, static_rows, group_flags, mask, nullptr, nullptr, 0, rows, n, k,
+                                 random_amount, stream);
 }
 
 extern "C" int chipmunk_compact_indices(const int32_t *indices, int64_t idx_stride, const int32_t *counts, const int64_t *offsets,
diff --git a/chipmunk_amd/csrc/torch_registry.cpp b/chipmunk_amd/csrc/torch_registry.cpp
--- a/chipmunk_amd/csrc/torch_registry.cpp
+++ b/chipmunk_amd/csrc/torch_registry.cpp
@@ -765,7 +765,7 @@
 }
 
 std::vector<at::Tensor> mask_to_ragged_indices(at::Tensor mask, at::IntArrayRef shape, int64_t multiple_of, int64_t pad_to_multiple_of,
-                                               bool sorted) {
+                                               bool sorted, const c10::optional<at::Tensor> &row_counts) {
     CHECK_DEV(mask);
     const bool packed = mask.scalar_type() == at::kByte;
     TORCH_CHECK(packed || mask.scalar_type() == at::kBool, "mask must be bool, or uint8 bit-packed with a shape");
@@ -778,11 +778,21 @@
     const int64_t pad_n = ((n + pad_to_multiple_of - 1) / pad_to_multiple_of) * pad_to_multiple_of;
     TORCH_CHECK(n > 0 && pad_n <= INT_MAX, "rows must have between 1 and 2^31 - 1 columns");
     c10::DeviceGuard guard(mask.device());
-    at::Tensor counts = at::empty({b, h, m}, mask.options().dtype(at::kInt));
-    at::Tensor len = at::empty({rows}, mask.options().dtype(at::kLong));
-    check(chipmunk_mask_row_counts(mask.data_ptr(), packed ? 1 : 0, counts.data_ptr<int>(), len.data_ptr<int64_t>(), rows, (int)n,
-                                   (int)pad_n, (int)multiple_of, cur_stream(mask)),
-          "mask_to_ragged_indices");
+    at::Tensor counts, len;
+    if (row_counts.has_value() && row_counts->defined()) {
+        counts = *row_counts;
+        CHECK_DEV(counts);
+        TORCH_CHECK(counts.scalar_type() == at::kInt && counts.numel() == rows && counts.is_contiguous() && counts.device() == mask.device(),
+                    "counts must be a contiguous int32 tensor of b * h * m entries on the mask's device");
+        counts = counts.view({b, h, m});
+        len = counts.reshape({rows}).to(at::kLong).clamp_max(pad_n).add_(31).div_(32, "floor").mul_(32);
+    } else {
+        counts = at::empty({b, h, m}, mask.options().dtype(at::kInt));
+        len = at::empty({rows}, mask.options().dtype(at::kLong));
+        check(chipmunk_mask_row_counts(mask.data_ptr(), packed ? 1 : 0, counts.data_ptr<int>(), len.data_ptr<int64_t>(), rows, (int)n,
+                                       (int)pad_n, (int)multiple_of, cur_stream(mask)),
+              "mask_to_ragged_indices");
+    }
     at::Tensor offsets = at::zeros({rows + 1}, len.options());
     if (rows) offsets.narrow(0, 1, rows).copy_(len.cumsum(0));
     const int64_t total = rows ? offsets[rows].item<int64_t>() : 0;
@@ -795,13 +805,14 @@
 }
 
 std::vector<at::Tensor> dense_colsum_attn_layout(at::Tensor q, at::Tensor k, at::Tensor v, at::Tensor p, bool token_major_o);
-at::Tensor topk_mask(at::Tensor cs, int64_t k, double random_amount, const c10::optional<at::Tensor> &groups,
-                     const c10::optional<at::Tensor> &static_mask);
-std::vector<at::Tensor> dense_colsum_topk_mask(at::Tensor q, at::Tensor k, at::Tensor v, at::Tensor p, int64_t k_top, double random_amount,
-                                               const c10::optional<at::Tensor> &groups, const c10::optional<at::Tensor> &static_mask,
-                                               bool token_major_o) {
+static std::vector<at::Tensor> topk_mask_impl(at::Tensor cs, int64_t k, double random_amount, const c10::optional<at::Tensor> &groups,
+                                              const c10::optional<at::Tensor> &static_mask, bool outputs, int64_t multiple_of, bool want_mask);
+static std::vector<at::Tensor> dense_colsum_topk_impl(at::Tensor q, at::Tensor k, at::Tensor v, at::Tensor p, int64_t k_top, double random_amount,
+                                                      const c10::optional<at::Tensor> &groups, const c10::optional<at::Tensor> &static_mask,
+                                                      bool token_major_o, bool outputs, int64_t multiple_of, bool want_mask) {
     CHECK_DEV(q); CHECK_DEV(k); CHECK_DEV(v); CHECK_DEV(p);
     CHECK_BF16(q); CHECK_BF16(k); CHECK_BF16(v);
+    if (outputs) TORCH_CHECK(k.dim() == 4 && k.size(2) % 8 == 0 && multiple_of > 0, "the packed output needs a key count that is a multiple of 8 and a positive multiple_of");
     const bool shapes_ok = q.dim() == 4 && k.dim() == 4 && v.dim() == 4 && q.size(3) == 128 && q.stride(3) == 1 && k.stride(3) == 1 &&
                            v.stride(3) == 1 && p.scalar_type() == at::kFloat && p.is_contiguous();
     if (shapes_ok) {
@@ -831,13 +842,21 @@
             at::Tensor o = alloc_o(q, q, token_major_o);
             const int64_t os[3] = {o.stride(0), o.stride(1), o.stride(2)};
             at::Tensor l = at::empty({B, H, Nq, 1}, q.options().dtype(at::kFloat));
-            at::Tensor mask = at::empty({B, H, G, Nk}, q.options().dtype(at::kBool));
+            const bool with_mask = want_mask || !outputs || !chipmunk_topk_select_fused((int)Nk);
+            at::Tensor mask = with_mask ? at::empty({B, H, G, Nk}, q.options().dtype(at::kBool)) : at::empty({0}, q.options().dtype(at::kBool));
+            at::Tensor packed, counts;
+            if (outputs) {
+                packed = at::empty({B * H * G * Nk / 8}, q.options().dtype(at::kByte));
+                counts = at::empty({B, H, G}, q.options().dtype(at::kInt));
+            }
             const int64_t qs[3] = {q.stride(0), q.stride(1), q.stride(2)}, ks[3] = {k.stride(0), k.stride(1), k.stride(2)},
                           vs[3] = {v.stride(0), v.stride(1), v.stride(2)};
-            const int rc = chipmunk_dense_colsum_topk_mask_strided(q.data_ptr(), k.data_ptr(), v.data_ptr(), qs, ks, vs, p.data_ptr<float>(), o.data_ptr(),
+            const int rc = chipmunk_dense_colsum_topk_mask_ex(q.data_ptr(), k.data_ptr(), v.data_ptr(), qs, ks, vs, p.data_ptr<float>(), o.data_ptr(),
                                                            os, l.data_ptr<float>(), (int)B, (int)H, (int)Nq, (int)Nk, st, st_stride, (int)st_rows, gf,
-                                                           mask.data_ptr(), (int)k_top, random_amount, cur_stream(q));
-            if (rc == CHIPMUNK_OK) return {o, mask, l};
+                                                           with_mask ? mask.data_ptr() : nullptr, outputs ? packed.data_ptr() : nullptr,
+                                                           outputs ? counts.data_ptr<int>() : nullptr, (int)multiple_of, (int)k_top, random_amount,
+                                                           cur_stream(q));
+            if (rc == CHIPMUNK_OK) return {o, mask, l, packed, counts};
             if (rc != CHIPMUNK_ERR_UNSUPPORTED) check(rc, "dense_colsum_topk_mask");
         }
     }
@@ -845,18 +864,32 @@
     at::Tensor cs = ocl[1];
     const int64_t Nk = k.size(2), G = (q.size(2) + 191) / 192;
     if (cs.size(-1) != Nk || cs.size(-2) != G) cs = cs.slice(-2, 0, G).slice(-1, 0, Nk);
-    return {ocl[0], topk_mask(cs, k_top, random_amount, groups, static_mask), ocl[2]};
-}
-
-at::Tensor topk_mask(at::Tensor cs, int64_t k, double random_amount, const c10::optional<at::Tensor> &groups,
-                     const c10::optional<at::Tensor> &static_mask) {
+    auto sel = topk_mask_impl(cs, k_top, random_amount, groups, static_mask, outputs, multiple_of, want_mask);
+    return {ocl[0], sel[0], ocl[2], sel[1], sel[2]};
+}
+
+std::vector<at::Tensor> dense_colsum_topk_mask(at::Tensor q, at::Tensor k, at::Tensor v, at::Tensor p, int64_t k_top, double random_amount,
+                                               const c10::optional<at::Tensor> &groups, const c10::optional<at::Tensor> &static_mask,
+                                               bool token_major_o) {
+    auto r = dense_colsum_topk_impl(q, k, v, p, k_top, random_amount, groups, static_mask, token_major_o, false, 0, true);
+    return {r[0], r[1], r[2]};
+}
+
+std::vector<at::Tensor> dense_colsum_topk_select(at::Tensor q, at::Tensor k, at::Tensor v, at::Tensor p, int64_t k_top, double random_amount,
+                                                 const c10::optional<at::Tensor> &groups, const c10::optional<at::Tensor> &static_mask,
+                                                 bool token_major_o, int64_t multiple_of, bool want_mask) {
+    return dense_colsum_topk_impl(q, k, v, p, k_top, random_amount, groups, static_mask, token_major_o, true, multiple_of, want_mask);
+}
+
+static std::vector<at::Tensor> topk_mask_impl(at::Tensor cs, int64_t k, double random_amount, const c10::optional<at::Tensor> &groups,
+                                              const c10::optional<at::Tensor> &static_mask, bool outputs, int64_t multiple_of, bool want_mask) {
     CHECK_DEV(cs); CHECK_BF16(cs);
     TORCH_CHECK(cs.dim() == 4 && cs.stride(3) == 1, "cs must be [B, H, G, N] with a contiguous last dim");
     const int64_t B = cs.size(0), H = cs.size(1), G = cs.size(2), N = cs.size(3);
+    if (outputs) TORCH_CHECK(N % 8 == 0 && multiple_of > 0, "the packed output needs rows of a multiple of 8 columns and a positive multiple_of");
     if (!(cs.stride(1) == G * cs.stride(2) && (B == 1 || cs.stride(0) == H * cs.stride(1)))) cs = cs.contiguous();
     const int64_t rows = B * H * G;
     c10::DeviceGuard guard(cs.device());
-    at::Tensor mask = at::empty({B, H, G, N}, cs.options().dtype(at::kBool));
     const void *st = nullptr, *gf = nullptr;
     int64_t st_stride = 0, st_rows = 1;
     at::Tensor stc, gfc;
@@ -877,10 +910,30 @@
         gfc = gfc.expand({B, H, G, 1}).contiguous();
         gf = gfc.data_ptr();
     }
-    check(chipmunk_topk_mask(cs.data_ptr(), cs.stride(2), st, st_stride, (int)st_rows, gf, mask.data_ptr(), (int)rows, (int)N,
-                             (int)k, random_amount, cur_stream(cs)),
+    const bool aligned = N % 4 == 0 && ((uintptr_t)cs.data_ptr() & 7) == 0 && cs.stride(2) % 4 == 0 &&
+                         (!st || (((uintptr_t)st & 3) == 0 && st_stride % 4 == 0));
+    const bool with_mask = want_mask || !outputs || !aligned || !chipmunk_topk_select_fused((int)N);
+    at::Tensor mask = with_mask ? at::empty({B, H, G, N}, cs.options().dtype(at::kBool)) : at::empty({0}, cs.options().dtype(at::kBool));
+    at::Tensor packed, counts;
+    if (outputs) {
+        packed = at::empty({rows * N / 8}, cs.options().dtype(at::kByte));
+        counts = at::empty({B, H, G}, cs.options().dtype(at::kInt));
+    }
+    check(chipmunk_topk_mask_ex(cs.data_ptr(), cs.stride(2), st, st_stride, (int)st_rows, gf, with_mask ? mask.data_ptr() : nullptr,
+                                outputs ? packed.data_ptr() : nullptr, outputs ? counts.data_ptr<int>() : nullptr, (int)multiple_of, (int)rows,
+                                (int)N, (int)k, random_amount, cur_stream(cs)),
           "topk_mask");
-    return mask;
+    return {mask, packed, counts};
+}
+
+at::Tensor topk_mask(at::Tensor cs, int64_t k, double random_amount, const c10::optional<at::Tensor> &groups,
+                     const c10::optional<at::Tensor> &static_mask) {
+    return topk_mask_impl(cs, k, random_amount, groups, static_mask, false, 0, true)[0];
+}
+
+std::vector<at::Tensor> topk_mask_select(at::Tensor cs, int64_t k, double random_amount, const c10::optional<at::Tensor> &groups,
+                                         const c10::optional<at::Tensor> &static_mask, int64_t multiple_of, bool want_mask) {
+    return topk_mask_impl(cs, k, random_amount, groups, static_mask, true, multiple_of, want_mask);
 }
 
 at::Tensor bitpack(at::Tensor mask) {
@@ -1030,10 +1083,12 @@
     m.def("mask_to_sorted_indices(Tensor mask, int[] shape, int multiple_of, int pad_to_multiple_of) -> Tensor[]");
     m.def("topk_mask(Tensor cs, int k, float random_amount, Tensor? groups, Tensor? static_mask) -> Tensor");
     m.def("dense_colsum_topk_mask(Tensor q, Tensor k, Tensor v, Tensor p, int k_top, float random_amount, Tensor? groups, Tensor? static_mask, bool token_major_o=False) -> Tensor[]");
+    m.def("dense_colsum_topk_select(Tensor q, Tensor k, Tensor v, Tensor p, int k_top, float random_amount, Tensor? groups, Tensor? static_mask, bool token_major_o, int multiple_of, bool want_mask) -> Tensor[]");
+    m.def("topk_mask_select(Tensor cs, int k, float random_amount, Tensor? groups, Tensor? static_mask, int multiple_of, bool want_mask) -> Tensor[]");
     m.def("dense_attn_layout(Tensor q, Tensor k, Tensor v, bool token_major_o) -> Tensor[]");
     m.def("dense_colsum_attn_layout(Tensor q, Tensor k, Tensor v, Tensor p, bool token_major_o) -> Tensor[]");
     m.def("compact_indices(Tensor indices, Tensor counts) -> Tensor[]");
-    m.def("mask_to_ragged_indices(Tensor mask, int[] shape, int multiple_of, int pad_to_multiple_of, bool sorted) -> Tensor[]");
+    m.def("mask_to_ragged_indices(Tensor mask, int[] shape, int multiple_of, int pad_to_multiple_of, bool sorted, Tensor? counts=None) -> Tensor[]");
     m.def("csp_attn_out_ragged(Tensor q, Tensor k, Tensor v, Tensor o_in, Tensor indices, Tensor offsets, Tensor indices_counts, int o_scale) -> Tensor");
     m.def("residual_ln_modulate(Tensor x, Tensor? y, Tensor? gate, Tensor shift, Tensor scale, float eps) -> Tensor[]");
     m.def("transpose_last2(Tensor x) -> Tensor");
@@ -1052,6 +1107,7 @@
     m.impl("split_heads_rownorm", &split_heads_rownorm);
     m.impl("csp_mlp_mm1_fp8_scatter", &csp_mlp_mm1_fp8_scatter);
     m.impl("dense_colsum_topk_mask", &dense_colsum_topk_mask);
+    m.impl("dense_colsum_topk_select", &dense_colsum_topk_select);
     m.impl("csp_mlp_mm1", &csp_mlp_mm1);
     m.impl("csp_mlp_mm2_and_scatter_add", &csp_mlp_mm2_and_scatter_add);
     m.impl("copy_indices", &copy_indices);
@@ -1078,6 +1134,7 @@
     m.impl("mask_to_sorted_indices", &mask_to_sorted_indices);
     m.impl("mask_to_ragged_indices", &mask_to_ragged_indices);
     m.impl("topk_mask", &topk_mask);
+    m.impl("topk_mask_select", &topk_mask_select);
     m.impl("transpose_last2", &transpose_last2);
     m.impl("transpose_last2_pitched", &transpose_last2_pitched);
     m.impl("block_mean", &block_mean);
diff --git a/chipmunk_amd/modules/attn.py b/chipmunk_amd/modules/attn.py
--- a/chipmunk_amd/modules/attn.py
+++ b/chipmunk_amd/modules/attn.py
@@ -138,10 +138,11 @@
                     and amd_key("attn", "fused_packed_mask_to_indices") and amd_key("attn", "ragged_mask_to_indices"))
 
     @torch.compiler.disable
-    def _ragged_indices(self, packed: Tensor, shape, multiple_of: int, bm: int, mask: Optional[Tensor] = None):
+    def _ragged_indices(self, packed: Tensor, shape, multiple_of: int, bm: int, mask: Optional[Tensor] = None,
+                        counts: Optional[Tensor] = None):
         if shape[-1] % 8 != 0:
             packed = mask if mask is not None else ops.bitunpack(packed, shape)
-        return ops.mask_to_ragged_indices(packed, shape, multiple_of, bm, bool(amd_key("attn", "sorted_indices")))
+        return ops.mask_to_ragged_indices(packed, shape, multiple_of, bm, bool(amd_key("attn", "sorted_indices")), counts)
 
     def _stored_indices(self, multiple_of: int, bm: int):
         cfg = GLOBAL_CONFIG["attn"]
@@ -178,11 +179,17 @@
             if inference_step == 1 or cfg["recompute_mask"]:
                 prev_lse = self.storage.get_lse_constants()
                 tk = int(multiple_of * round((cfg["top_keys"] * k.shape[-2]) / multiple_of))
-                mask = bs = None
+                mask = bs = packed = sel_counts = None
                 if (q.is_cuda and cfg["should_compress_indices"] and tk > 0 and amd_key("attn", "fused_colsum_topk")
                         and amd_key("attn", "fused_topk_mask") and k.shape[-2] <= ops.TOPK_MASK_MAX_N):
                     static, groups = self._static(q.shape[1], _cdiv(q.shape[-2], bm), k.shape[-2])
-                    o, mask, lse = ops.dense_colsum_topk_mask(q, k, v, prev_lse, tk, 0.01, groups, static, tm)
+                    if use_ragged and k.shape[-2] % 8 == 0 and amd_key("attn", "fused_select_outputs"):
+                        o, mask, lse, packed, sel_counts = ops.dense_colsum_topk_select(q, k, v, prev_lse, tk, 0.01, groups, static, tm,
+                                                                                        multiple_of, False)
+                        mask_shape = torch.Size((q.shape[0], q.shape[1], _cdiv(q.shape[-2], bm), k.shape[-2]))
+                        mask = mask if mask.numel() else None
+                    else:
+                        o, mask, lse = ops.dense_colsum_topk_mask(q, k, v, prev_lse, tk, 0.01, groups, static, tm)
                 elif do_padding:
                     o, bs, lse = ops.dense_colsum_attn(q, k, v, prev_lse, tm)
                 else:
@@ -191,17 +198,18 @@
                 lse[..., k.shape[-2]:, :] = 0
                 self.storage.set_lse_constants(lse)
                 if cfg["should_compress_indices"]:
-                    if mask is not None:
+                    if mask is not None or packed is not None:
                         pass
                     elif tk > 0:
                         mask = self.random_and_topk(bs, tk)
                     else:
                         mask = self._static(bs.shape[1], bs.shape[-2], bs.shape[-1])[0]
-                    packed, mask_shape = ops.bitpack(mask)
+                    if packed is None:
+                        packed, mask_shape = ops.bitpack(mask)
                     self.mask_shape[self.layer_counter.cur_model_invocation_per_step] = mask_shape
                     self.storage.set_indices(packed)
                     if use_ragged:
-                        ragged = self._ragged_indices(packed, mask_shape, multiple_of, bm, mask)
+                        ragged = self._ragged_indices(packed, mask_shape, multiple_of, bm, mask, sel_counts)
                         self._remember_indices(None, ragged[2], ragged[:2])
                     else:
                         if mask.is_cuda and amd_key("attn", "fused_packed_mask_to_indices") and amd_key("attn", "sorted_indices"):
diff --git a/chipmunk_amd/ops/__init__.py b/chipmunk_amd/ops/__init__.py
--- a/chipmunk_amd/ops/__init__.py
+++ b/chipmunk_amd/ops/__init__.py
@@ -2,8 +2,8 @@
 from .mlp import run_e2e_glu as mlp_glu, run_e2e_glu, mm1_glu
 from .mlp import run_e2e_glu_fp8 as mlp_glu_fp8, run_e2e_glu_fp8, mm1_glu_fp8
 from .indexed_io import (copy_indices, topk_indices, mask_to_indices, scatter_add, packed_mask_to_indices,
-                         mask_to_sorted_indices, mask_to_ragged_indices, topk_mask, manual_seed, TOPK_MASK_MAX_N)
-from .attn import compact_indices, csp_attn, csp_attn_inplace, csp_attn_out, csp_attn_out_ragged, dense_attn, dense_colsum_attn, dense_colsum_topk_mask
+                         mask_to_sorted_indices, mask_to_ragged_indices, topk_mask, topk_mask_select, manual_seed, TOPK_MASK_MAX_N)
+from .attn import compact_indices, csp_attn, csp_attn_inplace, csp_attn_out, csp_attn_out_ragged, dense_attn, dense_colsum_attn, dense_colsum_topk_mask, dense_colsum_topk_select
 from .patch import patchify, unpatchify, patchify_rope
 from .bitpack import bitpack, bitunpack
 from . import voxel
@@ -11,7 +11,7 @@
 
 __all__ = ["mlp", "copy_indices", "topk_indices", "mask_to_indices", "scatter_add", "csp_attn", "dense_attn",
            "dense_colsum_attn", "patchify", "unpatchify", "patchify_rope", "bitpack", "bitunpack",
-           "packed_mask_to_indices", "mask_to_sorted_indices", "csp_attn_inplace", "csp_attn_out", "topk_mask", "TOPK_MASK_MAX_N", "voxel", "manual_seed", "qkv_split_norm", "dense_colsum_topk_mask", "compact_indices", "csp_attn_out_ragged", "residual_ln_modulate",
+           "packed_mask_to_indices", "mask_to_sorted_indices", "csp_attn_inplace", "csp_attn_out", "topk_mask", "TOPK_MASK_MAX_N", "voxel", "manual_seed", "qkv_split_norm", "dense_colsum_topk_mask", "dense_colsum_topk_select", "topk_mask_select", "compact_indices", "csp_attn_out_ragged", "residual_ln_modulate",
            "split_heads_rownorm", "wan_rope_table", "mask_to_ragged_indices", "mlp_glu", "run_e2e_glu", "mm1_glu",
            "mlp_glu_fp8", "run_e2e_glu_fp8", "mm1_glu_fp8"]
 
diff --git a/chipmunk_amd/ops/_fake.py b/chipmunk_amd/ops/_fake.py
--- a/chipmunk_amd/ops/_fake.py
+++ b/chipmunk_amd/ops/_fake.py
@@ -100,6 +100,22 @@
         return [_o_like(q, token_major_o), q.new_empty((B, H, G, k.shape[2]), dtype=torch.bool),
                 q.new_empty((B, H, Nq, 1), dtype=torch.float32)]
 
+    @lib.register_fake("chipmunk::dense_colsum_topk_select")
+    def _(q, k, v, p, k_top, random_amount, groups, static_mask, token_major_o, multiple_of, want_mask):
+        B, H, Nq, D = q.shape
+        G, Nk = (Nq + 191) // 192, k.shape[2]
+        torch._check(Nk % 8 == 0 and multiple_of > 0, lambda: "the packed output needs a key count that is a multiple of 8 and a positive multiple_of")
+        return [_o_like(q, token_major_o), q.new_empty((B, H, G, Nk) if want_mask else (0,), dtype=torch.bool),
+                q.new_empty((B, H, Nq, 1), dtype=torch.float32), q.new_empty((B * H * G * Nk // 8,), dtype=torch.uint8),
+                q.new_empty((B, H, G), dtype=torch.int32)]
+
+    @lib.register_fake("chipmunk::topk_mask_select")
+    def _(cs, k, random_amount, groups, static_mask, multiple_of, want_mask):
+        B, H, G, N = cs.shape
+        torch._check(N % 8 == 0 and multiple_of > 0, lambda: "the packed output needs rows of a multiple of 8 columns and a positive multiple_of")
+        return [cs.new_empty(cs.shape if want_mask else (0,), dtype=torch.bool), cs.new_empty((B * H * G * N // 8,), dtype=torch.uint8),
+                cs.new_empty((B, H, G), dtype=torch.int32)]
+
     @lib.register_fake("chipmunk::qkv_split_norm")
     def _(qkv, q_weight, k_weight, heads, eps, freqs_cos=None, freqs_sin=None):
         out = qkv.new_empty((3, 1, heads, qkv.shape[0], 128))
diff --git a/chipmunk_amd/ops/attn.py b/chipmunk_amd/ops/attn.py
--- a/chipmunk_amd/ops/attn.py
+++ b/chipmunk_amd/ops/attn.py
@@ -59,6 +59,19 @@
     return o, mask, l
 
 
+def dense_colsum_topk_select(q: torch.Tensor, k: torch.Tensor, v: torch.Tensor, p: torch.Tensor, k_top: int, random_amount: float,
+                             groups, static_mask, token_major_o: bool = False, multiple_of: int = 1, want_mask: bool = False):
+    n = q.shape[-2]
+    padded = _pad_len(n)
+    assert p.shape[-2] in (n, padded), "p must be the l vector of the previous full step"
+    o, mask, l, packed, counts = torch.ops.chipmunk.dense_colsum_topk_select(
+        _last_dim_contiguous(q), _last_dim_contiguous(k), _last_dim_contiguous(v), p[..., :n, :].contiguous(), k_top, random_amount, groups,
+        static_mask, token_major_o, multiple_of, want_mask)
+    if padded != n:
+        l = F.pad(l, (0, 0, 0, padded - n))
+    return o, mask, l, packed, counts
+
+
 def csp_attn(q: torch.Tensor, k: torch.Tensor, v: torch.Tensor, indices: torch.Tensor,
              indices_counts: torch.Tensor) -> torch.Tensor:
     return torch.ops.chipmunk.csp_128_attn(q.contiguous(), k.contiguous(), v.contiguous(), indices.contiguous(),
@@ -85,4 +98,4 @@
 
 
 __all__ = ["csp_attn", "csp_attn_inplace", "csp_attn_out", "csp_attn_out_ragged", "compact_indices", "dense_attn", "dense_colsum_attn",
-           "dense_colsum_topk_mask"]
+           "dense_colsum_topk_mask", "dense_colsum_topk_select"]
diff --git a/chipmunk_amd/ops/indexed_io.py b/chipmunk_amd/ops/indexed_io.py
--- a/chipmunk_amd/ops/indexed_io.py
+++ b/chipmunk_amd/ops/indexed_io.py
@@ -40,9 +40,9 @@
 
 
 def mask_to_ragged_indices(mask: torch.Tensor, shape: Sequence[int], multiple_of: int, pad_to_multiple_of: int,
-                           sorted: bool = True) -> List[torch.Tensor]:
+                           sorted: bool = True, counts: Optional[torch.Tensor] = None) -> List[torch.Tensor]:
     if mask.is_cuda:
-        return torch.ops.chipmunk.mask_to_ragged_indices(mask, list(shape), multiple_of, pad_to_multiple_of, sorted)
+        return torch.ops.chipmunk.mask_to_ragged_indices(mask, list(shape), multiple_of, pad_to_multiple_of, sorted, counts)
     if mask.dtype == torch.uint8:
         from .bitpack import bitunpack
         mask = bitunpack(mask, shape)
@@ -70,6 +70,11 @@
     return torch.ops.chipmunk.topk_mask(cs, k, random_amount, groups, static_mask)
 
 
+def topk_mask_select(cs: torch.Tensor, k: int, random_amount: float = 0.0, groups: Optional[torch.Tensor] = None,
+                     static_mask: Optional[torch.Tensor] = None, multiple_of: int = 1, want_mask: bool = True) -> List[torch.Tensor]:
+    return torch.ops.chipmunk.topk_mask_select(cs, k, random_amount, groups, static_mask, multiple_of, want_mask)
+
+
 def manual_seed(seed: int) -> None:
     from .._native import manual_seed as _seed
     _seed(seed)
diff --git a/chipmunk_amd/util/config.py b/chipmunk_amd/util/config.py
--- a/chipmunk_amd/util/config.py
+++ b/chipmunk_amd/util/config.py
@@ -81,6 +81,7 @@
     "attn.keep_unpacked_indices_offloaded": True,
     "attn.kept_indices_offloaded_budget_gb": 8.0,
     "attn.ragged_mask_to_indices": True,
+    "attn.fused_select_outputs": True,
 }
 BASE_CONFIG["offloading"]["keep_resident_if_fits"] = AMD_EXTRA_KEYS["offloading.keep_resident_if_fits"]
 BASE_CONFIG["offloading"]["hbm_budget_gb"] = AMD_EXTRA_KEYS["offloading.hbm_budget_gb"]
@@ -97,6 +98,7 @@
 BASE_CONFIG["attn"]["keep_unpacked_indices_offloaded"] = AMD_EXTRA_KEYS["attn.keep_unpacked_indices_offloaded"]
 BASE_CONFIG["attn"]["kept_indices_offloaded_budget_gb"] = AMD_EXTRA_KEYS["attn.kept_indices_offloaded_budget_gb"]
 BASE_CONFIG["attn"]["ragged_mask_to_indices"] = AMD_EXTRA_KEYS["attn.ragged_mask_to_indices"]
+BASE_CONFIG["attn"]["fused_select_outputs"] = AMD_EXTRA_KEYS["attn.fused_select_outputs"]
 
 GLOBAL_CONFIG: Dict[str, Any] = copy.deepcopy(BASE_CONFIG)
 
diff --git a/include/chipmunk_hip.h b/include/chipmunk_hip.h
--- a/include/chipmunk_hip.h
+++ b/include/chipmunk_hip.h
@@ -157,6 +157,16 @@
                        int static_rows, const void *group_flags, void *mask, int rows, int n, int k,
                        double random_amount, void *stream);
 
+int chipmunk_topk_mask_ex(const void *cs, int64_t cs_stride, const void *static_mask, int64_t static_stride, int static_rows,
+                          const void *group_flags, void *mask, void *packed, int32_t *counts, int multiple_of, int rows, int n,
+                          int k, double random_amount, void *stream);
+int chipmunk_topk_select_fused(int n);
+int chipmunk_dense_colsum_topk_mask_ex(const void *q, const void *k, const void *v, const int64_t q_strides[3],
+                                       const int64_t k_strides[3], const int64_t v_strides[3], const float *p, void *o,
+                                       const int64_t *o_strides, float *l, int B, int H, int Nq, int Nk, const void *static_mask,
+                                       int64_t static_stride, int static_rows, const void *group_flags, void *mask, void *packed,
+                                       int32_t *counts, int multiple_of, int k_top, double random_amount, void *stream);
+
 int chipmunk_mask_to_indices(const void *mask, int32_t *indices, int32_t *counts, int64_t rows, int n, int pad_n,
                              int multiple_of, void *stream);
 
```

Measured after the change: 0.5819 (median of 2 runs). No clear change (+0.2%).
